# neu-vi/Superpoints_Registration

Hardware: AMD Instinct MI355X
Metric: point-cloud pairs/sec (16 384 pts/cloud) (higher is better)
Workload: dtype f32 (matrix products: range-scaled split-f16x2 MFMA, f32 accumulate; attention weights below 2^-5 of their row sum carried in one f16 plane); 1 GPU; synthetic 16384-pt pairs, full KPConv backbone + superpoint attn + Sinkhorn-SVD pose (3dmatch config, BASELINE configs[1]); streams_per_gpu=1, points_per_cloud=16384, generator=box, point_order=reference, upsample_indices=True, cross_step_overlap=True, streams_inside_a_forward=3: main path, pyramid searches, ResNet shortcut branches

## Files before the change

### include/spr.h

```cpp
#ifndef SPR_H_
#define SPR_H_

#include <stddef.h>
#include <stdint.h>

#ifdef __cplusplus
extern "C" {
#endif

#define SPR_VERSION 5

#define SPR_ACT_NONE 0
#define SPR_ACT_RELU 1
#define SPR_ACT_SIGMOID 2

#define SPR_ORDER_REFERENCE 0
#define SPR_ORDER_CANONICAL 1

int spr_version(void);
const char* spr_last_error(void);

size_t spr_grid_subsample_workspace_bytes(int n, int nb);
int spr_grid_subsample(const float* xyz, const int* cu, int n, int nb, float dl,
                       int max_p, int order_mode, float* out_xyz, int* out_lens,
                       int* out_total, void* ws, size_t ws_bytes, void* stream);

size_t spr_voxel_downsample_workspace_bytes(int n);
int spr_voxel_downsample(const float* xyz, int n, double voxel_size, int* out_idx,
                         int* out_count, void* ws, size_t ws_bytes, void* stream);

size_t spr_radius_neighbors_workspace_bytes(int nq, int ns, int nb);
int spr_radius_neighbors(const float* q_xyz, const int* q_cu, int nq,
                         const float* s_xyz, const int* s_cu, int ns, int nb,
                         float radius, int limit, int algo, int* out_idx,
                         int* max_count, void* ws, size_t ws_bytes, void* stream);

size_t spr_radius_table_bytes(int ns, int nb);
size_t spr_radius_table_build_workspace_bytes(int ns, int nb);
size_t spr_radius_table_query_workspace_bytes(int nq);
int spr_radius_table_slots(void);
int spr_radius_table_build(const float* s_xyz, const int* s_cu, int ns, int nb, float radius,
                           void* table, size_t table_bytes, void* ws, size_t ws_bytes, void* stream);
int spr_radius_table_query(const float* q_xyz, const int* q_cu, int nq, int self, int ns, int nb,
                           float radius, int limit, int slot, const void* table, int* out_idx,
                           int* max_count, void* ws, size_t ws_bytes, void* stream);
int spr_radius_table_query_a(const float* q_xyz, const int* q_cu, int nq, int self, int ns, int nb,
                             float radius, int limit, int slot, const void* table, int* out_idx,
                             int* max_count, int algo, void* ws, size_t ws_bytes, void* stream);

size_t spr_kpconv_workspace_bytes(int nq, int ns, int cin, int cout);
int spr_kpconv_fwd(const float* q_xyz, int nq, const float* s_xyz, int ns,
                   const int* nbr, int nbr_stride, int kmax, int rows_sorted,
                   const float* x, int cin, const float* weights, int cout,
                   const float* kernel_points, int n_kp, float kp_extent,
                   float* out, int impl, void* ws, size_t ws_bytes,
                   void* stream);

size_t spr_instnorm_workspace_bytes(int max_len_host, int nb, int c);
int spr_instnorm(const float* x, const int* cu, int n, int nb, int max_len_host,
                 int c, float eps, int norm, const float* add, float slope,
                 float* out, void* ws, size_t ws_bytes, void* stream);

int spr_block_tail_tile_rows(int ka, int kb, int n_out);
size_t spr_block_tail_tiles_len(int n, int nb, int tile_rows);
int spr_block_tail_tiles(const int* cu, int n, int nb, int tile_rows, int* tiles, void* stream);
size_t spr_block_tail_workspace_bytes(int n, int nb, int kb, int n_out, int tile_rows);
int spr_block_tail(const float* xa, int ka, const float* wa, const float* xb, int kb,
                   const float* wb, const float* add, const int* cu, const int* tiles, int n,
                   int nb, int n_out, float eps, float slope, float* out,
                   const float* xa_range, int xa_range_n, const float* wa_range, int wa_range_n,
                   const float* xb_range, int xb_range_n, const float* wb_range, int wb_range_n,
                   float* out_range, int out_range_n, void* ws, size_t ws_bytes, void* stream);
int spr_block_tail_n(const float* xa, int ka, const float* wa, const float* xb, int kb, const float* wb,
                     const float* add, const int* cu, const int* tiles, int n, int nb, int n_out, float eps,
                     float slope, float* out, const float* xa_range, int xa_range_n, const float* wa_range,
                     int wa_range_n, const float* xb_range, int xb_range_n, const float* wb_range,
                     int wb_range_n, float* out_range, int out_range_n, const float* xa_mean,
                     const float* xa_rstd, float xa_slope, void* ws, size_t ws_bytes, void* stream);
int spr_instnorm_stats(const float* x, const int* cu, int n, int nb, int max_len_host, int c, float eps,
                       float* mean, float* rstd, void* ws, size_t ws_bytes, void* stream);

int spr_maxpool_gather(const float* x, int ns, int c, const int* idx, int nq,
                       int idx_stride, int k, float* out, void* stream);

size_t spr_linear_workspace_bytes(void);
int spr_linear(const float* x, int m, int k, const float* w, int n,
               const float* bias, const float* residual, int act, float* out,
               void* ws, size_t ws_bytes, void* stream);
int spr_range_parts(void);
int spr_absmax(const float* x, long rows, int cols, long stride, float* parts, void* stream);
int spr_absmax_multi(const void* jobs_dev, int njobs, int parts_per_job, float* parts_out, void* stream);
int spr_linear_r(const float* x, int m, int k, const float* w, int n, const float* bias,
                 const float* residual, int act, float* out, const float* x_range,
                 int x_range_n, const float* w_range, int w_range_n, float* out_range,
                 int out_range_cap, int* out_range_n_host, void* ws, size_t ws_bytes, void* stream);
int spr_kpconv_fwd_r(const float* q_xyz, int nq, const float* s_xyz, int ns, const int* nbr,
                     int nbr_stride, int kmax, int rows_sorted, const float* x, int cin,
                     const float* weights, int cout, const float* kernel_points, int n_kp,
                     float kp_extent, float* out, int impl, const float* x_range, int x_range_n,
                     const float* w_range, int w_range_n, void* ws, size_t ws_bytes, void* stream);
size_t spr_kpconv_plan_bytes(int nq);
int spr_kpconv_plan(const int* nbr, int nq, int ns, int nbr_stride, int kmax, int rows_sorted,
                    const int* order, void* plan, size_t plan_bytes, void* stream);
size_t spr_kpconv_wplanes_bytes(int cin, int cout);
int spr_kpconv_prep_weights(const float* weights, int n_kp, int cin, int cout, const float* w_range,
                            int w_range_n, void* wplanes, size_t wplanes_bytes, void* stream);
int spr_kpconv_fwd_p(const float* q_xyz, int nq, const float* s_xyz, int ns, const int* nbr,
                     int nbr_stride, int kmax, int rows_sorted, const float* x, int cin,
                     const float* weights, int cout, const float* kernel_points, int n_kp,
                     float kp_extent, float* out, int impl, const float* x_range, int x_range_n,
                     const float* w_range, int w_range_n, const void* plan, const void* wplanes,
                     void* ws, size_t ws_bytes, void* stream);
int spr_instnorm_r(const float* x, const int* cu, int n, int nb, int max_len_host, int c,
                   float eps, int norm, const float* add, float slope, float* out,
                   float* out_range, int out_range_n, void* ws, size_t ws_bytes, void* stream);
int spr_maxpool_gather_r(const float* x, int ns, int c, const int* idx, int nq, int idx_stride,
                         int k, float* out, float* out_range, int out_range_n, void* stream);
int spr_maxpool_gather_o(const float* x, int ns, int c, const int* idx, int nq, int idx_stride, int k,
                         const int* order, float* out, float* out_range, int out_range_n, void* stream);
size_t spr_cell_order_workspace_bytes(int n);
int spr_cell_order(const float* xyz, const int* cu, int n, int nb, float cell, int* order, void* ws, size_t ws_bytes,
                   void* stream);
int spr_layernorm_range_count(int m);
int spr_layernorm_r(const float* x, int m, int c, const float* gamma, const float* beta,
                    float eps, const float* pos, float* out_norm, float* out_pos,
                    float* range_norm, float* range_pos, void* stream);
int spr_attn_inproj_prepare(const float* w_in, int d, float* out, void* stream);
int spr_attn_inproj_varlen_fwd_r(const float* x_qk, const float* x_v, int t, const float* w_in,
                                 const float* b_in, const int* cu, const int* kv_seg, int nseg,
                                 int max_len_host, int nhead, int head_dim, float scale,
                                 float* out, int o_stride, const float* xqk_range,
                                 int xqk_range_n, const float* xv_range, int xv_range_n,
                                 float* out_range, const float* w_prep, void* ws, size_t ws_bytes, void* stream);

int spr_set_gemm_mode(int mode);

int spr_layernorm(const float* x, int m, int c, const float* gamma,
                  const float* beta, float eps, const float* pos,
                  float* out_norm, float* out_pos, void* stream);

int spr_posemb_sine(const float* xyz, int n, int d_model, float scale,
                    float temperature, float* out, void* stream);

size_t spr_attn_workspace_bytes(int t, int nseg, int nhead, int head_dim);
int spr_attn_varlen_fwd(const float* q, int q_stride, const float* k,
                        int k_stride, const float* v, int v_stride,
                        const int* cu, const int* kv_seg, int t, int nseg,
                        int max_len_host, int nhead, int head_dim, float scale,
                        float* out, int o_stride, void* ws, size_t ws_bytes,
                        void* stream);
int spr_attn_varlen_fwd_lse(const float* q, int q_stride, const float* k, int k_stride, const float* v,
                            int v_stride, const int* cu, const int* kv_seg, int t, int nseg, int max_len_host,
                            int nhead, int head_dim, float scale, float* out, int o_stride, float* lse,
                            int* lse_written, void* ws, size_t ws_bytes, void* stream);

size_t spr_attn_inproj_workspace_bytes(int t, int nseg, int nhead, int head_dim);
int spr_attn_inproj_varlen_fwd(const float* x_qk, const float* x_v, int t,
                               const float* w_in, const float* b_in,
                               const int* cu, const int* kv_seg, int nseg,
                               int max_len_host, int nhead, int head_dim,
                               float scale, float* out, int o_stride, void* ws,
                               size_t ws_bytes, void* stream);

size_t spr_attn_probs_workspace_bytes(int t, int nhead, int head_dim);
int spr_attn_probs(const float* q, int q_stride, const float* k, int k_stride, const int* cu,
                   const int* kv_seg, int t, int nseg, int max_len_host, int nhead, int head_dim,
                   float scale, int per_head, float* out, const long long* place, int max_rows_host,
                   int max_cols_host, void* ws, size_t ws_bytes, void* stream);

#define SPR_XENC_PTRS_PER_LAYER 18
size_t spr_xenc_prepared_bytes(int n_layers, int d_ff);
size_t spr_xenc_plan_bytes(void);
int spr_xenc_prepare(const void* const* layer_ptrs_host, const float* eps_host, int n_layers,
                     int d_model, int nhead, int d_ff, const float* final_g, const float* final_b,
                     float final_eps, float pos_bound, void* prepared, size_t prepared_bytes,
                     void* plan_host, size_t plan_bytes, void* stream);
size_t spr_xenc_workspace_bytes(int t, int nseg);
int spr_xenc_forward(const void* plan_host, const float* x, const float* pos, const int* cu,
                     const int* kv_self, const int* kv_cross, int t, int nseg, int max_len_host,
                     float* out, void* ws, size_t ws_bytes, void* stream);

size_t spr_attn_bwd_workspace_bytes(int t, int nhead);
size_t spr_attn_bwd_workspace_bytes2(int t, int nseg, int nhead);
int spr_attn_varlen_bwd(const float* q, int q_stride, const float* k, int k_stride, const float* v,
                        int v_stride, const float* out, int o_stride, const float* dout,
                        int do_stride, const int* cu, const int* kv_seg, const int* q_seg, int t,
                        int nseg, int max_len_host, int nhead, int head_dim, float scale,
                        float* dq, float* dk, float* dv, void* ws, size_t ws_bytes, void* stream);
int spr_attn_varlen_bwd_lse(const float* q, int q_stride, const float* k, int k_stride, const float* v,
                            int v_stride, const float* out, int o_stride, const float* dout, int do_stride,
                            const float* lse, const int* cu, const int* kv_seg, const int* q_seg, int t, int nseg,
                            int max_len_host, int nhead, int head_dim, float scale, float* dq, float* dk,
                            float* dv, void* ws, size_t ws_bytes, void* stream);

int spr_set_attn_mode(int mode);

size_t spr_match_workspace_bytes(const int* cu_host, int npairs);
int spr_match_dualsoftmax(const float* feat, int d, const int* cu,
                          const int* cu_host, int npairs, float* match_val,
                          int* match_ind, void* ws, size_t ws_bytes,
                          void* stream);

int spr_match_dualsoftmax2(const float* feat, int d, const int* cu,
                           const int* cu_host, int npairs, float* match_val,
                           float* match_val2, int* match_ind, void* ws, size_t ws_bytes,
                           void* stream);

int spr_pose_residuals(const float* pose, const float* a, const float* b, const int* pair_cu,
                       int npairs, int total_host, float* res, void* stream);
int spr_pose_scores(const float* poses, int nh, const float* a, const float* b, int n,
                    float* score, void* stream);

int spr_weighted_procrustes(const float* a, const float* b, const float* w,
                            const int* pair_cu, int npairs, float* out_pose,
                            void* stream);

size_t spr_sinkhorn_workspace_bytes(const int* cu_host, int npairs);
int spr_sinkhorn_correspondences(const float* feat, int d, const float* xyz,
                                 const int* cu, const int* cu_host, int npairs,
                                 const float* alpha, const float* beta, int n_iters,
                                 int slack, float* out_w, float* out_that,
                                 void* ws, size_t ws_bytes, void* stream);

int spr_match_sinkhorn(const float* feat, int d, const float* xyz, const int* cu, const int* cu_host,
                       int npairs, const float* alpha, const float* beta, int n_iters, float* match_val,
                       float* match_val2, int* match_ind, float* out_w, float* out_that, void* ws,
                       size_t ws_bytes, void* stream);

int spr_gather_rows(const float* x, int n_src, int c, const int* idx, int n,
                    float* out, void* stream);

size_t spr_loss_workspace_bytes(int n_max, int m_max, int d);
int spr_overlap_pool(const float* ov_prev, int ns_prev, const int* pool,
                     int pool_stride, int w, int nq, float* out, void* stream);
int spr_bce_logits_mean(const float* x, const float* y, int n, float* out,
                        void* ws, size_t ws_bytes, void* stream);
int spr_infonce_pair(const float* anchor_feat, int n, const float* positive_feat,
                     int m, int d, const float* anchor_xyz, const float* pose_gt,
                     const float* positive_xyz, const float* W, float r_p,
                     float r_n, float* out, void* ws, size_t ws_bytes,
                     void* stream);
int spr_transform_l1_pair(const float* pose_gt, const float* pose_pred,
                          const float* xyz, int n, float* out, void* ws,
                          size_t ws_bytes, void* stream);
int spr_sum_scaled(const float* values, int n, float scale, float* out,
                   void* stream);

int spr_bgemm(const float* A, const float* B, float* C, const void* desc_dev, int nbatch,
              int max_m, int max_n, long sa_i, long sa_k, long sb_k, long sb_j, long sc_i,
              long sc_j, float alpha, float beta, void* stream);
size_t spr_tn_product_split_workspace_bytes(void);
int spr_tn_product_split(const float* L, const float* R, long rows, int nl, int nr, int chunk,
                         const float* l_range, int l_range_n, const float* r_range, int r_range_n,
                         float* parts, void* ws, size_t ws_bytes, void* stream);
size_t spr_tn_product_f64_workspace_bytes(long rows, int nl, int nr);
int spr_tn_product_f64(const float* L, const float* R, long rows, int nl, int nr, float* out,
                       void* ws, size_t ws_bytes, void* stream);
int spr_reduce_parts(const float* parts, int nparts, long n, float scale, float* out,
                     int accumulate, void* stream);
int spr_act_bwd(const float* y, const float* dy, int act, long n, float* out, void* stream);
size_t spr_colsum_workspace_bytes(int n);
int spr_colsum(const float* x, long m, int n, float* out, void* ws, size_t ws_bytes, void* stream);
size_t spr_layernorm_bwd_workspace_bytes(int c);
int spr_layernorm_bwd(const float* x, int m, int c, const float* gamma, float eps,
                      const float* dy_norm, const float* dy_pos, float* dx, float* dgamma,
                      float* dbeta, void* ws, size_t ws_bytes, void* stream);
size_t spr_instnorm_bwd_workspace_bytes(int max_len_host, int nb, int c);
int spr_instnorm_bwd(const float* x, const float* out, const float* dout, const int* cu, int n,
                     int nb, int max_len_host, int c, float eps, int norm, float slope,
                     float* dx, float* dadd, void* ws, size_t ws_bytes, void* stream);
size_t spr_scatter_workspace_bytes(long rows, int c);
int spr_maxpool_bwd(const float* x, int ns, int c, const int* idx, int nq, int idx_stride, int k,
                    const float* dy, float* dx, void* ws, size_t ws_bytes, void* stream);
int spr_scatter_rows_add(const float* dy, const int* idx, int n, int c, int n_src, float* dx,
                         void* ws, size_t ws_bytes, void* stream);
int spr_kpconv_weighted_features(const float* q_xyz, int nq, const float* s_xyz, int ns,
                                 const int* nbr, int nbr_stride, int kmax, const float* x, int cin,
                                 const float* kernel_points, int n_kp, float kp_extent,
                                 float* wf, float* cnt, void* stream);
int spr_kpconv_weighted_features_f(const float* q_xyz, int nq, const float* s_xyz, int ns,
                                   const int* nbr, int nbr_stride, int kmax, const float* x, int cin,
                                   const float* kernel_points, int n_kp, float kp_extent,
                                   float* wf, float* cnt, void* ws, size_t ws_bytes, void* stream);
size_t spr_kpconv_weighted_features_workspace_bytes(int ns);
int spr_kpconv_bwd_dx(const float* q_xyz, int nq, const float* s_xyz, int ns, const int* nbr,
                      int nbr_stride, int kmax, int cin, const float* kernel_points, int n_kp,
                      float kp_extent, const float* dwf, float* dx, void* ws, size_t ws_bytes,
                      void* stream);
int spr_kpconv_bwd_dx_r(const float* q_xyz, int nq, const float* s_xyz, int ns, const int* nbr,
                        int nbr_stride, int kmax, int cin, const float* kernel_points, int n_kp,
                        float kp_extent, const float* dwf, const float* dwf_range, int dwf_range_n, float* dx,
                        void* ws, size_t ws_bytes, void* stream);
int spr_softmax_rows(float* mat, const void* desc_dev, int nbatch, int max_m, void* stream);
int spr_softmax_bwd_rows(const float* p, float* dp, const void* desc_dev, int nbatch, int max_m,
                         void* stream);

int spr_bce_logits_mean_bwd(const float* x, const float* y, int n, const float* gout, float* dx,
                            void* stream);
int spr_infonce_pair_dlogits(const float* anchor_feat, int n, const float* positive_feat, int m,
                             int d, const float* anchor_xyz, const float* pose_gt,
                             const float* positive_xyz, const float* W, float r_p, float r_n,
                             float* dlogits, float* row_mask, float* wsym_out, float* t_out,
                             void* ws, size_t ws_bytes, void* stream);
int spr_wsym_bwd(const float* dwsym, int d, float* dW, void* stream);
int spr_transform_l1_pair_bwd(const float* pose_gt, const float* pose_pred, const float* xyz, int n,
                              const float* gout, float* dpose_pred, void* stream);
int spr_weighted_procrustes_bwd(const float* a, const float* b, const float* w,
                                const int* pair_cu, int npairs, const float* dpose, float* da,
                                float* db, float* dw, void* stream);
size_t spr_sinkhorn_bwd_workspace_bytes(const int* cu_host, int npairs, int n_iters);
int spr_sinkhorn_bwd(const float* feat, int d, const float* xyz, const int* cu,
                     const int* cu_host, int npairs, const float* alpha, const float* beta,
                     int n_iters, const float* dw, const float* dthat, float* dfeat,
                     float* dalpha, float* dbeta, void* ws, size_t ws_bytes, void* stream);

size_t spr_circle_loss_workspace_bytes(int nbatch, int max_n, int max_m);
int spr_circle_loss(const float* src_feat, const float* tgt_feat, int d, const float* src_xyz,
                    const float* pose_gt, const float* tgt_xyz, const int* cu_src, const int* cu_tgt,
                    int nbatch, int max_n, int max_m, float r_p, float r_n, float* out, void* ws,
                    size_t ws_bytes, void* stream);
int spr_circle_loss_bwd(const float* src_feat, const float* tgt_feat, int d, const float* src_xyz,
                        const float* pose_gt, const float* tgt_xyz, const int* cu_src, const int* cu_tgt,
                        int nbatch, int max_n, int max_m, float r_p, float r_n, const float* gout, float* G,
                        float* d_src, float* d_tgt, void* ws, size_t ws_bytes, void* stream);

int spr_prof_enable(int on);
int spr_prof_read(int max_records, int* codes_host, int* nqs_host, float* ms_host);

int spr_selftest(int* status_host);

#ifdef __cplusplus
}
#endif
#endif
```

### superpoints_registration_amd/_lib.py

```python
import ctypes
import os
import subprocess

_HERE = os.path.dirname(os.path.abspath(__file__))
LIB_PATH = os.environ.get("SPR_HIP_LIB") or os.path.join(_HERE, "libspr_hip.so")

_vp = ctypes.c_void_p
_i = ctypes.c_int
_f = ctypes.c_float
_sz = ctypes.c_size_t
_l = ctypes.c_long

SIGNATURES = {
    "spr_version": (_i, []),
    "spr_last_error": (ctypes.c_char_p, []),
    "spr_grid_subsample_workspace_bytes": (_sz, [_i, _i]),
    "spr_grid_subsample": (_i, [_vp, _vp, _i, _i, _f, _i, _i, _vp, _vp, _vp, _vp, _sz, _vp]),
    "spr_voxel_downsample_workspace_bytes": (_sz, [_i]),
    "spr_voxel_downsample": (_i, [_vp, _i, ctypes.c_double, _vp, _vp, _vp, _sz, _vp]),
    "spr_radius_neighbors_workspace_bytes": (_sz, [_i, _i, _i]),
    "spr_radius_neighbors": (_i, [_vp, _vp, _i, _vp, _vp, _i, _i, _f, _i, _i, _vp, _vp, _vp, _sz, _vp]),
    "spr_radius_table_bytes": (_sz, [_i, _i]),
    "spr_radius_table_build_workspace_bytes": (_sz, [_i, _i]),
    "spr_radius_table_query_workspace_bytes": (_sz, [_i]),
    "spr_radius_table_slots": (_i, []),
    "spr_radius_table_build": (_i, [_vp, _vp, _i, _i, _f, _vp, _sz, _vp, _sz, _vp]),
    "spr_radius_table_query": (_i, [_vp, _vp, _i, _i, _i, _i, _f, _i, _i, _vp, _vp, _vp, _vp, _sz, _vp]),
    "spr_radius_table_query_a": (_i, [_vp, _vp, _i, _i, _i, _i, _f, _i, _i, _vp, _vp, _vp, _i, _vp, _sz, _vp]),
    "spr_kpconv_workspace_bytes": (_sz, [_i, _i, _i, _i]),
    "spr_kpconv_fwd": (_i, [_vp, _i, _vp, _i, _vp, _i, _i, _i, _vp, _i, _vp, _i, _vp, _i, _f, _vp,
                            _i, _vp, _sz, _vp]),
    "spr_instnorm_workspace_bytes": (_sz, [_i, _i, _i]),
    "spr_instnorm": (_i, [_vp, _vp, _i, _i, _i, _i, _f, _i, _vp, _f, _vp, _vp, _sz, _vp]),
    "spr_maxpool_gather": (_i, [_vp, _i, _i, _vp, _i, _i, _i, _vp, _vp]),
    "spr_linear_workspace_bytes": (_sz, []),
    "spr_linear": (_i, [_vp, _i, _i, _vp, _i, _vp, _vp, _i, _vp, _vp, _sz, _vp]),
    "spr_linear_r": (_i, [_vp, _i, _i, _vp, _i, _vp, _vp, _i, _vp, _vp, _i, _vp, _i, _vp, _i, _vp, _vp, _sz, _vp]),
    "spr_range_parts": (_i, []),
    "spr_absmax_multi": (_i, [_vp, _i, _i, _vp, _vp]),
    "spr_absmax": (_i, [_vp, _l, _i, _l, _vp, _vp]),
    "spr_kpconv_fwd_r": (_i, [_vp, _i, _vp, _i, _vp, _i, _i, _i, _vp, _i, _vp, _i, _vp, _i, _f, _vp,
                              _i, _vp, _i, _vp, _i, _vp, _sz, _vp]),
    "spr_kpconv_plan_bytes": (_sz, [_i]),
    "spr_kpconv_plan": (_i, [_vp, _i, _i, _i, _i, _i, _vp, _vp, _sz, _vp]),
    "spr_kpconv_wplanes_bytes": (_sz, [_i, _i]),
    "spr_kpconv_prep_weights": (_i, [_vp, _i, _i, _i, _vp, _i, _vp, _sz, _vp]),
    "spr_kpconv_fwd_p": (_i, [_vp, _i, _vp, _i, _vp, _i, _i, _i, _vp, _i, _vp, _i, _vp, _i, _f, _vp,
                              _i, _vp, _i, _vp, _i, _vp, _vp, _vp, _sz, _vp]),
    "spr_instnorm_r": (_i, [_vp, _vp, _i, _i, _i, _i, _f, _i, _vp, _f, _vp, _vp, _i, _vp, _sz, _vp]),
    "spr_block_tail_tile_rows": (_i, [_i, _i, _i]),
    "spr_block_tail_tiles_len": (_sz, [_i, _i, _i]),
    "spr_block_tail_tiles": (_i, [_vp, _i, _i, _i, _vp, _vp]),
    "spr_block_tail_workspace_bytes": (_sz, [_i, _i, _i, _i, _i]),
    "spr_block_tail": (_i, [_vp, _i, _vp, _vp, _i, _vp, _vp, _vp, _vp, _i, _i, _i, _f, _f, _vp, _vp, _i, _vp, _i,
                            _vp, _i, _vp, _i, _vp, _i, _vp, _sz, _vp]),
    "spr_block_tail_n": (_i, [_vp, _i, _vp, _vp, _i, _vp, _vp, _vp, _vp, _i, _i, _i, _f, _f, _vp, _vp, _i, _vp, _i,
                              _vp, _i, _vp, _i, _vp, _i, _vp, _vp, _f, _vp, _sz, _vp]),
    "spr_instnorm_stats": (_i, [_vp, _vp, _i, _i, _i, _i, _f, _vp, _vp, _vp, _sz, _vp]),
    "spr_maxpool_gather_r": (_i, [_vp, _i, _i, _vp, _i, _i, _i, _vp, _vp, _i, _vp]),
    "spr_maxpool_gather_o": (_i, [_vp, _i, _i, _vp, _i, _i, _i, _vp, _vp, _vp, _i, _vp]),
    "spr_cell_order_workspace_bytes": (_sz, [_i]),
    "spr_cell_order": (_i, [_vp, _vp, _i, _i, _f, _vp, _vp, _sz, _vp]),
    "spr_layernorm_range_count": (_i, [_i]),
    "spr_layernorm_r": (_i, [_vp, _i, _i, _vp, _vp, _f, _vp, _vp, _vp, _vp, _vp, _vp]),
    "spr_attn_inproj_varlen_fwd_r": (_i, [_vp, _vp, _i, _vp, _vp, _vp, _vp, _i, _i, _i, _i, _f, _vp, _i, _vp, _i, _vp,
                                          _i, _vp, _vp, _vp, _sz, _vp]),
    "spr_attn_inproj_prepare": (_i, [_vp, _i, _vp, _vp]),
    "spr_set_gemm_mode": (_i, [_i]),
    "spr_layernorm": (_i, [_vp, _i, _i, _vp, _vp, _f, _vp, _vp, _vp, _vp]),
    "spr_posemb_sine": (_i, [_vp, _i, _i, _f, _f, _vp, _vp]),
    "spr_attn_workspace_bytes": (_sz, [_i, _i, _i, _i]),
    "spr_attn_varlen_fwd": (_i, [_vp, _i, _vp, _i, _vp, _i, _vp, _vp, _i, _i, _i, _i, _i, _f, _vp, _i,
                                 _vp, _sz, _vp]),
    "spr_attn_varlen_fwd_lse": (_i, [_vp, _i, _vp, _i, _vp, _i, _vp, _vp, _i, _i, _i, _i, _i, _f, _vp, _i, _vp, _vp,
                                     _vp, _sz, _vp]),
    "spr_attn_varlen_bwd_lse": (_i, [_vp, _i, _vp, _i, _vp, _i, _vp, _i, _vp, _i, _vp, _vp, _vp, _vp, _i, _i, _i, _i,
                                     _i, _f, _vp, _vp, _vp, _vp, _sz, _vp]),
    "spr_attn_probs_workspace_bytes": (_sz, [_i, _i, _i]),
    "spr_attn_probs": (_i, [_vp, _i, _vp, _i, _vp, _vp, _i, _i, _i, _i, _i, _f, _i, _vp, _vp, _i, _i, _vp, _sz,
                            _vp]),
    "spr_attn_bwd_workspace_bytes": (_sz, [_i, _i]),
    "spr_attn_bwd_workspace_bytes2": (_sz, [_i, _i, _i]),
    "spr_attn_varlen_bwd": (_i, [_vp, _i, _vp, _i, _vp, _i, _vp, _i, _vp, _i, _vp, _vp, _vp, _i, _i, _i, _i, _i, _f,
                                 _vp, _vp, _vp, _vp, _sz, _vp]),
    "spr_attn_inproj_workspace_bytes": (_sz, [_i, _i, _i, _i]),
    "spr_attn_inproj_varlen_fwd": (_i, [_vp, _vp, _i, _vp, _vp, _vp, _vp, _i, _i, _i, _i, _f, _vp, _i, _vp,
                                        _sz, _vp]),
    "spr_set_attn_mode": (_i, [_i]),
    "spr_xenc_prepared_bytes": (_sz, [_i, _i]),
    "spr_xenc_plan_bytes": (_sz, []),
    "spr_xenc_prepare": (_i, [_vp, _vp, _i, _i, _i, _i, _vp, _vp, _f, _f, _vp, _sz, _vp, _sz, _vp]),
    "spr_xenc_workspace_bytes": (_sz, [_i, _i]),
    "spr_xenc_forward": (_i, [_vp, _vp, _vp, _vp, _vp, _vp, _i, _i, _i, _vp, _vp, _sz, _vp]),
    "spr_match_workspace_bytes": (_sz, [_vp, _i]),
    "spr_match_dualsoftmax": (_i, [_vp, _i, _vp, _vp, _i, _vp, _vp, _vp, _sz, _vp]),
    "spr_match_dualsoftmax2": (_i, [_vp, _i, _vp, _vp, _i, _vp, _vp, _vp, _vp, _sz, _vp]),
    "spr_pose_residuals": (_i, [_vp, _vp, _vp, _vp, _i, _i, _vp, _vp]),
    "spr_pose_scores": (_i, [_vp, _i, _vp, _vp, _i, _vp, _vp]),
    "spr_weighted_procrustes": (_i, [_vp, _vp, _vp, _vp, _i, _vp, _vp]),
    "spr_sinkhorn_workspace_bytes": (_sz, [_vp, _i]),
    "spr_match_sinkhorn": (_i, [_vp, _i, _vp, _vp, _vp, _i, _vp, _vp, _i, _vp, _vp, _vp, _vp, _vp, _vp, _sz, _vp]),
    "spr_sinkhorn_correspondences": (_i, [_vp, _i, _vp, _vp, _vp, _i, _vp, _vp, _i, _i, _vp, _vp, _vp,
                                          _sz, _vp]),
    "spr_loss_workspace_bytes": (_sz, [_i, _i, _i]),
    "spr_overlap_pool": (_i, [_vp, _i, _vp, _i, _i, _i, _vp, _vp]),
    "spr_bce_logits_mean": (_i, [_vp, _vp, _i, _vp, _vp, _sz, _vp]),
    "spr_infonce_pair": (_i, [_vp, _i, _vp, _i, _i, _vp, _vp, _vp, _vp, _f, _f, _vp, _vp, _sz, _vp]),
    "spr_transform_l1_pair": (_i, [_vp, _vp, _vp, _i, _vp, _vp, _sz, _vp]),
    "spr_sum_scaled": (_i, [_vp, _i, _f, _vp, _vp]),
    "spr_gather_rows": (_i, [_vp, _i, _i, _vp, _i, _vp, _vp]),
    "spr_bgemm": (_i, [_vp, _vp, _vp, _vp, _i, _i, _i, _l, _l, _l, _l, _l, _l, _f, _f, _vp]),
    "spr_tn_product_split_workspace_bytes": (_sz, []),
    "spr_tn_product_split": (_i, [_vp, _vp, _l, _i, _i, _i, _vp, _i, _vp, _i, _vp, _vp, _sz, _vp]),
    "spr_tn_product_f64_workspace_bytes": (_sz, [_l, _i, _i]),
    "spr_tn_product_f64": (_i, [_vp, _vp, _l, _i, _i, _vp, _vp, _sz, _vp]),
    "spr_reduce_parts": (_i, [_vp, _i, _l, _f, _vp, _i, _vp]),
    "spr_act_bwd": (_i, [_vp, _vp, _i, _l, _vp, _vp]),
    "spr_colsum_workspace_bytes": (_sz, [_i]),
    "spr_colsum": (_i, [_vp, _l, _i, _vp, _vp, _sz, _vp]),
    "spr_layernorm_bwd_workspace_bytes": (_sz, [_i]),
    "spr_layernorm_bwd": (_i, [_vp, _i, _i, _vp, _f, _vp, _vp, _vp, _vp, _vp, _vp, _sz, _vp]),
    "spr_instnorm_bwd_workspace_bytes": (_sz, [_i, _i, _i]),
    "spr_instnorm_bwd": (_i, [_vp, _vp, _vp, _vp, _i, _i, _i, _i, _f, _i, _f, _vp, _vp, _vp, _sz, _vp]),
    "spr_scatter_workspace_bytes": (_sz, [_l, _i]),
    "spr_maxpool_bwd": (_i, [_vp, _i, _i, _vp, _i, _i, _i, _vp, _vp, _vp, _sz, _vp]),
    "spr_scatter_rows_add": (_i, [_vp, _vp, _i, _i, _i, _vp, _vp, _sz, _vp]),
    "spr_kpconv_weighted_features_workspace_bytes": (_sz, [_i]),
    "spr_kpconv_weighted_features": (_i, [_vp, _i, _vp, _i, _vp, _i, _i, _vp, _i, _vp, _i, _f, _vp, _vp, _vp]),
    "spr_kpconv_weighted_features_f": (_i, [_vp, _i, _vp, _i, _vp, _i, _i, _vp, _i, _vp, _i, _f, _vp, _vp, _vp, _sz, _vp]),
    "spr_kpconv_bwd_dx": (_i, [_vp, _i, _vp, _i, _vp, _i, _i, _i, _vp, _i, _f, _vp, _vp, _vp, _sz, _vp]),
    "spr_kpconv_bwd_dx_r": (_i, [_vp, _i, _vp, _i, _vp, _i, _i, _i, _vp, _i, _f, _vp, _vp, _i, _vp, _vp, _sz, _vp]),
    "spr_softmax_rows": (_i, [_vp, _vp, _i, _i, _vp]),
    "spr_softmax_bwd_rows": (_i, [_vp, _vp, _vp, _i, _i, _vp]),
    "spr_bce_logits_mean_bwd": (_i, [_vp, _vp, _i, _vp, _vp, _vp]),
    "spr_infonce_pair_dlogits": (_i, [_vp, _i, _vp, _i, _i, _vp, _vp, _vp, _vp, _f, _f, _vp, _vp, _vp, _vp, _vp, _sz,
                                      _vp]),
    "spr_wsym_bwd": (_i, [_vp, _i, _vp, _vp]),
    "spr_transform_l1_pair_bwd": (_i, [_vp, _vp, _vp, _i, _vp, _vp, _vp]),
    "spr_weighted_procrustes_bwd": (_i, [_vp, _vp, _vp, _vp, _i, _vp, _vp, _vp, _vp, _vp]),
    "spr_sinkhorn_bwd_workspace_bytes": (_sz, [_vp, _i, _i]),
    "spr_sinkhorn_bwd": (_i, [_vp, _i, _vp, _vp, _vp, _i, _vp, _vp, _i, _vp, _vp, _vp, _vp, _vp, _vp, _sz, _vp]),
    "spr_circle_loss_workspace_bytes": (_sz, [_i, _i, _i]),
    "spr_circle_loss": (_i, [_vp, _vp, _i, _vp, _vp, _vp, _vp, _vp, _i, _i, _i, _f, _f, _vp, _vp, _sz, _vp]),
    "spr_circle_loss_bwd": (_i, [_vp, _vp, _i, _vp, _vp, _vp, _vp, _vp, _i, _i, _i, _f, _f, _vp, _vp, _vp, _vp, _vp,
                                 _sz, _vp]),
    "spr_selftest": (_i, [_vp]),
    "spr_prof_enable": (_i, [_i]),
    "spr_prof_read": (_i, [_i, _vp, _vp, _vp]),
}

_lib = None


def build(force: bool = False) -> str:
    if force:
        subprocess.check_call(["make", "-s", "-C", os.path.join(_HERE, "csrc"), "clean"])
    subprocess.check_call(["make", "-s", "-j8", "-C", os.path.join(_HERE, "csrc")])
    return LIB_PATH


def lib():
    global _lib
    if _lib is None:
        if not os.path.exists(LIB_PATH):
            raise RuntimeError(
                f"{LIB_PATH} is missing: build it with "
                "`python -c 'import __graft_entry__ as g; g.build()'` "
                "(there is no fallback path)")
        l = ctypes.CDLL(LIB_PATH)
        for name, (res, args) in SIGNATURES.items():
            fn = getattr(l, name)
            fn.restype = res
            fn.argtypes = args
        _lib = l
    return _lib


def check(rc: int, what: str) -> None:
    if rc != 0:
        msg = lib().spr_last_error()
        raise RuntimeError(f"{what}: {msg.decode() if msg else 'error'} (status {rc})")
```

### superpoints_registration_amd/csrc/kpconv.hip

```cpp
#include "spr_common.h"

namespace spr {
namespace {

constexpr int kKP = 15;

__global__ __launch_bounds__(256) void k_rowflag(const float* __restrict__ x, const float* __restrict__ s_xyz,
                                                 int ns, int cin, unsigned char* __restrict__ flag,
                                                 float4* __restrict__ sxf, int* __restrict__ tile_ctr) {
  const int wid = (blockIdx.x * blockDim.x + threadIdx.x) >> 6;
  const int lane = threadIdx.x & 63;
  const int c4 = cin >> 2;
  if (blockIdx.x == 0 && threadIdx.x == 0) {
    sxf[ns] = make_float4(-1.0e17f, -1.0e17f, -1.0e17f, __int_as_float(0));
    tile_ctr[0] = 0;
  }
  if ((cin & 3) == 0 && c4 <= 64 && (c4 & (c4 - 1)) == 0) {
    constexpr int kRfSteps = 4;
    const int rpl = 64 / c4;
    const int sub = lane / c4, chunk = lane % c4;
    const int row0 = wid * rpl * kRfSteps + sub;
    float4 v[kRfSteps];
#pragma unroll
    for (int r = 0; r < kRfSteps; ++r) {
      const int row = row0 + r * rpl;
      v[r] = make_float4(0.f, 0.f, 0.f, 0.f);
      if (row < ns) v[r] = reinterpret_cast<const float4*>(x + (size_t)row * cin)[chunk];
    }
#pragma unroll
    for (int r = 0; r < kRfSteps; ++r) {
      const int row = row0 + r * rpl;
      float c[4] = {v[r].x, v[r].y, v[r].z, v[r].w};
#pragma unroll
      for (int e = 0; e < 4; ++e) {
        float t = c[e];
        if (c4 == 64) {
          const int b = lane & 15;
          const float a0 = __shfl(t, b, 64), a1 = __shfl(t, b | 16, 64), a2 = __shfl(t, b | 32, 64),
                      a3 = __shfl(t, b | 48, 64);
          t = ((a0 + a1) + a2) + a3;
        } else if (c4 == 32) {
          t += __shfl_xor(t, 16, 64);
        }
        for (int o = (c4 < 16 ? c4 : 16) >> 1; o > 0; o >>= 1) t += __shfl_xor(t, o, 64);
        c[e] = t;
      }
      const float t = (c[0] + c[2]) + (c[1] + c[3]);
      if (chunk == 0 && row < ns) {
        const int f = t > 0.f ? 1 : 0;
        flag[row] = (unsigned char)f;
        sxf[row] = make_float4(s_xyz[3 * (size_t)row], s_xyz[3 * (size_t)row + 1],
                               s_xyz[3 * (size_t)row + 2], __int_as_float(f));
      }
    }
    return;
  }
  const int row = wid;
  if (row >= ns) return;
  float s = 0.f;
  for (int c = lane; c < cin; c += 64) s += x[(size_t)row * cin + c];
  s = wave_sum(s);
  if (lane == 0) {
    const int f = s > 0.f ? 1 : 0;
    flag[row] = (unsigned char)f;
    sxf[row] = make_float4(s_xyz[3 * (size_t)row], s_xyz[3 * (size_t)row + 1],
                           s_xyz[3 * (size_t)row + 2], __int_as_float(f));
  }
}

__global__ void k_kpconv_simple(const float* __restrict__ q_xyz, int nq,
                                const float* __restrict__ s_xyz, int ns,
                                const int* __restrict__ nbr, int nbr_stride, int kmax,
                                const float* __restrict__ x, int cin,
                                const float* __restrict__ W, int cout,
                                const float* __restrict__ kpts, int n_kp, float inv_extent,
                                const unsigned char* __restrict__ flag,
                                float* __restrict__ out) {
  const long gid = (long)blockIdx.x * blockDim.x + threadIdx.x;
  if (gid >= (long)nq * cout) return;
  const int n = (int)(gid / cout), o = (int)(gid % cout);
  const float qx = q_xyz[3 * (size_t)n], qy = q_xyz[3 * (size_t)n + 1], qz = q_xyz[3 * (size_t)n + 2];
  float acc = 0.f;
  int cnt = 0;
  for (int k = 0; k < kmax; ++k) {
    const int idx = nbr[(size_t)n * nbr_stride + k];
    if (idx < 0 || idx >= ns) continue;
    cnt += flag[idx];
    const float rx = s_xyz[3 * (size_t)idx] - qx, ry = s_xyz[3 * (size_t)idx + 1] - qy,
                rz = s_xyz[3 * (size_t)idx + 2] - qz;
    for (int p = 0; p < n_kp; ++p) {
      const float dx = rx - kpts[3 * p], dy = ry - kpts[3 * p + 1], dz = rz - kpts[3 * p + 2];
      const float w = fmaxf(0.f, 1.f - sqrtf(dx * dx + dy * dy + dz * dz) * inv_extent);
      if (w > 0.f) {
        float d = 0.f;
        for (int c = 0; c < cin; ++c)
          d += x[(size_t)idx * cin + c] * W[((size_t)p * cin + c) * cout + o];
        acc += w * d;
      }
    }
  }
  out[(size_t)n * cout + o] = acc / (float)max(cnt, 1);
}

__global__ __launch_bounds__(256) void k_records_cin1(const float* __restrict__ x, const float* __restrict__ s_xyz,
                                                      int ns, float4* __restrict__ sxf) {
  const int i = blockIdx.x * blockDim.x + threadIdx.x;
  if (i < ns) sxf[i] = make_float4(s_xyz[3 * (size_t)i], s_xyz[3 * (size_t)i + 1], s_xyz[3 * (size_t)i + 2], x[i]);
}

__global__ __launch_bounds__(256) void k_kpconv_cin1(
    const float* __restrict__ q_xyz, int nq, const float* __restrict__ s_xyz, int ns,
    const int* __restrict__ nbr, int nbr_stride, int kmax, int rows_sorted,
    const float4* __restrict__ sxf, const float* __restrict__ W, int cout,
    const float* __restrict__ kpts, int n_kp, float inv_extent, float* __restrict__ out) {
  const int lane = threadIdx.x & 63, wave = threadIdx.x >> 6;
  const int qv = lane & 15, g = lane >> 4;
  const int q0 = blockIdx.x * 64 + wave * 16;
  if (q0 >= nq) return;
  const int n = min(q0 + qv, nq - 1);
  const float qx = q_xyz[3 * (size_t)n], qy = q_xyz[3 * (size_t)n + 1], qz = q_xyz[3 * (size_t)n + 2];
  float kx[4], ky[4], kz[4];
  bool kok[4];
#pragma unroll
  for (int s = 0; s < 4; ++s) {
    const int p = 4 * s + g;
    kok[s] = p < n_kp;
    kx[s] = kok[s] ? kpts[3 * p] : 0.f;
    ky[s] = kok[s] ? kpts[3 * p + 1] : 0.f;
    kz[s] = kok[s] ? kpts[3 * p + 2] : 0.f;
  }
  float wf[4] = {0.f, 0.f, 0.f, 0.f};
  int cnt = 0;
  const int* row = nbr + (size_t)n * nbr_stride;
  for (int k = 0; k < kmax; ++k) {
    const int idx = row[k];
    const bool ok = idx >= 0 && idx < ns;
    if (rows_sorted && __ballot(ok) == 0ull) break;
    const size_t id = ok ? (size_t)idx : 0;
    const float4 rec = sxf[id];
    const float xv = ok ? rec.w : 0.f;
    cnt += xv > 0.f ? 1 : 0;
    const float rx = rec.x - qx, ry = rec.y - qy, rz = rec.z - qz;
#pragma unroll
    for (int s = 0; s < 4; ++s) {
      const float dx = rx - kx[s], dy = ry - ky[s], dz = rz - kz[s];
      const float w = fmaxf(0.f, 1.f - __builtin_amdgcn_sqrtf(dx * dx + dy * dy + dz * dz) * inv_extent);
      wf[s] += kok[s] ? w * xv : 0.f;
    }
  }
  const float inv = 1.f / (float)max(cnt, 1);
#pragma unroll
  for (int s = 0; s < 4; ++s) wf[s] *= inv;
  for (int o0 = 0; o0 < cout; o0 += 16) {
    f32x4 acc = {0.f, 0.f, 0.f, 0.f};
#pragma unroll
    for (int s = 0; s < 4; ++s) {
      const int p = 4 * s + g;
      const float bv = (p < n_kp && o0 + qv < cout) ? W[(size_t)p * cout + o0 + qv] : 0.f;
      acc = __builtin_amdgcn_mfma_f32_16x16x4f32(wf[s], bv, acc, 0, 0, 0);
    }
#pragma unroll
    for (int r = 0; r < 4; ++r) {
      const int qn = q0 + 4 * g + r;
      if (qn < nq && o0 + qv < cout) out[(size_t)qn * cout + o0 + qv] = acc[r];
    }
  }
}

__global__ __launch_bounds__(256) void k_w_prep(const float* __restrict__ W, int cin, int cout, int cc,
                                                const float* __restrict__ w_parts, int n_wparts,
                                                _Float16* __restrict__ Wh, _Float16* __restrict__ Wl) {
  __shared__ float sh[17];
  const float sb = pow2f(pow2_exp_for(block_absmax(w_parts, sh, n_wparts)));
  const int total = kKP * cin * cout;
  const int i = blockIdx.x * blockDim.x + threadIdx.x;
  if (i >= total) return;
  const int KS = kKP * cc / 32, NT = cout / 16;
  const int e = i & 7, lane = (i >> 3) & 63;
  int r = i >> 9;
  const int ks = r % KS;
  r /= KS;
  const int nt = r % NT, chunk = r / NT;
  const int p16 = lane & 15, j4 = lane >> 4;
  const int kk = 32 * ks + 8 * j4 + e;
  const int p = kk / cc, c = chunk * cc + kk % cc;
  const float w = W[((size_t)p * cin + c) * cout + 16 * nt + p16] * sb;
  const _Float16 h = (_Float16)w;
  Wh[i] = h;
  Wl[i] = (_Float16)(w - (float)h);
}

__device__ __forceinline__ void wait_vm(int n) {
  switch (n) {
    case 0: asm volatile("s_waitcnt vmcnt(0)" ::: "memory"); break;
    case 2: asm volatile("s_waitcnt vmcnt(2)" ::: "memory"); break;
    case 4: asm volatile("s_waitcnt vmcnt(4)" ::: "memory"); break;
    case 6: asm volatile("s_waitcnt vmcnt(6)" ::: "memory"); break;
    case 8: asm volatile("s_waitcnt vmcnt(8)" ::: "memory"); break;
    case 12: asm volatile("s_waitcnt vmcnt(12)" ::: "memory"); break;
    case 16: asm volatile("s_waitcnt vmcnt(16)" ::: "memory"); break;
    default: asm volatile("s_waitcnt vmcnt(0)" ::: "memory"); break;
  }
}

typedef _Float16 kh8 __attribute__((ext_vector_type(8)));
template <int N> struct VecF;
template <> struct VecF<2> { typedef float type __attribute__((ext_vector_type(2))); };
template <> struct VecF<4> { typedef float type __attribute__((ext_vector_type(4))); };
template <int N> struct VecH;
template <> struct VecH<2> { typedef _Float16 type __attribute__((ext_vector_type(2))); };
template <> struct VecH<4> { typedef _Float16 type __attribute__((ext_vector_type(4))); };

template <int NTC>
struct KpItem {
  int idx[4];
  float4 sp[4];
  float b[4][NTC];
  float qx, qy, qz;
};

template <int CC, int TQ, int NTW, int NW, int SK, int P1W>
__global__ __launch_bounds__(64 * P1W) void k_kpconv_mfma(
    const float* __restrict__ q_xyz, int nq, const float* __restrict__ s_xyz, int ns,
    const int* __restrict__ nbr, int nbr_stride, int kmax, int rows_sorted,
    const float* __restrict__ x, int cin, const _Float16* __restrict__ Wh,
    const _Float16* __restrict__ Wl, int cout, const float* __restrict__ kpts, float inv_extent,
    const float4* __restrict__ sxf, const float* __restrict__ x_parts,
    const float* __restrict__ w_parts, int n_xparts, int n_wparts, float* __restrict__ out) {
  constexpr int NTC = CC / 16;
  constexpr int MT = TQ / 16;
  constexpr int KW = kKP * CC;
  constexpr int SH = KW + 16;
  constexpr int QPW = TQ / P1W;
  constexpr int NTHR = 64 * P1W;
  static_assert(P1W >= NW && TQ % P1W == 0, "phase-1 waves");
  extern __shared__ __align__(16) unsigned char lds_raw[];
  _Float16* wfh = (_Float16*)lds_raw;
  _Float16* wfl = wfh + TQ * SH;
  int* lcnt = (int*)(wfl + TQ * SH);
  int* lnit = lcnt + TQ;
  int* litem = lnit + P1W;
  const int nblk = (kmax + 15) >> 4;
  const int KP = nblk * 16;
  int* lidx = litem + P1W * QPW * nblk;

  const int tid = threadIdx.x;
  const int wave = tid >> 6, lane = tid & 63;
  const int p16 = lane & 15, j4 = lane >> 4;

  float kx = 0.f, ky = 0.f, kz = 0.f;
  if (p16 < kKP) {
    kx = kpts[3 * p16];
    ky = kpts[3 * p16 + 1];
    kz = kpts[3 * p16 + 2];
  }

  float sa, unscale;
  {
    float* shf = reinterpret_cast<float*>(lds_raw);
    const int ka = pow2_exp_for(block_absmax(x_parts, shf, n_xparts) * (float)kmax);
    const int kb = pow2_exp_for(block_absmax(w_parts, shf, n_wparts));
    __syncthreads();
    sa = pow2f(ka);
    unscale = pow2f(-ka - kb);
  }

  const int ntiles = (nq + TQ - 1) / TQ;
  for (int tile = blockIdx.x; tile < ntiles; tile += gridDim.x) {
  const int q0 = tile * TQ;

  for (int e = tid; e < TQ * KP; e += NTHR) {
    const int q = e / KP, k = e - q * KP;
    const int n = q0 + q;
    lidx[e] = (n < nq && k < kmax) ? nbr[(size_t)n * nbr_stride + k] : ns;
  }
  __syncthreads();
  {
    int n_it = 0;
    for (int qi = 0; qi < QPW; ++qi) {
      const int* row = lidx + (wave * QPW + qi) * KP;
      int nb = nblk;
      if (rows_sorted) {
        int v = 0;
        for (int k0 = 0; k0 < KP; k0 += 64) {
          const int k = k0 + lane;
          const bool ok = k < KP && row[min(k, KP - 1)] >= 0 && row[min(k, KP - 1)] < ns;
          v += __popcll(__ballot(ok));
        }
        nb = max(1, (v + 15) >> 4);
      }
      if (lane < nb) litem[wave * QPW * nblk + n_it + lane] = (qi << 8) | ((lane == nb - 1) ? 128 : 0) | lane;
      n_it += nb;
    }
    if (lane == 0) lnit[wave] = n_it;
  }
  __syncthreads();
  const int n_items = lnit[wave];
  const int* my_items = litem + wave * QPW * nblk;

  constexpr int NG = (SK == 1) ? NW / MT : NW / SK;
  constexpr int MTW = (SK == 1) ? 1 : MT;
  const int mt = (SK == 1) ? wave % MT : 0;
  const int ng = (SK == 1) ? wave / MT : wave % NG;
  const int kh = (SK == 1) ? 0 : wave / NG;
  f32x4 acc2[MTW][NTW];
#pragma unroll
  for (int m = 0; m < MTW; ++m)
#pragma unroll
    for (int t = 0; t < NTW; ++t) acc2[m][t] = (f32x4){0.f, 0.f, 0.f, 0.f};

  for (int c0 = 0; c0 < cin; c0 += CC) {
    f32x4 acc1[NTC];
#pragma unroll
    for (int t = 0; t < NTC; ++t) acc1[t] = (f32x4){0.f, 0.f, 0.f, 0.f};
    int cnt = 0;

    auto issue = [&](int it, KpItem<NTC>& I) {
      const int code = my_items[min(it, n_items - 1)];
      const int qi = code >> 8, b = code & 127;
      const int n = min(q0 + wave * QPW + qi, nq - 1);
      const int* row = lidx + (wave * QPW + qi) * KP + b * 16 + j4;
      I.qx = q_xyz[3 * (size_t)n];
      I.qy = q_xyz[3 * (size_t)n + 1];
      I.qz = q_xyz[3 * (size_t)n + 2];
#pragma unroll
      for (int s = 0; s < 4; ++s) {
        const int id_ = row[4 * s];
        I.idx[s] = id_;
        const bool ok = id_ >= 0 && id_ < ns;
        const size_t id = ok ? (size_t)id_ : 0;
        I.sp[s] = sxf[id];
        typedef typename VecF<NTC>::type vec_t;
        const vec_t xv = *reinterpret_cast<const vec_t*>(x + id * cin + c0 + NTC * p16);
#pragma unroll
        for (int t = 0; t < NTC; ++t) I.b[s][t] = xv[t];
      }
    };
    auto compute = [&](int it, const KpItem<NTC>& I) {
      if (it >= n_items) return;
      const int code = my_items[it];
#pragma unroll
      for (int s = 0; s < 4; ++s) {
        const bool ok = I.idx[s] >= 0 && I.idx[s] < ns;
        const float dx = (I.sp[s].x - I.qx) - kx, dy = (I.sp[s].y - I.qy) - ky,
                    dz = (I.sp[s].z - I.qz) - kz;
        float w = fmaxf(0.f, 1.f - __builtin_amdgcn_sqrtf(dx * dx + dy * dy + dz * dz) * inv_extent);
        if (!ok || p16 >= kKP) w = 0.f;
        cnt += (ok && c0 == 0 && p16 == 0) ? __float_as_int(I.sp[s].w) : 0;
#pragma unroll
        for (int t = 0; t < NTC; ++t) {
          acc1[t] = __builtin_amdgcn_mfma_f32_16x16x4f32(w, I.b[s][t], acc1[t], 0, 0, 0);
        }
      }
      if (code & 128) {
        const int ql = wave * QPW + (code >> 8);
#pragma unroll
        for (int r = 0; r < 4; ++r) {
          const int p = 4 * j4 + r;
          typedef typename VecH<NTC>::type hv_t;
          hv_t hh, ll;
          if constexpr (NTC == 2) {
            unsigned int hu, lu;
            split_pk_s(acc1[0][r], acc1[1][r], sa, hu, lu);
            hh = __builtin_bit_cast(hv_t, hu);
            ll = __builtin_bit_cast(hv_t, lu);
          } else {
            static_assert(NTC == 4, "NTC is 2 or 4");
            typedef unsigned int u2_t __attribute__((ext_vector_type(2)));
            unsigned int h0, l0, h1, l1;
            split_pk_s(acc1[0][r], acc1[1][r], sa, h0, l0);
            split_pk_s(acc1[2][r], acc1[3][r], sa, h1, l1);
            hh = __builtin_bit_cast(hv_t, (u2_t){h0, h1});
            ll = __builtin_bit_cast(hv_t, (u2_t){l0, l1});
          }
          if (p < kKP) {
            *reinterpret_cast<hv_t*>(wfh + ql * SH + p * CC + NTC * p16) = hh;
            *reinterpret_cast<hv_t*>(wfl + ql * SH + p * CC + NTC * p16) = ll;
          }
        }
#pragma unroll
        for (int t = 0; t < NTC; ++t) acc1[t] = (f32x4){0.f, 0.f, 0.f, 0.f};
        if (c0 == 0) {
          int c = cnt;
          c += __shfl_xor(c, 16, 64);
          c += __shfl_xor(c, 32, 64);
          if (lane == 0) lcnt[ql] = c;
        }
        cnt = 0;
      }
    };

    {
      KpItem<NTC> A, B;
      issue(0, A);
      for (int it = 0; it < n_items; it += 2) {
        issue(it + 1, B);
        compute(it, A);
        issue(it + 2, A);
        compute(it + 1, B);
      }
    }
    __syncthreads();
    if (wave < NW) {
      constexpr int NBATCH = KW / 32 / SK;
      const int ks0 = kh * NBATCH;
      constexpr int LPB = 2 * NTW;
      constexpr int D = (NTW <= 2) ? 5 : 3;
      static_assert(NBATCH % D == 0 && NBATCH >= 2 * D && (D - 1) * LPB <= 16, "ring shape");
      const _Float16* ah_row = wfh + (mt * 16 + p16) * SH + 8 * j4;
      const _Float16* al_row = wfl + (mt * 16 + p16) * SH + 8 * j4;
      constexpr int KS = KW / 32;
      const size_t wofs = ((size_t)(c0 / CC) * (cout / 16) + ng * NTW) * KS * 512 + lane * 8;
      kh8 bh[D][NTW], bl[D][NTW];
      auto load_step = [&](int ks, kh8 (&dh)[NTW], kh8 (&dl)[NTW]) {
        const size_t gk = wofs + (size_t)(ks0 + ks) * 512;
#pragma unroll
        for (int t = 0; t < NTW; ++t) {
          const _Float16* ph = Wh + gk + (size_t)t * KS * 512;
          const _Float16* pl = Wl + gk + (size_t)t * KS * 512;
          asm volatile("global_load_dwordx4 %0, %1, off" : "=v"(dh[t]) : "v"(ph));
          asm volatile("global_load_dwordx4 %0, %1, off" : "=v"(dl[t]) : "v"(pl));
        }
      };
      auto mma_step = [&](int ks, const kh8 (&sh)[NTW], const kh8 (&sl)[NTW]) {
#pragma unroll
        for (int m = 0; m < MTW; ++m) {
          const kh8 ah = *reinterpret_cast<const kh8*>(ah_row + m * 16 * SH + 32 * (ks0 + ks));
          const kh8 al = *reinterpret_cast<const kh8*>(al_row + m * 16 * SH + 32 * (ks0 + ks));
#pragma unroll
          for (int t = 0; t < NTW; ++t) {
            acc2[m][t] = __builtin_amdgcn_mfma_f32_16x16x32_f16(ah, sl[t], acc2[m][t], 0, 0, 0);
            acc2[m][t] = __builtin_amdgcn_mfma_f32_16x16x32_f16(al, sh[t], acc2[m][t], 0, 0, 0);
            acc2[m][t] = __builtin_amdgcn_mfma_f32_16x16x32_f16(ah, sh[t], acc2[m][t], 0, 0, 0);
          }
        }
      };
      wait_vm(0);
#pragma unroll
      for (int d = 0; d < D; ++d) load_step(d, bh[d], bl[d]);
      for (int b0 = 0; b0 < NBATCH - D; b0 += D) {
#pragma unroll
        for (int d = 0; d < D; ++d) {
          wait_vm((D - 1) * LPB);
          __builtin_amdgcn_sched_barrier(0);
          mma_step(b0 + d, bh[d], bl[d]);
          __builtin_amdgcn_sched_barrier(0);
          load_step(b0 + d + D, bh[d], bl[d]);
        }
      }
#pragma unroll
      for (int d = 0; d < D; ++d) {
        wait_vm((D - 1 - d) * LPB);
        __builtin_amdgcn_sched_barrier(0);
        mma_step(NBATCH - D + d, bh[d], bl[d]);
      }
    }
    __syncthreads();
  }
  const bool writer = (SK == 1) ? (wave < NW) : (wave < NW && kh == 0);
  if (SK == 2) {
    float* red = reinterpret_cast<float*>(lds_raw);
    if (wave < NW && kh == 1) {
#pragma unroll
      for (int m = 0; m < MTW; ++m)
#pragma unroll
        for (int t = 0; t < NTW; ++t)
#pragma unroll
          for (int r = 0; r < 4; ++r)
            red[(((ng * MTW + m) * NTW + t) * 4 + r) * 64 + lane] = acc2[m][t][r];
    }
    __syncthreads();
    if (writer) {
#pragma unroll
      for (int m = 0; m < MTW; ++m)
#pragma unroll
        for (int t = 0; t < NTW; ++t)
#pragma unroll
          for (int r = 0; r < 4; ++r)
            acc2[m][t][r] += red[(((ng * MTW + m) * NTW + t) * 4 + r) * 64 + lane];
    }
  }
  if (writer) {
#pragma unroll
    for (int m = 0; m < MTW; ++m)
#pragma unroll
      for (int r = 0; r < 4; ++r) {
        const int ql = (mt + m) * 16 + 4 * j4 + r;
        const int n = q0 + ql;
        if (n < nq) {
          const float inv = unscale / (float)max(lcnt[ql], 1);
#pragma unroll
          for (int t = 0; t < NTW; ++t)
            out[(size_t)n * cout + (ng * NTW + t) * 16 + p16] = acc2[m][t][r] * inv;
        }
      }
  }
  __syncthreads();
  }
}

template <int CC, int TQ, int NTW, int NW, int SK, int P1W = NW>
int launch_mfma(const float* q_xyz, int nq, const float* s_xyz, int ns, const int* nbr,
                int nbr_stride, int kmax, int rows_sorted, const float* x, int cin,
                const _Float16* Wh, const _Float16* Wl, int cout, const float* kpts,
                float inv_extent, const float4* sxf, const float* x_parts, const float* w_parts, int n_xparts,
                int n_wparts, float* out, hipStream_t stream) {
  constexpr int SH = kKP * CC + 16;
  constexpr int QPW = TQ / P1W;
  const int nblk = (kmax + 15) / 16;
  const size_t lds = 2 * sizeof(_Float16) * (size_t)TQ * SH + sizeof(int) * (TQ + P1W) +
                     sizeof(int) * (size_t)P1W * QPW * nblk + sizeof(int) * (size_t)TQ * nblk * 16;
  auto kern = k_kpconv_mfma<CC, TQ, NTW, NW, SK, P1W>;
  ProfScope prof(stream, cin * 100000 + cout, nq);
  SPR_REQUIRE(lds <= 160 * 1024, "kpconv: neighbour rows too wide for the LDS tile (kmax=%d)", kmax);
  if (lds > 64 * 1024)
    if (int rc = ensure_dyn_lds((const void*)kern, 160 * 1024)) return rc;
  const int n_cu = device_cu_count();
  const int per_cu = (int)((160 * 1024) / lds) > 0 ? (int)((160 * 1024) / lds) : 1;
  const int ntiles = cdiv(nq, TQ);
  const int grid = ntiles < n_cu * per_cu ? ntiles : n_cu * per_cu;
  hipLaunchKernelGGL(kern, dim3(grid), dim3(64 * P1W), lds, stream, q_xyz, nq, s_xyz, ns,
                     nbr, nbr_stride, kmax, rows_sorted, x, cin, Wh, Wl, cout, kpts, inv_extent,
                     sxf, x_parts, w_parts, n_xparts, n_wparts, out);
  SPR_LAUNCH_CHECK();
  return 0;
}


constexpr int kRingTQ = 16;
#ifndef SPR_KP_NS64
#define SPR_KP_NS64 4
#endif

__global__ __launch_bounds__(256) void k_kp_tiles(const int* __restrict__ nbr, int nq, int ns, int nbr_stride,
                                                  int kmax, int rows_sorted, const int* __restrict__ order,
                                                  int ntiles, int4* __restrict__ desc, int* __restrict__ pad_word) {
  const int tile = (blockIdx.x * blockDim.x + threadIdx.x) >> 6;
  const int lane = threadIdx.x & 63;
  if (blockIdx.x == 0 && threadIdx.x == 0) pad_word[0] = ns;
  if (tile >= ntiles) return;
  int my_q = -1, my_c = 0;
  for (int r = 0; r < kRingTQ; ++r) {
    const int pos = tile * kRingTQ + r;
    int q = -1, c = 0;
    if (pos < nq) {
      q = order ? order[pos] : pos;
      if (rows_sorted) {
        int v = 0;
        for (int k0 = 0; k0 < kmax; k0 += 64) {
          const int k = k0 + lane;
          const int id = k < kmax ? nbr[(size_t)q * nbr_stride + k] : ns;
          v += __popcll(__ballot(id >= 0 && id < ns));
        }
        c = max(1, (v + 7) >> 3);
      } else {
        c = (kmax + 7) >> 3;
      }
    }
    if (lane == r) { my_q = q; my_c = c; }
  }
  int rank = 0;
  for (int j = 0; j < kRingTQ; ++j) {
    const int cj = __shfl(my_c, j, 64);
    rank += (cj > my_c || (cj == my_c && j < lane)) ? 1 : 0;
  }
  if (lane < kRingTQ) {
    int* d = reinterpret_cast<int*>(desc + (size_t)tile * 8);
    const int w = rank < 8 ? rank : 15 - rank, second = rank < 8 ? 0 : 1;
    d[w * 4 + second] = my_q;
    d[w * 4 + 2 + second] = my_c;
  }
}

__device__ __forceinline__ void ring_dma16(const void* base, unsigned off, unsigned dst_s) {
  unsigned keep;
  asm volatile(
      "s_waitcnt lgkmcnt(0)\n\ts_mov_b32 %0, m0\n\ts_mov_b32 m0, %3\n\ts_nop 0\n\t"
      "global_load_lds_dwordx4 %1, %2\n\ts_mov_b32 m0, %0"
      : "=&s"(keep) : "v"(off), "s"(base), "s"(dst_s) : "memory");
}
__device__ __forceinline__ void ring_dma16_nw(const void* base, unsigned off, unsigned dst_s) {
  unsigned keep;
  asm volatile(
      "s_mov_b32 %0, m0\n\ts_mov_b32 m0, %3\n\ts_nop 0\n\t"
      "global_load_lds_dwordx4 %1, %2\n\ts_mov_b32 m0, %0"
      : "=&s"(keep) : "v"(off), "s"(base), "s"(dst_s) : "memory");
}
__device__ __forceinline__ void ring_dma16_m0(const void* base, unsigned off, unsigned dst_s) {
  asm volatile("s_mov_b32 m0, %2\n\ts_nop 0\n\tglobal_load_lds_dwordx4 %0, %1"
               : : "v"(off), "s"(base), "s"(dst_s) : "memory", "m0");
}
__device__ __forceinline__ void ring_dma16_rec8(const void* base, unsigned off, unsigned dst_s) {
  unsigned long long keep;
  asm volatile(
      "s_mov_b64 %0, exec\n\ts_mov_b64 exec, 0xff\n\ts_mov_b32 m0, %3\n\ts_nop 0\n\t"
      "global_load_lds_dwordx4 %1, %2\n\ts_mov_b64 exec, %0"
      : "=&s"(keep) : "v"(off), "s"(base), "s"(dst_s) : "memory", "m0");
}
template <int PPI, int RB>
__device__ __forceinline__ void ring_item_dma(const void* x, const void* x_m1k, const void* sx_m, unsigned off0,
                                              unsigned off1, unsigned off_rec, unsigned dst_s) {
  unsigned long long keep;
  if constexpr (PPI == 2) {
    asm volatile(
        "s_mov_b32 m0, %7\n\ts_nop 0\n\t"
        "global_load_lds_dwordx4 %1, %4\n\t"
        "global_load_lds_dwordx4 %2, %5 offset:1024\n\t"
        "s_mov_b64 %0, exec\n\ts_mov_b64 exec, 0xff\n\t"
        "global_load_lds_dwordx4 %3, %6 offset:%8\n\t"
        "s_mov_b64 exec, %0"
        : "=&s"(keep) : "v"(off0), "v"(off1), "v"(off_rec), "s"(x), "s"(x_m1k), "s"(sx_m), "s"(dst_s), "n"(8 * RB)
        : "memory", "m0");
  } else {
    asm volatile(
        "s_mov_b32 m0, %5\n\ts_nop 0\n\t"
        "global_load_lds_dwordx4 %1, %3\n\t"
        "s_mov_b64 %0, exec\n\ts_mov_b64 exec, 0xff\n\t"
        "global_load_lds_dwordx4 %2, %4 offset:%6\n\t"
        "s_mov_b64 exec, %0"
        : "=&s"(keep) : "v"(off0), "v"(off_rec), "s"(x), "s"(sx_m), "s"(dst_s), "n"(8 * RB)
        : "memory", "m0");
  }
}
__device__ __forceinline__ void ring_dma4(const void* base, unsigned off, unsigned dst_s) {
  unsigned keep;
  asm volatile(
      "s_waitcnt lgkmcnt(0)\n\ts_mov_b32 %0, m0\n\ts_mov_b32 m0, %3\n\ts_nop 0\n\t"
      "global_load_lds_dword %1, %2\n\ts_mov_b32 m0, %0"
      : "=&s"(keep) : "v"(off), "s"(base), "s"(dst_s) : "memory");
}
__device__ __forceinline__ void wait_vm_any(int n) {
  switch (n) {
    case 0: asm volatile("s_waitcnt vmcnt(0)" ::: "memory"); break;
    case 1: asm volatile("s_waitcnt vmcnt(1)" ::: "memory"); break;
    case 2: asm volatile("s_waitcnt vmcnt(2)" ::: "memory"); break;
    case 3: asm volatile("s_waitcnt vmcnt(3)" ::: "memory"); break;
    case 4: asm volatile("s_waitcnt vmcnt(4)" ::: "memory"); break;
    case 5: asm volatile("s_waitcnt vmcnt(5)" ::: "memory"); break;
    case 6: asm volatile("s_waitcnt vmcnt(6)" ::: "memory"); break;
    case 7: asm volatile("s_waitcnt vmcnt(7)" ::: "memory"); break;
    case 8: asm volatile("s_waitcnt vmcnt(8)" ::: "memory"); break;
    case 9: asm volatile("s_waitcnt vmcnt(9)" ::: "memory"); break;
    case 10: asm volatile("s_waitcnt vmcnt(10)" ::: "memory"); break;
    case 11: asm volatile("s_waitcnt vmcnt(11)" ::: "memory"); break;
    case 12: asm volatile("s_waitcnt vmcnt(12)" ::: "memory"); break;
    case 13: asm volatile("s_waitcnt vmcnt(13)" ::: "memory"); break;
    case 14: asm volatile("s_waitcnt vmcnt(14)" ::: "memory"); break;
    case 15: asm volatile("s_waitcnt vmcnt(15)" ::: "memory"); break;
    case 16: asm volatile("s_waitcnt vmcnt(16)" ::: "memory"); break;
    case 17: asm volatile("s_waitcnt vmcnt(17)" ::: "memory"); break;
    case 18: asm volatile("s_waitcnt vmcnt(18)" ::: "memory"); break;
    case 19: asm volatile("s_waitcnt vmcnt(19)" ::: "memory"); break;
    case 20: asm volatile("s_waitcnt vmcnt(20)" ::: "memory"); break;
    case 21: asm volatile("s_waitcnt vmcnt(21)" ::: "memory"); break;
    case 22: asm volatile("s_waitcnt vmcnt(22)" ::: "memory"); break;
    case 23: asm volatile("s_waitcnt vmcnt(23)" ::: "memory"); break;
    case 24: asm volatile("s_waitcnt vmcnt(24)" ::: "memory"); break;
    case 25: asm volatile("s_waitcnt vmcnt(25)" ::: "memory"); break;
    case 26: asm volatile("s_waitcnt vmcnt(26)" ::: "memory"); break;
    case 27: asm volatile("s_waitcnt vmcnt(27)" ::: "memory"); break;
    case 28: asm volatile("s_waitcnt vmcnt(28)" ::: "memory"); break;
    default: asm volatile("s_waitcnt vmcnt(0)" ::: "memory"); break;
  }
}

template <int CC, int COUT, int NS>
struct RingShape {
  static constexpr int NTC = CC / 16;
  static constexpr int KW = kKP * CC;
  static constexpr int SH = KW + 16;
  static constexpr int KS = KW / 32;
  static constexpr int NG = COUT / 16;
  static constexpr int SPLIT = 8 / NG;
  static constexpr int KSW = (KS + SPLIT - 1) / SPLIT;
  static constexpr int RB = CC * 4;
  static constexpr int LPR = RB / 16;
  static constexpr int RPP = 64 / LPR;
  static constexpr int PPI = 8 / RPP;
  static constexpr int DPI = PPI + 1;
  static constexpr int SLOT = 8 * RB + 128;
  static constexpr int WF_BYTES = 2 * kRingTQ * SH * 2;
  static constexpr int RED_BYTES = NG * (SPLIT - 1) * 4 * 64 * 4;
  static constexpr int RING_BYTES = 8 * NS * SLOT;
  static constexpr int SMALL_BYTES = 2 * kRingTQ * 4 * 2 + 16;
  static constexpr int MINW = (CC == 32 && COUT == 32) ? 4 : 2;
  static_assert(NG * SPLIT == 8 && NS >= 3, "shape");
  static __host__ __device__ size_t lds_bytes(int idxw) {
    return (size_t)WF_BYTES + RED_BYTES + RING_BYTES + SMALL_BYTES + (size_t)8 * 2 * 2 * idxw * 4;
  }
};

#ifdef SPR_KP_RING_PROF
constexpr int kTraceN = 160;
__device__ unsigned long long g_kp_trace[8 * kTraceN];
#define KP_STAMP(id)                                                                            \
  do {                                                                                          \
    if (blockIdx.x == 0 && trace_n < kTraceN) {                                                 \
      const unsigned long long t_ = __builtin_amdgcn_s_memtime();                               \
      if (lane == 0) trace_lds[wave * kTraceN + trace_n] = (t_ << 4) | (unsigned long long)(id); \
      ++trace_n;                                                                                \
    }                                                                                           \
  } while (0)
#else
#define KP_STAMP(id)
#endif

template <int CC, int COUT, int NS>
__global__ __launch_bounds__(512, (RingShape<CC, COUT, NS>::MINW)) void k_kpconv_ring(
    const float* __restrict__ q_xyz, int ns, const int* __restrict__ nbr, int nbr_stride, int kmax,
    const float* __restrict__ x, const _Float16* __restrict__ Wh, const _Float16* __restrict__ Wl,
    const float* __restrict__ kpts, float inv_extent, const float4* __restrict__ sxf,
    const int4* __restrict__ desc, int ntiles, const int* __restrict__ pad_word, int idxw,
    const float* __restrict__ x_parts, const float* __restrict__ w_parts, int n_xparts, int n_wparts,
    int* __restrict__ tile_ctr, float* __restrict__ out) {
  typedef RingShape<CC, COUT, NS> S;
  constexpr int NTC = S::NTC, SH = S::SH, KS = S::KS, NG = S::NG, SPLIT = S::SPLIT, KSW = S::KSW;
  constexpr int RB = S::RB, LPR = S::LPR, RPP = S::RPP, PPI = S::PPI, DPI = S::DPI, SLOT = S::SLOT;
  extern __shared__ __align__(16) unsigned char lds_raw[];
  _Float16* wfh = (_Float16*)lds_raw;
  _Float16* wfl = wfh + kRingTQ * SH;
  float* red = (float*)(lds_raw + S::WF_BYTES);
  unsigned char* ring_all = lds_raw + S::WF_BYTES + S::RED_BYTES;
  int* lcnt = (int*)(ring_all + S::RING_BYTES);
  int* lqid = lcnt + 2 * kRingTQ;
  int* ltile = lqid + 2 * kRingTQ;
  int* idx_all = ltile + 4;

  const int tid = threadIdx.x;
  const int lane = tid & 63;
  const int wave = __builtin_amdgcn_readfirstlane(tid >> 6);
  const int p16 = lane & 15, j4 = lane >> 4;
  unsigned char* ring = ring_all + wave * (NS * SLOT);
  int* idxbuf = idx_all + wave * (4 * idxw);
  const unsigned ring_s = (unsigned)(uintptr_t)ring;
  const unsigned idx_s = (unsigned)(uintptr_t)idxbuf;

  float kx = 1.0e18f, ky = 1.0e18f, kz = 1.0e18f;
  if (p16 < kKP) {
    kx = kpts[3 * p16];
    ky = kpts[3 * p16 + 1];
    kz = kpts[3 * p16 + 2];
  }
  float sa, unscale;
  {
    float* shf = reinterpret_cast<float*>(lds_raw);
    const int ka = pow2_exp_for(block_absmax(x_parts, shf, n_xparts) * (float)kmax);
    const int kb = pow2_exp_for(block_absmax(w_parts, shf, n_wparts));
    __syncthreads();
    sa = pow2f(ka);
    unscale = pow2f(-ka - kb);
  }

  const int ng = wave % NG, sp = wave / NG;
  const int ks0 = sp * KSW;
  kh8 bh[KSW], bl[KSW];
#pragma unroll
  for (int k = 0; k < KSW; ++k) {
    const int ks = ks0 + k;
    if (ks < KS) {
      const size_t o = ((size_t)ng * KS + ks) * 512 + lane * 8;
      bh[k] = *reinterpret_cast<const kh8*>(Wh + o);
      bl[k] = *reinterpret_cast<const kh8*>(Wl + o);
    } else {
#pragma unroll
      for (int e = 0; e < 8; ++e) { bh[k][e] = (_Float16)0.f; bl[k][e] = (_Float16)0.f; }
    }
  }
  asm volatile("s_waitcnt vmcnt(0)" ::: "memory");

  const int idxb = 2 * idxw;
  auto stage_idx = [&](const int4 d, int par) {
#pragma unroll
    for (int sel = 0; sel < 2; ++sel) {
      const int q = sel ? d.y : d.x;
      for (int h = 0; h < idxw; h += 64) {
        const int k = h + lane;
        const unsigned dst = __builtin_amdgcn_readfirstlane(idx_s + (par * idxb + (sel ? 8 * d.z : 0) + h) * 4);
        if (q >= 0 && k < kmax) ring_dma4(nbr, (unsigned)(((size_t)q * nbr_stride + k) * 4), dst);
        else ring_dma4(pad_word, 0u, dst);
      }
    }
  };
  struct Ids { unsigned row[PPI]; unsigned rec; };
  const unsigned a_idr = (lane / LPR) * 4, a_idc = (lane & 7) * 4;
  auto load_ids = [&](int par, int j) -> Ids {
    const unsigned char* base = reinterpret_cast<const unsigned char*>(idxbuf) + (par * idxb + 8 * j) * 4;
    Ids r;
#pragma unroll
    for (int pc = 0; pc < PPI; ++pc) r.row[pc] = *reinterpret_cast<const unsigned*>(base + a_idr + pc * RPP * 4);
    r.rec = *reinterpret_cast<const unsigned*>(base + a_idc);
    return r;
  };
  const unsigned a_dma = (lane % LPR) * 16;
  auto issue_ids = [&](unsigned slot_off, const Ids& ids) {
#ifdef SPR_KP_ABL_NODMA
    return;
#endif
    const unsigned slot = __builtin_amdgcn_readfirstlane(ring_s + slot_off);
#ifndef SPR_KP_RING_NO_LGKM
    asm volatile("s_waitcnt lgkmcnt(0)" ::: "memory");
#endif
#ifdef SPR_KP_ITEM_DMA_OLD
#pragma unroll
    for (int pc = 0; pc < PPI; ++pc) {
      const unsigned rid = min(ids.row[pc], (unsigned)(ns - 1));
      ring_dma16_m0(x, rid * RB + a_dma, slot + pc * 1024);
    }
    ring_dma16_rec8(sxf, min(ids.rec, (unsigned)ns) * 16, slot + 8 * RB);
#else
    static_assert(PPI == 1 || PPI == 2, "ring item: one or two row pieces");
    const unsigned o0 = min(ids.row[0], (unsigned)(ns - 1)) * RB + a_dma;
    const unsigned o1 = min(ids.row[PPI - 1], (unsigned)(ns - 1)) * RB + a_dma;
    const unsigned orec = min(ids.rec, (unsigned)ns) * 16;
    ring_item_dma<PPI, RB>(x, reinterpret_cast<const char*>(x) - 1024, reinterpret_cast<const char*>(sxf) - 8 * RB, o0, o1,
                           orec, slot);
#endif
  };
  auto prime = [&](const int4 d, int par) {
    const int n = d.z + d.w;
    Ids ids[NS];
#pragma unroll
    for (int i = 0; i < NS; ++i) ids[i] = load_ids(par, i);
#pragma unroll
    for (int i = 0; i < NS; ++i)
      if (i < n) issue_ids(i * SLOT, ids[i]);
  };

#ifdef SPR_KP_PRIO
  if (wave >= 4) __builtin_amdgcn_s_setprio(1);
#endif
  if (tid == 0) {
    const int t0 = __hip_atomic_fetch_add(tile_ctr, 3, __ATOMIC_RELAXED, __HIP_MEMORY_SCOPE_AGENT);
    ltile[0] = t0;
  }
  __syncthreads();
  int tile = __builtin_amdgcn_readfirstlane(ltile[0]);
  int tile_nxt = tile + 1, tile_nn = tile + 2;
  __syncthreads();
  int4 d_cur = make_int4(-1, -1, 0, 0), d_nxt = make_int4(-1, -1, 0, 0);
  if (tile < ntiles) d_cur = desc[(size_t)tile * 8 + wave];
  if (tile_nxt < ntiles) d_nxt = desc[(size_t)tile_nxt * 8 + wave];
  if (tile < ntiles) {
    stage_idx(d_cur, 0);
    asm volatile("s_waitcnt vmcnt(0)" ::: "memory");
    if (tile_nxt < ntiles) stage_idx(d_nxt, 1);
    prime(d_cur, 0);
  }

#ifdef SPR_KP_RING_PROF
  unsigned long long* trace_lds = reinterpret_cast<unsigned long long*>(lds_raw + S::lds_bytes(idxw));
  int trace_n = 0;
#endif
  typedef typename VecF<NTC>::type vec_t;
  struct KStep { float4 rec; vec_t xv; };
  const unsigned a_rec = 8 * RB + j4 * 16, a_xv = j4 * RB + p16 * (NTC * 4);
  auto ld_kstep = [&](unsigned slot_off, int s2) -> KStep {
    KStep k;
    k.rec = *reinterpret_cast<const float4*>(ring + slot_off + a_rec + s2 * 64);
    k.xv = *reinterpret_cast<const vec_t*>(ring + slot_off + a_xv + s2 * 4 * RB);
    return k;
  };
  float pend_v[4] = {0.f, 0.f, 0.f, 0.f};
  int pend_n[4] = {-1, -1, -1, -1};
  auto flush_pending = [&]() {
#pragma unroll
    for (int r = 0; r < 4; ++r)
      if (pend_n[r] >= 0) out[(size_t)pend_n[r] * COUT + ng * 16 + p16] = pend_v[r];
  };
  int par = 0;
  for (; tile < ntiles; par ^= 1) {
    const int4 d = d_cur;
    KP_STAMP(1);
    const int n_items = d.z + d.w;
    int4 d_nn = make_int4(-1, -1, 0, 0);
    const bool has_nxt = tile_nxt < ntiles, has_nn = tile_nn < ntiles;
    if (has_nn) d_nn = desc[(size_t)tile_nn * 8 + wave];
    int drawn = ntiles;
    if (tid == 0 && has_nn) drawn = __hip_atomic_fetch_add(tile_ctr, 1, __ATOMIC_RELAXED, __HIP_MEMORY_SCOPE_AGENT);

    float qax = 0.f, qay = 0.f, qaz = 0.f, qbx = 0.f, qby = 0.f, qbz = 0.f;
    if (d.x >= 0) { qax = q_xyz[3 * (size_t)d.x]; qay = q_xyz[3 * (size_t)d.x + 1]; qaz = q_xyz[3 * (size_t)d.x + 2]; }
    if (d.y >= 0) { qbx = q_xyz[3 * (size_t)d.y]; qby = q_xyz[3 * (size_t)d.y + 1]; qbz = q_xyz[3 * (size_t)d.y + 2]; }
    auto wait_item = [&](int i) {
      const int younger = n_items - 1 - i;
      if (younger >= NS - 2) wait_vm_any(DPI * (NS - 2));
      else wait_vm_any(DPI * max(younger, 0));
    };
    KStep R0, R1;
    if (n_items == 0) {
      wait_vm_any(0);
    } else {
      wait_item(0);
      R0 = ld_kstep(0, 0);
      R1 = ld_kstep(0, 1);
    }
    Ids ids_next = load_ids(par, NS);
    int i = 0;
    unsigned slot_off = 0;
    auto flush = [&](const f32x4 (&acc)[NTC], int cnt, int ql, int qid) {
#pragma unroll
      for (int r = 0; r < 4; ++r) {
        const int p = 4 * j4 + r;
        typedef typename VecH<NTC>::type hv_t;
        hv_t hh, ll;
        if constexpr (NTC == 2) {
          unsigned int hu, lu;
          split_pk_s(acc[0][r], acc[1][r], sa, hu, lu);
          hh = __builtin_bit_cast(hv_t, hu);
          ll = __builtin_bit_cast(hv_t, lu);
        } else {
          typedef unsigned int u2_t __attribute__((ext_vector_type(2)));
          unsigned int h0, l0, h1, l1;
          split_pk_s(acc[0][r], acc[1][r], sa, h0, l0);
          split_pk_s(acc[2][r], acc[3][r], sa, h1, l1);
          hh = __builtin_bit_cast(hv_t, (u2_t){h0, h1});
          ll = __builtin_bit_cast(hv_t, (u2_t){l0, l1});
        }
        if (p < kKP) {
          *reinterpret_cast<hv_t*>(wfh + ql * SH + p * CC + NTC * p16) = hh;
          *reinterpret_cast<hv_t*>(wfl + ql * SH + p * CC + NTC * p16) = ll;
        }
      }
      int c = cnt;
      c += __shfl_xor(c, 16, 64);
      c += __shfl_xor(c, 32, 64);
      if (lane == 0) {
        lcnt[par * kRingTQ + ql] = c;
        lqid[par * kRingTQ + ql] = qid;
      }
    };
    auto item = [&](f32x4 (&acc)[NTC], int& cnt, float qx, float qy, float qz, auto&& between) {
      KP_STAMP(2);
      const unsigned nslot = slot_off + SLOT == NS * SLOT ? 0u : slot_off + SLOT;
      {
        const float dx = (R0.rec.x - qx) - kx, dy = (R0.rec.y - qy) - ky, dz = (R0.rec.z - qz) - kz;
        const float w = fmaxf(0.f, 1.f - __builtin_amdgcn_sqrtf(dx * dx + dy * dy + dz * dz) * inv_extent);
        cnt += __float_as_int(R0.rec.w);
#ifndef SPR_KP_ABL_NOMFMA1
#pragma unroll
        for (int t = 0; t < NTC; ++t) acc[t] = __builtin_amdgcn_mfma_f32_16x16x4f32(w, R0.xv[t], acc[t], 0, 0, 0);
#else
#pragma unroll
        for (int t = 0; t < NTC; ++t) acc[t][0] += w * R0.xv[t];
#endif
      }
      wait_item(i + 1);
      R0 = ld_kstep(nslot, 0);
      if (i + NS < n_items) issue_ids(slot_off, ids_next);
      between();
      {
        const float dx = (R1.rec.x - qx) - kx, dy = (R1.rec.y - qy) - ky, dz = (R1.rec.z - qz) - kz;
        const float w = fmaxf(0.f, 1.f - __builtin_amdgcn_sqrtf(dx * dx + dy * dy + dz * dz) * inv_extent);
        cnt += __float_as_int(R1.rec.w);
#ifndef SPR_KP_ABL_NOMFMA1
#pragma unroll
        for (int t = 0; t < NTC; ++t) acc[t] = __builtin_amdgcn_mfma_f32_16x16x4f32(w, R1.xv[t], acc[t], 0, 0, 0);
#else
#pragma unroll
        for (int t = 0; t < NTC; ++t) acc[t][0] += w * R1.xv[t];
#endif
      }
      R1 = ld_kstep(nslot, 1);
      ids_next = load_ids(par, i + NS + 1);
      slot_off = nslot;
      ++i;
    };
    auto nothing = [] {};
    f32x4 accA[NTC], accB[NTC];
#pragma unroll
    for (int t = 0; t < NTC; ++t) accA[t] = accB[t] = (f32x4){0.f, 0.f, 0.f, 0.f};
    int cntA = 0, cntB = 0;
#pragma unroll 1
    for (int b = 0; b < d.z; ++b) item(accA, cntA, qax, qay, qaz, nothing);
    if (d.w > 0) {
      item(accB, cntB, qbx, qby, qbz, [&] { flush(accA, cntA, wave, d.x); });
#pragma unroll 1
      for (int b = 1; b < d.w; ++b) item(accB, cntB, qbx, qby, qbz, nothing);
      flush(accB, cntB, 15 - wave, d.y);
    } else if (d.z > 0) {
      flush(accA, cntA, wave, d.x);
    }
    KP_STAMP(3);
    if (lane == 0) {
      if (d.x < 0) lqid[par * kRingTQ + wave] = -1;
      if (d.y < 0) lqid[par * kRingTQ + 15 - wave] = -1;
    }
    if (sp == 0) flush_pending();
    if (tid == 0) ltile[1 + par] = drawn;
    if (has_nn) stage_idx(d_nn, par);
    if (has_nxt) prime(d_nxt, par ^ 1);
    KP_STAMP(4);
    asm volatile("s_waitcnt lgkmcnt(0)" ::: "memory");
    __builtin_amdgcn_s_barrier();
    KP_STAMP(5);

    f32x4 acc2 = {0.f, 0.f, 0.f, 0.f};
    {
      const _Float16* ah_row = wfh + p16 * SH + 8 * j4;
      const _Float16* al_row = wfl + p16 * SH + 8 * j4;
#ifdef SPR_KP_ABL_NOP2
      if (ntiles < 0)
#endif
#pragma unroll
      for (int k = 0; k < KSW; ++k) {
        const int ks = min(ks0 + k, KS - 1);
        const kh8 ah = *reinterpret_cast<const kh8*>(ah_row + 32 * ks);
        const kh8 al = *reinterpret_cast<const kh8*>(al_row + 32 * ks);
        acc2 = __builtin_amdgcn_mfma_f32_16x16x32_f16(ah, bl[k], acc2, 0, 0, 0);
        acc2 = __builtin_amdgcn_mfma_f32_16x16x32_f16(al, bh[k], acc2, 0, 0, 0);
        acc2 = __builtin_amdgcn_mfma_f32_16x16x32_f16(ah, bh[k], acc2, 0, 0, 0);
      }
    }
    if (sp > 0) {
#pragma unroll
      for (int r = 0; r < 4; ++r) red[((ng * (SPLIT - 1) + sp - 1) * 4 + r) * 64 + lane] = acc2[r];
    }
    KP_STAMP(6);
    asm volatile("s_waitcnt lgkmcnt(0)" ::: "memory");
    __builtin_amdgcn_s_barrier();
    KP_STAMP(7);
    if (sp == 0) {
#pragma unroll
      for (int s2 = 1; s2 < SPLIT; ++s2)
#pragma unroll
        for (int r = 0; r < 4; ++r) acc2[r] += red[((ng * (SPLIT - 1) + s2 - 1) * 4 + r) * 64 + lane];
#pragma unroll
      for (int r = 0; r < 4; ++r) {
        const int ql = 4 * j4 + r;
        pend_n[r] = lqid[par * kRingTQ + ql];
        const float inv = unscale / (float)max(lcnt[par * kRingTQ + ql], 1);
        pend_v[r] = acc2[r] * inv;
      }
    }
    KP_STAMP(8);
    d_cur = d_nxt;
    d_nxt = d_nn;
    tile = tile_nxt;
    tile_nxt = tile_nn;
    tile_nn = __builtin_amdgcn_readfirstlane(ltile[1 + par]);
  }
  if (sp == 0) flush_pending();
  asm volatile("s_waitcnt vmcnt(0)" ::: "memory");
#ifdef SPR_KP_RING_PROF
  if (blockIdx.x == 0) {
    asm volatile("s_waitcnt lgkmcnt(0)" ::: "memory");
    for (int k = lane; k < kTraceN; k += 64) g_kp_trace[wave * kTraceN + k] = k < trace_n ? trace_lds[wave * kTraceN + k] : 0ull;
  }
#endif
}

template <int CC, int COUT, int NS>
int launch_ring(const float* q_xyz, int nq, int ns, const int* nbr, int nbr_stride, int kmax, const float* x,
                const _Float16* Wh, const _Float16* Wl, const float* kpts, float inv_extent, const float4* sxf,
                const int4* desc, const int* pad_word, const float* x_parts, const float* w_parts, int n_xparts,
                int n_wparts, int* tile_ctr, float* out, hipStream_t stream) {
  typedef RingShape<CC, COUT, NS> S;
  const int idxw = kmax <= 64 ? 64 : 128;
#ifdef SPR_KP_RING_PROF
  const size_t lds = S::lds_bytes(idxw) + 8 * kTraceN * 8;
#else
  const size_t lds = S::lds_bytes(idxw);
#endif
  auto kern = k_kpconv_ring<CC, COUT, NS>;
  ProfScope prof(stream, CC * 100000 + COUT, nq);
  if (lds > 64 * 1024)
    if (int rc = ensure_dyn_lds((const void*)kern, 160 * 1024)) return rc;
  const int ntiles = cdiv(nq, kRingTQ);
  const int n_cu = device_cu_count();
  int per_cu = (int)((160 * 1024) / lds);
  per_cu = per_cu < 1 ? 1 : (per_cu > S::MINW / 2 ? S::MINW / 2 : per_cu);
  const int grid = ntiles < n_cu * per_cu ? ntiles : n_cu * per_cu;
  hipLaunchKernelGGL(kern, dim3(grid), dim3(512), lds, stream, q_xyz, ns, nbr, nbr_stride, kmax, x, Wh, Wl, kpts,
                     inv_extent, sxf, desc, ntiles, pad_word, idxw, x_parts, w_parts, n_xparts, n_wparts, tile_ctr, out);
  SPR_LAUNCH_CHECK();
  return 0;
}

}

void launch_rowflag(const float* x, const float* s_xyz, int ns, int cin, unsigned char* flag, float4* sxf,
                    int* tile_ctr, hipStream_t stream) {
  const int c4 = cin >> 2;
  const bool wide = (cin & 3) == 0 && c4 <= 64 && (c4 & (c4 - 1)) == 0;
  const long waves = wide ? cdiv(ns, (64 / c4) * 4) : (long)ns;
  hipLaunchKernelGGL(k_rowflag, dim3(cdiv(waves * 64, 256)), dim3(256), 0, stream, x, s_xyz, ns, cin, flag, sxf, tile_ctr);
}
}

using namespace spr;

#ifdef SPR_KP_RING_PROF
extern "C" int spr_debug_kp_trace(unsigned long long* out, int n) {
  if (hipDeviceSynchronize() != hipSuccess) return 1;
  if (hipMemcpyFromSymbol(out, HIP_SYMBOL(g_kp_trace), sizeof(unsigned long long) * n) != hipSuccess) return 1;
  return 0;
}
#endif

static inline size_t plan_desc_bytes(int nq) { return align_up((size_t)cdiv(nq > 0 ? nq : 1, kRingTQ) * 8 * sizeof(int4), 256); }
static inline int w_chunk(int cin) { return cin % 64 == 0 ? 64 : 32; }
static inline bool ring_shape(int cin, int cout) {
  return (cin == 32 || cin == 64) && cin * cout <= 4096 && cout % 32 == 0 && 8 % (cout / 16) == 0;
}

extern "C" size_t spr_kpconv_plan_bytes(int nq) { return plan_desc_bytes(nq) + 256; }

extern "C" int spr_kpconv_plan(const int* nbr, int nq, int ns, int nbr_stride, int kmax, int rows_sorted,
                               const int* order, void* plan, size_t plan_bytes, void* stream_) {
  hipStream_t stream = (hipStream_t)stream_;
  SPR_REQUIRE(nq > 0 && ns > 0 && kmax >= 1 && kmax <= nbr_stride, "kpconv plan: bad sizes");
  SPR_REQUIRE(plan != nullptr && plan_bytes >= spr_kpconv_plan_bytes(nq), "kpconv plan: buffer too small");
  const int ntiles = cdiv(nq, kRingTQ);
  int4* desc = (int4*)plan;
  int* pad_word = (int*)((char*)plan + plan_desc_bytes(nq));
  hipLaunchKernelGGL(k_kp_tiles, dim3(cdiv((long)ntiles * 64, 256)), dim3(256), 0, stream, nbr, nq, ns, nbr_stride,
                     kmax, rows_sorted, order, ntiles, desc, pad_word);
  SPR_LAUNCH_CHECK();
  return 0;
}

extern "C" size_t spr_kpconv_wplanes_bytes(int cin, int cout) { return 2 * align_up((size_t)32 * cin * cout * 2, 256); }

extern "C" int spr_kpconv_prep_weights(const float* weights, int n_kp, int cin, int cout, const float* w_range,
                                       int w_range_n, void* wplanes, size_t bytes, void* stream_) {
  hipStream_t stream = (hipStream_t)stream_;
  SPR_REQUIRE(n_kp == kKP && cin % 32 == 0 && cout % 32 == 0 && cout <= 256,
              "kpconv weight planes exist for the MFMA shapes only (15 kernel points, channels in multiples of 32)");
  SPR_REQUIRE(w_range != nullptr && w_range_n >= 1, "kpconv weight planes: the weight range is required");
  SPR_REQUIRE(wplanes != nullptr && bytes >= spr_kpconv_wplanes_bytes(cin, cout), "kpconv weight planes: buffer too small");
  _Float16* wh = (_Float16*)wplanes;
  _Float16* wl = (_Float16*)((char*)wplanes + align_up((size_t)32 * cin * cout * 2, 256));
  hipLaunchKernelGGL(k_w_prep, dim3(cdiv((long)n_kp * cin * cout, 256)), dim3(256), 0, stream, weights, cin, cout,
                     w_chunk(cin), w_range, w_range_n, wh, wl);
  SPR_LAUNCH_CHECK();
  return 0;
}

extern "C" size_t spr_kpconv_workspace_bytes(int nq, int ns, int cin, int cout) {
  const size_t n = (size_t)(ns > 0 ? ns : 1);
  return align_up(n, 256) + align_up(16 * (n + 1), 256) + spr_kpconv_wplanes_bytes(cin, cout) +
         2 * align_up(kAmaxParts * sizeof(float), 256) + spr_kpconv_plan_bytes(nq) + 256;
}

extern "C" int spr_kpconv_fwd(const float* q_xyz, int nq, const float* s_xyz, int ns,
                              const int* nbr, int nbr_stride, int kmax, int rows_sorted,
                              const float* x, int cin, const float* weights, int cout,
                              const float* kernel_points, int n_kp, float kp_extent,
                              float* out, int impl, void* ws, size_t ws_bytes,
                              void* stream_) {
  return spr_kpconv_fwd_r(q_xyz, nq, s_xyz, ns, nbr, nbr_stride, kmax, rows_sorted, x, cin, weights, cout, kernel_points,
                          n_kp, kp_extent, out, impl, nullptr, 0, nullptr, 0, ws, ws_bytes, stream_);
}

extern "C" int spr_kpconv_fwd_r(const float* q_xyz, int nq, const float* s_xyz, int ns,
                                const int* nbr, int nbr_stride, int kmax, int rows_sorted,
                                const float* x, int cin, const float* weights, int cout,
                                const float* kernel_points, int n_kp, float kp_extent,
                                float* out, int impl, const float* x_range, int x_range_n, const float* w_range,
                                int w_range_n, void* ws, size_t ws_bytes, void* stream_) {
  return spr_kpconv_fwd_p(q_xyz, nq, s_xyz, ns, nbr, nbr_stride, kmax, rows_sorted, x, cin, weights, cout, kernel_points,
                          n_kp, kp_extent, out, impl, x_range, x_range_n, w_range, w_range_n, nullptr, nullptr, ws,
                          ws_bytes, stream_);
}

extern "C" int spr_kpconv_fwd_p(const float* q_xyz, int nq, const float* s_xyz, int ns,
                                const int* nbr, int nbr_stride, int kmax, int rows_sorted,
                                const float* x, int cin, const float* weights, int cout,
                                const float* kernel_points, int n_kp, float kp_extent,
                                float* out, int impl, const float* x_range, int x_range_n, const float* w_range,
                                int w_range_n, const void* plan, const void* wplanes, void* ws, size_t ws_bytes,
                                void* stream_) {
  hipStream_t stream = (hipStream_t)stream_;
  SPR_REQUIRE((x_range == nullptr || x_range_n >= 1) && (w_range == nullptr || w_range_n >= 1),
              "kpconv: a range needs a count");
  SPR_REQUIRE(nq > 0 && ns > 0, "kpconv: empty input");
  SPR_REQUIRE(kmax >= 1 && kmax <= nbr_stride, "kpconv: bad kmax=%d stride=%d", kmax, nbr_stride);
  SPR_REQUIRE(cin >= 1 && cout >= 1 && n_kp >= 1 && n_kp <= 32, "kpconv: bad dims");
  SPR_REQUIRE(kp_extent > 0.f, "kpconv: KP_extent must be > 0");
  SPR_REQUIRE(ws_bytes >= spr_kpconv_workspace_bytes(nq, ns, cin, cout), "kpconv: workspace too small");
  unsigned char* flag = (unsigned char*)ws;
  float4* sxf = (float4*)((char*)ws + align_up((size_t)ns, 256));
  _Float16* wh = (_Float16*)((char*)sxf + align_up(((size_t)ns + 1) * 16, 256));
  _Float16* wl = (_Float16*)((char*)wh + align_up((size_t)32 * cin * cout * 2, 256));
  float* x_parts = (float*)((char*)wl + align_up((size_t)32 * cin * cout * 2, 256));
  float* w_parts = x_parts + align_up(kAmaxParts * sizeof(float), 256) / sizeof(float);
  void* ws_plan = (char*)w_parts + align_up(kAmaxParts * sizeof(float), 256);
  int* tile_ctr = (int*)((char*)ws_plan + spr_kpconv_plan_bytes(nq));
  SPR_REQUIRE(wplanes == nullptr || w_range != nullptr, "kpconv: prepared weight planes come with the range they were scaled by");
  if (wplanes != nullptr) {
    wh = (_Float16*)wplanes;
    wl = (_Float16*)((char*)wplanes + align_up((size_t)32 * cin * cout * 2, 256));
  }
  const float inv_extent = 1.0f / kp_extent;

  if (cin == 1 && (impl == 0 || impl == 2) && n_kp <= 16) {
    hipLaunchKernelGGL(k_records_cin1, dim3(cdiv(ns, 256)), dim3(256), 0, stream, x, s_xyz, ns, sxf);
    ProfScope prof(stream, cin * 100000 + cout, nq);
    hipLaunchKernelGGL(k_kpconv_cin1, dim3(cdiv(nq, 64)), dim3(256), 0, stream, q_xyz, nq, s_xyz, ns, nbr,
                       nbr_stride, kmax, rows_sorted, sxf, weights, cout, kernel_points, n_kp, inv_extent, out);
    SPR_LAUNCH_CHECK();
    return 0;
  }

  launch_rowflag(x, s_xyz, ns, cin, flag, sxf, tile_ctr, stream);
  SPR_LAUNCH_CHECK();

  if ((impl == 0 || impl == 2) && n_kp == kKP && cin % 32 == 0 && cout % 32 == 0 && cout <= 256) {
    const int ktot = n_kp * cin;
    const float* xp = x_range != nullptr ? x_range : x_parts;
    const float* wp = w_range != nullptr ? w_range : w_parts;
    const int n_xp = x_range != nullptr ? x_range_n : kAmaxParts, n_wp = w_range != nullptr ? w_range_n : kAmaxParts;
    if (x_range == nullptr && w_range == nullptr) {
      if (int rc = launch_absmax2(x, ns, cin, cin, x_parts, weights, ktot, cout, cout, w_parts, stream)) return rc;
    } else if (x_range == nullptr) {
      if (int rc = launch_absmax(x, ns, cin, cin, x_parts, stream)) return rc;
    } else if (w_range == nullptr) {
      if (int rc = launch_absmax(weights, ktot, cout, cout, w_parts, stream)) return rc;
    }
    if (wplanes == nullptr)
      hipLaunchKernelGGL(k_w_prep, dim3(cdiv((long)ktot * cout, 256)), dim3(256), 0, stream, weights, cin, cout,
                         w_chunk(cin), wp, n_wp, wh, wl);
    const bool ring_ok = impl == 0 && ring_shape(cin, cout) && kmax <= 128 && (size_t)ns * cin * 4 < (1ull << 32) &&
                         (size_t)nq * nbr_stride * 4 < (1ull << 32);
    if (ring_ok) {
      if (plan == nullptr) {
        if (int rc = spr_kpconv_plan(nbr, nq, ns, nbr_stride, kmax, rows_sorted, nullptr, ws_plan,
                                     spr_kpconv_plan_bytes(nq), stream_)) return rc;
        plan = ws_plan;
      }
      const int4* desc = (const int4*)plan;
      const int* pad_word = (const int*)((const char*)plan + plan_desc_bytes(nq));
#define SPR_RING_ARGS                                                                                       \
  q_xyz, nq, ns, nbr, nbr_stride, kmax, x, wh, wl, kernel_points, inv_extent, sxf, desc, pad_word, xp, wp, \
      n_xp, n_wp, tile_ctr, out, stream
      if (cin == 64 && cout == 64) return launch_ring<64, 64, SPR_KP_NS64>(SPR_RING_ARGS);
      if (cin == 64 && cout == 32) return launch_ring<64, 32, 4>(SPR_RING_ARGS);
      if (cin == 32 && cout == 32) return launch_ring<32, 32, 3>(SPR_RING_ARGS);
      if (cin == 32 && cout == 64) return launch_ring<32, 64, 8>(SPR_RING_ARGS);
      if (cin == 32 && cout == 128) return launch_ring<32, 128, 8>(SPR_RING_ARGS);
#undef SPR_RING_ARGS
    }
#define SPR_KP_ARGS                                                                         \
  q_xyz, nq, s_xyz, ns, nbr, nbr_stride, kmax, rows_sorted, x, cin, wh, wl, cout,           \
      kernel_points, inv_extent, sxf, xp, wp, n_xp, n_wp, out, stream
    if (cin % 64 == 0) {
      if (cout == 64) return launch_mfma<64, 32, 1, 8, 2>(SPR_KP_ARGS);
      if (cout == 128) return launch_mfma<64, 32, 2, 8, 2>(SPR_KP_ARGS);
      if (cout == 256) return launch_mfma<64, 32, 4, 8, 2>(SPR_KP_ARGS);
    } else {
      if (cout == 32) return launch_mfma<32, 64, 1, 8, 1>(SPR_KP_ARGS);
      if (cout == 64) return launch_mfma<32, 64, 2, 8, 1>(SPR_KP_ARGS);
      if (cout == 128) return launch_mfma<32, 64, 4, 8, 1>(SPR_KP_ARGS);
    }
#undef SPR_KP_ARGS
  }
  const long total = (long)nq * cout;
  hipLaunchKernelGGL(k_kpconv_simple, dim3(cdiv(total, 256)), dim3(256), 0, stream, q_xyz, nq,
                     s_xyz, ns, nbr, nbr_stride, kmax, x, cin, weights, cout, kernel_points, n_kp,
                     inv_extent, flag, out);
  SPR_LAUNCH_CHECK();
  return 0;
}
```

### superpoints_registration_amd/csrc/spr_common.h

```cpp
#pragma once
#include <hip/hip_runtime.h>

#include <cstdarg>
#include <cstdio>
#include <cstdint>
#include <cstring>

#include "../../include/spr.h"

namespace spr {

constexpr int kWave = 64;

void set_error(const char* fmt, ...);

#define SPR_HIP_CHECK(expr)                                                   \
  do {                                                                        \
    hipError_t _e = (expr);                                                   \
    if (_e != hipSuccess) {                                                   \
      ::spr::set_error("%s failed: %s (%s:%d)", #expr, hipGetErrorString(_e), \
                       __FILE__, __LINE__);                                   \
      return 1;                                                               \
    }                                                                         \
  } while (0)

#define SPR_LAUNCH_CHECK()                                                  \
  do {                                                                      \
    hipError_t _e = hipGetLastError();                                      \
    if (_e != hipSuccess) {                                                 \
      ::spr::set_error("kernel launch failed: %s (%s:%d)",                  \
                       hipGetErrorString(_e), __FILE__, __LINE__);          \
      return 1;                                                             \
    }                                                                       \
  } while (0)

#define SPR_REQUIRE(cond, ...)        \
  do {                                \
    if (!(cond)) {                    \
      ::spr::set_error(__VA_ARGS__);  \
      return 2;                       \
    }                                 \
  } while (0)

static inline size_t align_up(size_t x, size_t a) { return (x + a - 1) / a * a; }
static inline int cdiv(long a, long b) { return (int)((a + b - 1) / b); }

struct Workspace {
  char* base;
  size_t size;
  size_t off;
  Workspace(void* p, size_t n) : base((char*)p), size(n), off(0) {}
  template <typename T>
  T* take(size_t count) {
    size_t bytes = align_up(count * sizeof(T), 256);
    if (off + bytes > size) return nullptr;
    T* r = (T*)(base + off);
    off += bytes;
    return r;
  }
};

bool prof_enabled();
void prof_push(hipEvent_t beg, hipEvent_t end, int code, int n);
struct ProfScope {
  hipStream_t stream;
  bool on;
  hipEvent_t beg, end;
  int code, n;
  ProfScope(hipStream_t s, int code_, int n_) : stream(s), on(prof_enabled()), code(code_), n(n_) {
    if (!on) return;
    if (hipEventCreate(&beg) != hipSuccess || hipEventCreate(&end) != hipSuccess) {
      on = false;
      return;
    }
    (void)hipEventRecord(beg, stream);
  }
  ~ProfScope() {
    if (!on) return;
    (void)hipEventRecord(end, stream);
    prof_push(beg, end, code, n);
  }
};

int ensure_dyn_lds(const void* kernel, int bytes);
int device_cu_count();

int launch_absmax(const float* x, long rows, int cols, long stride, float* parts, hipStream_t stream);
int launch_absmax2(const float* x0, long rows0, int cols0, long stride0, float* parts0, const float* x1,
                   long rows1, int cols1, long stride1, float* parts1, hipStream_t stream);

#ifdef __HIPCC__
typedef float f32x4 __attribute__((ext_vector_type(4)));
typedef float f32x16 __attribute__((ext_vector_type(16)));

__device__ __forceinline__ int find_segment(const int* __restrict__ cu, int nseg,
                                            int i) {
  int lo = 0, hi = nseg;
  while (hi - lo > 1) {
    int mid = (lo + hi) >> 1;
    if (cu[mid] <= i)
      lo = mid;
    else
      hi = mid;
  }
  return lo;
}

__device__ __forceinline__ int xcd_swizzle(int b, int nwg) {
  const int q = nwg >> 3, r = nwg & 7;
  const int xcd = b & 7, idx = b >> 3;
  const int base = (xcd < r) ? xcd * (q + 1) : r * (q + 1) + (xcd - r) * q;
  return base + idx;
}

typedef _Float16 spr_h16x2 __attribute__((ext_vector_type(2)));
__device__ __forceinline__ void split_pk(float a, float b, unsigned int& hi_u, unsigned int& lo_u) {
  const spr_h16x2 hi = {(_Float16)a, (_Float16)b};
  hi_u = __builtin_bit_cast(unsigned int, hi);
  asm("v_fma_mixlo_f16 %0, %1, -1.0, %2 op_sel_hi:[1,0,0]\n\t"
      "v_fma_mixhi_f16 %0, %1, -1.0, %3 op_sel:[1,0,0] op_sel_hi:[1,0,0]"
      : "=&v"(lo_u)
      : "v"(hi_u), "v"(a), "v"(b));
}

__device__ __forceinline__ void split_pk_s(float a, float b, float s, unsigned int& hi_u,
                                           unsigned int& lo_u) {
  asm("v_fma_mixlo_f16 %0, %1, %3, 0 op_sel_hi:[0,0,0]\n\t"
      "v_fma_mixhi_f16 %0, %2, %3, 0 op_sel_hi:[0,0,0]"
      : "=&v"(hi_u)
      : "v"(a), "v"(b), "v"(s));
  asm("v_fma_mixlo_f16 %0, %2, %4, -%1 op_sel_hi:[0,0,1]\n\t"
      "v_fma_mixhi_f16 %0, %3, %4, -%1 op_sel:[0,0,1] op_sel_hi:[0,0,1]"
      : "=&v"(lo_u)
      : "v"(hi_u), "v"(a), "v"(b), "v"(s));
}

__device__ __forceinline__ void split_pk_s_hi(float a, float b, float s, unsigned int& hi_u) {
  asm("v_fma_mixlo_f16 %0, %1, %3, 0 op_sel_hi:[0,0,0]\n\t"
      "v_fma_mixhi_f16 %0, %2, %3, 0 op_sel_hi:[0,0,0]"
      : "=&v"(hi_u)
      : "v"(a), "v"(b), "v"(s));
}
__device__ __forceinline__ void split_pk_s_lo(float a, float b, float s, unsigned int hi_u, unsigned int& lo_u) {
  asm("v_fma_mixlo_f16 %0, %2, %4, -%1 op_sel_hi:[0,0,1]\n\t"
      "v_fma_mixhi_f16 %0, %3, %4, -%1 op_sel:[0,0,1] op_sel_hi:[0,0,1]"
      : "=&v"(lo_u)
      : "v"(hi_u), "v"(a), "v"(b), "v"(s));
}

__host__ __device__ __forceinline__ int pow2_exp_for(float amax) {
  if (!(amax > 0.f) || !(amax < 3.0e38f)) return 0;
  unsigned int u;
#ifdef __HIP_DEVICE_COMPILE__
  u = __float_as_uint(amax);
#else
  memcpy(&u, &amax, 4);
#endif
  const int e = (int)((u >> 23) & 0xff) - 127;
  int k = 14 - e;
  if (k > 60) k = 60;
  if (k < -60) k = -60;
  return k;
}
__host__ __device__ __forceinline__ float pow2f(int k) {
  const unsigned int u = (unsigned int)(127 + k) << 23;
  float f;
#ifdef __HIP_DEVICE_COMPILE__
  f = __uint_as_float(u);
#else
  memcpy(&f, &u, 4);
#endif
  return f;
}

constexpr int kAmaxParts = 512;
constexpr int kRangeSlots = 64;
__device__ __forceinline__ float block_absmax(const float* __restrict__ parts, float* sh, int n = kAmaxParts) {
  float m = 0.f;
  for (int i = threadIdx.x; i < n; i += blockDim.x) m = fmaxf(m, parts[i]);
#pragma unroll
  for (int o = 32; o > 0; o >>= 1) m = fmaxf(m, __shfl_xor(m, o, 64));
  if ((threadIdx.x & 63) == 0) sh[threadIdx.x >> 6] = m;
  __syncthreads();
  if (threadIdx.x == 0) {
    float t = sh[0];
    for (int w = 1; w < (int)(blockDim.x >> 6); ++w) t = fmaxf(t, sh[w]);
    sh[16] = t;
  }
  __syncthreads();
  return sh[16];
}

__device__ __forceinline__ float wave_sum(float v) {
#pragma unroll
  for (int o = 32; o > 0; o >>= 1) v += __shfl_xor(v, o, 64);
  return v;
}
__device__ __forceinline__ double wave_sum_d(double v) {
#pragma unroll
  for (int o = 32; o > 0; o >>= 1) v += __shfl_xor(v, o, 64);
  return v;
}
__device__ __forceinline__ float wave_max(float v) {
#pragma unroll
  for (int o = 32; o > 0; o >>= 1) v = fmaxf(v, __shfl_xor(v, o, 64));
  return v;
}
#endif

}
```

### superpoints_registration_amd/ops.py

```python
import ctypes
import math
import threading
from typing import Optional, Sequence, Tuple

import numpy as np
import torch

from . import _lib

ACT_NONE, ACT_RELU, ACT_SIGMOID = 0, 1, 2
ORDER_REFERENCE, ORDER_CANONICAL = 0, 1


def _stream(t: torch.Tensor):
    return ctypes.c_void_p(torch.cuda.current_stream(t.device).cuda_stream)


def _ptr(t: Optional[torch.Tensor]):
    return None if t is None else ctypes.c_void_p(t.data_ptr())


def _dev(t: torch.Tensor, name: str, dtype=None) -> torch.Tensor:
    if not isinstance(t, torch.Tensor) or not t.is_cuda:
        raise RuntimeError(f"{name} must be a tensor on the MI355X device (got "
                           f"{t.device if isinstance(t, torch.Tensor) else type(t)}); "
                           "the HIP path has no CPU fallback")
    if dtype is not None and t.dtype != dtype:
        t = t.to(dtype)
    return t.contiguous()


_ws_cache = {}


_range_epoch = [0]


def invalidate_ranges() -> None:
    _range_epoch[0] += 1


def _set_range(t: torch.Tensor, parts: torch.Tensor, n: int, guard=None) -> None:
    if n > 0:
        t._spr_range = (parts, int(n), t._version, t.data_ptr(), _range_epoch[0], guard)


def _get_range(t):
    r = getattr(t, '_spr_range', None)
    if r is None or r[2] != t._version or r[3] != t.data_ptr() or r[4] != _range_epoch[0]:
        return None, 0
    if r[5] is not None:
        r[5].acquire()
    return r[0], r[1]

_RANGE_CAP = 4096
_STREAM_SLOTS = 512
_zero_pool = {}


def _zero_slots(n: int, device) -> torch.Tensor:
    key = (device, torch.cuda.current_stream(device).cuda_stream)
    pool = _zero_pool.get(key)
    if pool is None or pool[1] + n > pool[0].numel():
        pool = [torch.zeros(1 << 18, dtype=torch.float32, device=device), 0]
        _zero_pool[key] = pool
    out = pool[0][pool[1]:pool[1] + n]
    pool[1] += n
    return out


class _StreamGuard:

    def __init__(self, buf: torch.Tensor):
        self.stream = torch.cuda.current_stream(buf.device)
        self.event = torch.cuda.Event()
        self.event.record(self.stream)
        self.buf = buf
        self.seen = {self.stream.cuda_stream}

    def acquire(self):
        cur = torch.cuda.current_stream(self.buf.device)
        if cur.cuda_stream not in self.seen:
            cur.wait_event(self.event)
            self.buf.record_stream(cur)
            self.seen.add(cur.cuda_stream)


def _static_range(w: torch.Tensor):
    r, n = _get_range(w)
    if r is not None:
        return r, n
    L = _lib.lib()
    n = L.spr_range_parts()
    flat = w.reshape(-1, w.shape[-1])
    parts = torch.empty((n,), dtype=torch.float32, device=w.device)
    _lib.check(L.spr_absmax(_ptr(flat), flat.shape[0], flat.shape[1], flat.shape[1], _ptr(parts), _stream(w)),
               "spr_absmax")
    _set_range(w, parts, n, _StreamGuard(parts))
    return parts, n


_PRIME_PARTS = 16


def prime_weight_ranges(params) -> int:
    todo = [p for p in params if isinstance(p, torch.Tensor) and p.is_cuda and p.dtype == torch.float32
            and p.dim() >= 2 and p.is_contiguous() and p.numel() > 0 and _get_range(p)[0] is None]
    if not todo:
        return 0
    dev = todo[0].device
    todo = [p for p in todo if p.device == dev]
    rec = np.zeros((len(todo), 2), dtype=np.int64)
    for i, p in enumerate(todo):
        rec[i, 0] = p.data_ptr()
        rec[i, 1] = p.numel()
    jobs = torch.from_numpy(rec).to(dev)
    parts = torch.empty((len(todo), _PRIME_PARTS), dtype=torch.float32, device=dev)
    _lib.check(_lib.lib().spr_absmax_multi(_ptr(jobs), len(todo), _PRIME_PARTS, _ptr(parts), _stream(parts)),
               "spr_absmax_multi")
    guard = _StreamGuard(parts)
    for i, p in enumerate(todo):
        _set_range(p, parts[i], _PRIME_PARTS, guard)
    return len(todo)


def weight_transposed(w: torch.Tensor) -> torch.Tensor:
    c = getattr(w, '_spr_wt', None)
    if c is not None and c[1] == w._version and c[2] == w.data_ptr() and c[3] == _range_epoch[0]:
        c[4].acquire()
        return c[0]
    wt = w.detach().t().contiguous()
    r, n = _static_range(w)
    if r is not None:
        rw = getattr(w, '_spr_range', None)
        _set_range(wt, r, n, rw[5] if rw is not None else None)
    w._spr_wt = (wt, w._version, w.data_ptr(), _range_epoch[0], _StreamGuard(wt))
    return wt


def ensure_range(t: torch.Tensor) -> torch.Tensor:
    if t.dim() != 2 or not t.is_contiguous() or _get_range(t)[0] is not None:
        return t
    L = _lib.lib()
    n = L.spr_range_parts()
    parts = torch.empty((n,), dtype=torch.float32, device=t.device)
    _lib.check(L.spr_absmax(_ptr(t), t.shape[0], t.shape[1], t.shape[1], _ptr(parts), _stream(t)), "spr_absmax")
    _set_range(t, parts, n)
    return t


def _workspace(nbytes: int, device) -> torch.Tensor:
    key = (device, torch.cuda.current_stream(device).cuda_stream)
    buf = _ws_cache.get(key)
    if buf is None or buf.numel() < nbytes:
        buf = torch.empty(max(int(nbytes), 1 << 20), dtype=torch.uint8, device=device)
        _ws_cache[key] = buf
    return buf


def lengths_to_cu(lengths, device) -> torch.Tensor:
    if isinstance(lengths, torch.Tensor):
        l = lengths.to(device=device, dtype=torch.int32)
        cu = torch.zeros(l.numel() + 1, dtype=torch.int32, device=device)
        cu[1:] = torch.cumsum(l, 0)
        return cu
    arr = np.zeros(len(lengths) + 1, dtype=np.int32)
    arr[1:] = np.cumsum(np.asarray(lengths, dtype=np.int64))
    return torch.from_numpy(arr).to(device)


def selftest() -> None:
    st = ctypes.c_int(-1)
    _lib.check(_lib.lib().spr_selftest(ctypes.byref(st)), "spr_selftest")


def grid_subsample(points: torch.Tensor, cu: torch.Tensor, dl: float, max_p: int = 0,
                   order: int = ORDER_REFERENCE) -> Tuple[torch.Tensor, torch.Tensor]:
    points = _dev(points, "points", torch.float32)
    cu = _dev(cu, "cu", torch.int32)
    n, nb = points.shape[0], cu.numel() - 1
    L = _lib.lib()
    ws = _workspace(L.spr_grid_subsample_workspace_bytes(n, nb), points.device)
    out = torch.empty((max(n, 1), 3), dtype=torch.float32, device=points.device)
    out_lens = torch.empty((nb,), dtype=torch.int32, device=points.device)
    total = torch.empty((1,), dtype=torch.int32, device=points.device)
    _lib.check(L.spr_grid_subsample(_ptr(points), _ptr(cu), n, nb, float(dl), int(max_p), int(order),
                                    _ptr(out), _ptr(out_lens), _ptr(total), _ptr(ws), ws.numel(),
                                    _stream(points)), "spr_grid_subsample")
    m = int(total.item())
    if m < 0:
        raise RuntimeError("spr_grid_subsample: voxel grid too large for 40-bit keys")
    return out[:m], out_lens


def voxel_downsample(points: torch.Tensor, voxel_size: float) -> torch.Tensor:
    points = _dev(points, "points", torch.float32)
    n = points.shape[0]
    L = _lib.lib()
    ws = _workspace(L.spr_voxel_downsample_workspace_bytes(n), points.device)
    idx = torch.empty((n,), dtype=torch.int32, device=points.device)
    cnt = torch.empty((1,), dtype=torch.int32, device=points.device)
    _lib.check(L.spr_voxel_downsample(_ptr(points), n, float(voxel_size), _ptr(idx), _ptr(cnt), _ptr(ws), ws.numel(),
                                      _stream(points)), "spr_voxel_downsample")
    m = int(cnt.item())
    if m < 0:
        raise RuntimeError("spr_voxel_downsample: coordinates exceed 2^20 voxels")
    return points[idx[:m].long()]


def radius_neighbors(queries: torch.Tensor, supports: torch.Tensor, q_cu: torch.Tensor,
                     s_cu: torch.Tensor, radius: float, limit: int,
                     exact_width: bool = True, algo: int = 0) -> Tuple[torch.Tensor, int]:
    queries = _dev(queries, "queries", torch.float32)
    supports = _dev(supports, "supports", torch.float32)
    q_cu = _dev(q_cu, "q_cu", torch.int32)
    s_cu = _dev(s_cu, "s_cu", torch.int32)
    nq, ns, nb = queries.shape[0], supports.shape[0], q_cu.numel() - 1
    L = _lib.lib()
    ws = _workspace(L.spr_radius_neighbors_workspace_bytes(nq, ns, nb), queries.device)
    out = torch.empty((nq, limit), dtype=torch.int32, device=queries.device)
    mc = torch.empty((1,), dtype=torch.int32, device=queries.device)
    _lib.check(L.spr_radius_neighbors(_ptr(queries), _ptr(q_cu), nq, _ptr(supports), _ptr(s_cu), ns,
                                      nb, float(radius), int(limit), int(algo), _ptr(out), _ptr(mc),
                                      _ptr(ws), ws.numel(), _stream(queries)), "spr_radius_neighbors")
    if not exact_width:
        return out, -1
    m = int(mc.item())
    if m == -2 and algo == 0:
        return radius_neighbors(queries, supports, q_cu, s_cu, radius, limit, exact_width, algo=1)
    if m < 0:
        raise RuntimeError("spr_radius_neighbors: cloud extent / radius exceeds 8191 cells per axis")
    if m < 1:
        raise RuntimeError("Error")
    return out[:, :min(m, limit)], m


class RadiusTable:

    def __init__(self, supports: torch.Tensor, s_cu: torch.Tensor, radius: float):
        self.supports = _dev(supports, "supports", torch.float32)
        self.s_cu = _dev(s_cu, "s_cu", torch.int32)
        self.radius = float(radius)
        self.ns, self.nb = self.supports.shape[0], self.s_cu.numel() - 1
        L = _lib.lib()
        self.blob = torch.empty((L.spr_radius_table_bytes(self.ns, self.nb),), dtype=torch.uint8, device=supports.device)
        ws = _workspace(L.spr_radius_table_build_workspace_bytes(self.ns, self.nb), supports.device)
        _lib.check(L.spr_radius_table_build(_ptr(self.supports), _ptr(self.s_cu), self.ns, self.nb, self.radius,
                                            _ptr(self.blob), self.blob.numel(), _ptr(ws), ws.numel(),
                                            _stream(self.supports)), "spr_radius_table_build")
        self._slot = 0
        self._slots = L.spr_radius_table_slots()
        self._versions = (self.supports._version, self.s_cu._version)

    def matches(self, supports: torch.Tensor, s_cu: torch.Tensor, radius: float) -> bool:
        return (supports.data_ptr() == self.supports.data_ptr() and supports.shape[0] == self.ns
                and s_cu.data_ptr() == self.s_cu.data_ptr() and float(radius) == self.radius
                and (self.supports._version, self.s_cu._version) == self._versions
                and supports._version == self.supports._version and s_cu._version == self.s_cu._version
                and self._slot < self._slots)

    def query(self, queries: torch.Tensor, q_cu: torch.Tensor, limit: int,
              dense: Optional[bool] = None) -> Tuple[torch.Tensor, int]:
        queries = _dev(queries, "queries", torch.float32)
        q_cu = _dev(q_cu, "q_cu", torch.int32)
        nq = queries.shape[0]
        self_search = int(queries.data_ptr() == self.supports.data_ptr() and nq == self.ns
                          and q_cu.data_ptr() == self.s_cu.data_ptr())
        L = _lib.lib()
        ws = _workspace(L.spr_radius_table_query_workspace_bytes(nq), queries.device)
        out = torch.empty((nq, limit), dtype=torch.int32, device=queries.device)
        mc = torch.empty((1,), dtype=torch.int32, device=queries.device)
        slot, self._slot = self._slot, self._slot + 1
        if dense is None:
            _lib.check(L.spr_radius_table_query(_ptr(queries), _ptr(q_cu), nq, self_search, self.ns, self.nb, self.radius,
                                                int(limit), slot, _ptr(self.blob), _ptr(out), _ptr(mc), _ptr(ws),
                                                ws.numel(), _stream(queries)), "spr_radius_table_query")
        else:
            _lib.check(L.spr_radius_table_query_a(_ptr(queries), _ptr(q_cu), nq, self_search, self.ns, self.nb,
                                                  self.radius, int(limit), slot, _ptr(self.blob), _ptr(out), _ptr(mc),
                                                  1 if dense else 0, _ptr(ws), ws.numel(), _stream(queries)),
                       "spr_radius_table_query_a")
        m = int(mc.item())
        if m == -2:
            return radius_neighbors(queries, self.supports, q_cu, self.s_cu, self.radius, limit, True, algo=1)
        if m < 0:
            raise RuntimeError("spr_radius_neighbors: cloud extent / radius exceeds 8191 cells per axis")
        if m < 1:
            raise RuntimeError("Error")
        return out[:, :min(m, limit)], m


def _wants_grad(*tensors) -> bool:
    return torch.is_grad_enabled() and any(isinstance(t, torch.Tensor) and t.requires_grad for t in tensors)


def kpconv(q_pts, s_pts, nbr, x, weights, kernel_points, kp_extent: float, rows_sorted: bool = False,
           impl: int = 0) -> torch.Tensor:
    if _wants_grad(x, weights):
        from .autograd import KPConvFn
        return KPConvFn.apply(_dev(q_pts, "q_pts", torch.float32), _dev(s_pts, "s_pts", torch.float32), nbr,
                              _dev(x, "x", torch.float32), weights, kernel_points, float(kp_extent),
                              bool(rows_sorted), int(impl))
    return kpconv_raw(q_pts, s_pts, nbr, x, weights, kernel_points, kp_extent, rows_sorted, impl)


def kpconv_raw(q_pts, s_pts, nbr, x, weights, kernel_points, kp_extent: float, rows_sorted: bool = False,
               impl: int = 0, order: Optional[torch.Tensor] = None) -> torch.Tensor:
    q_pts = _dev(q_pts, "q_pts", torch.float32)
    s_pts = _dev(s_pts, "s_pts", torch.float32)
    x = _dev(x, "x", torch.float32)
    weights = _dev(weights, "weights", torch.float32)
    kernel_points = _dev(kernel_points, "kernel_points", torch.float32)
    if not nbr.is_cuda:
        raise RuntimeError("neighb_inds must be on the device")
    if nbr.dtype != torch.int32:
        nbr = nbr.to(torch.int32)
    stride = nbr.stride(0) if nbr.stride(1) == 1 and nbr.shape[1] > 0 else None
    if stride is None:
        nbr = nbr.contiguous()
        stride = nbr.shape[1]
    nq, ns, kmax = q_pts.shape[0], s_pts.shape[0], nbr.shape[1]
    n_kp, cin, cout = weights.shape
    assert x.shape == (ns, cin), (x.shape, ns, cin)
    L = _lib.lib()
    ws = _workspace(L.spr_kpconv_workspace_bytes(nq, ns, cin, cout), x.device)
    out = torch.empty((nq, cout), dtype=torch.float32, device=x.device)
    xr, xr_n = _get_range(x)
    wr, wr_n = _static_range(weights)
    plan = wplanes = None
    if impl == 0 and n_kp == 15 and cin % 32 == 0 and cout % 32 == 0 and cout <= 256:
        if cin in (32, 64) and cin * cout <= 4096 and kmax <= 128:
            plan = _kpconv_plan(nbr, nq, ns, int(stride), kmax, bool(rows_sorted), order)
        if wr is not None:
            wplanes = _kpconv_wplanes(weights, wr, wr_n)
    _lib.check(L.spr_kpconv_fwd_p(_ptr(q_pts), nq, _ptr(s_pts), ns, _ptr(nbr), int(stride), kmax,
                                  int(bool(rows_sorted)), _ptr(x), cin, _ptr(weights), cout,
                                  _ptr(kernel_points), n_kp, float(kp_extent), _ptr(out), int(impl),
                                  _ptr(xr), int(xr_n), _ptr(wr), int(wr_n), _ptr(plan), _ptr(wplanes),
                                  _ptr(ws), ws.numel(), _stream(x)), "spr_kpconv_fwd_p")
    return out


def _kpconv_plan(nbr: torch.Tensor, nq: int, ns: int, stride: int, kmax: int, rows_sorted: bool,
                 order: Optional[torch.Tensor] = None) -> torch.Tensor:
    if order is not None:
        order = _dev(order, "order", torch.int32)
        assert order.shape == (nq,)
    key = (nbr.data_ptr(), nbr._version, nq, ns, stride, kmax, rows_sorted, _range_epoch[0],
           None if order is None else (order.data_ptr(), order._version))
    c = getattr(nbr, '_spr_kp_plan', None)
    if c is not None and c[0] == key:
        c[2].acquire()
        return c[1]
    L = _lib.lib()
    nbytes = L.spr_kpconv_plan_bytes(nq)
    plan = torch.empty((nbytes,), dtype=torch.uint8, device=nbr.device)
    _lib.check(L.spr_kpconv_plan(_ptr(nbr), nq, ns, stride, kmax, int(rows_sorted), _ptr(order), _ptr(plan), nbytes,
                                 _stream(nbr)), "spr_kpconv_plan")
    nbr._spr_kp_plan = (key, plan, _StreamGuard(plan))
    return plan


def kpconv_plan_prefetch(nbr: torch.Tensor, ns: int, rows_sorted: bool = True) -> None:
    if nbr is None or not nbr.is_cuda or nbr.dtype != torch.int32 or nbr.dim() != 2 or nbr.shape[1] < 1:
        return
    if nbr.stride(1) != 1 or nbr.shape[1] > 128 or nbr.shape[0] < 1:
        return
    _kpconv_plan(nbr, nbr.shape[0], int(ns), int(nbr.stride(0)), nbr.shape[1], bool(rows_sorted))


def _kpconv_wplanes(weights: torch.Tensor, wr: torch.Tensor, wr_n: int) -> torch.Tensor:
    key = (weights.data_ptr(), weights._version, wr.data_ptr(), _range_epoch[0])
    c = getattr(weights, '_spr_kp_wplanes', None)
    if c is not None and c[0] == key:
        c[2].acquire()
        return c[1]
    L = _lib.lib()
    n_kp, cin, cout = weights.shape
    nbytes = L.spr_kpconv_wplanes_bytes(cin, cout)
    planes = torch.empty((nbytes,), dtype=torch.uint8, device=weights.device)
    _lib.check(L.spr_kpconv_prep_weights(_ptr(weights), n_kp, cin, cout, _ptr(wr), int(wr_n), _ptr(planes), nbytes,
                                         _stream(weights)), "spr_kpconv_prep_weights")
    weights._spr_kp_wplanes = (key, planes, _StreamGuard(planes))
    return planes


def instnorm(x, cu, eps: float = 1e-5, norm: bool = True, add=None, slope: float = 1.0,
             out=None, max_len: Optional[int] = None) -> torch.Tensor:
    if _wants_grad(x, add):
        from .autograd import InstNormFn
        return InstNormFn.apply(_dev(x, "x", torch.float32), _dev(cu, "cu", torch.int32), float(eps), bool(norm),
                                None if add is None else _dev(add, "add", torch.float32), float(slope), max_len)
    return instnorm_raw(x, cu, eps, norm, add, slope, out, max_len)


def instnorm_raw(x, cu, eps: float = 1e-5, norm: bool = True, add=None, slope: float = 1.0,
                 out=None, max_len: Optional[int] = None) -> torch.Tensor:
    x = _dev(x, "x", torch.float32)
    cu = _dev(cu, "cu", torch.int32)
    n, c = x.shape
    nb = cu.numel() - 1
    if add is not None:
        add = _dev(add, "add", torch.float32)
        assert add.shape == x.shape
    if out is None:
        out = torch.empty_like(x)
    L = _lib.lib()
    max_len = n if max_len is None else max(1, min(int(max_len), n))
    ws = _workspace(L.spr_instnorm_workspace_bytes(max_len, nb, c), x.device)
    cnt = _STREAM_SLOTS
    rng = _zero_slots(cnt, x.device)
    _lib.check(L.spr_instnorm_r(_ptr(x), _ptr(cu), n, nb, max_len, c, float(eps), int(bool(norm)), _ptr(add),
                                float(slope), _ptr(out), _ptr(rng), cnt, _ptr(ws), ws.numel(), _stream(x)),
               "spr_instnorm_r")
    if rng is not None:
        _set_range(out, rng, cnt)
    return out


def block_tail_tile_rows(ka: int, kb: int, n_out: int) -> int:
    if _modes["gemm"] != 1:
        return 0
    return int(_lib.lib().spr_block_tail_tile_rows(int(ka), int(kb), int(n_out)))


def _tail_tiles(cu: torch.Tensor, n: int, tr: int) -> torch.Tensor:
    key = (cu.data_ptr(), cu._version, n, tr, _range_epoch[0])
    cache = getattr(cu, '_spr_tail_tiles', None)
    if cache is None:
        cache = {}
        cu._spr_tail_tiles = cache
    c = cache.get(tr)
    if c is not None and c[0] == key:
        c[2].acquire()
        return c[1]
    L = _lib.lib()
    t = torch.empty((L.spr_block_tail_tiles_len(n, cu.numel() - 1, tr),), dtype=torch.int32, device=cu.device)
    _lib.check(L.spr_block_tail_tiles(_ptr(cu), n, cu.numel() - 1, tr, _ptr(t), _stream(cu)), "spr_block_tail_tiles")
    cache[tr] = (key, t, _StreamGuard(t))
    return t


def instnorm_stats(x, cu, eps: float = 1e-5, max_len: Optional[int] = None):
    x = _dev(x, "x", torch.float32)
    cu = _dev(cu, "cu", torch.int32)
    n, c = x.shape
    nb = cu.numel() - 1
    L = _lib.lib()
    max_len = n if max_len is None else max(1, min(int(max_len), n))
    ws = _workspace(L.spr_instnorm_workspace_bytes(max_len, nb, c), x.device)
    st = torch.empty((2, nb, c), dtype=torch.float32, device=x.device)
    _lib.check(L.spr_instnorm_stats(_ptr(x), _ptr(cu), n, nb, max_len, c, float(eps), _ptr(st[0]), _ptr(st[1]),
                                    _ptr(ws), ws.numel(), _stream(x)), "spr_instnorm_stats")
    return st[0], st[1]


_NORM_BOUNDS = {}


def _norm_bound(max_len: int, device) -> torch.Tensor:
    key = (int(max_len), str(device))
    t = _NORM_BOUNDS.get(key)
    if t is None:
        t = torch.full((1,), float(max(1, int(max_len))) ** 0.5, dtype=torch.float32, device=device)
        _NORM_BOUNDS[key] = t
    return t


def block_tail(xa, wa, cu, xb=None, wb=None, add=None, eps: float = 1e-5, slope: float = 0.1,
               xa_stats=None, xa_slope: float = 0.1, xa_max_len: Optional[int] = None) -> torch.Tensor:
    xa = _dev(xa, "xa", torch.float32)
    wa = _dev(wa, "wa", torch.float32)
    cu = _dev(cu, "cu", torch.int32)
    n, ka = xa.shape
    n_out = wa.shape[0]
    assert wa.shape[1] == ka
    kb = 0
    if xb is not None:
        xb = _dev(xb, "xb", torch.float32)
        wb = _dev(wb, "wb", torch.float32)
        kb = xb.shape[1]
        assert xb.shape[0] == n and wb.shape == (n_out, kb) and add is None
    if add is not None:
        add = _dev(add, "add", torch.float32)
        assert add.shape == (n, n_out)
    nb = cu.numel() - 1
    L = _lib.lib()
    tr = L.spr_block_tail_tile_rows(ka, kb, n_out)
    if tr <= 0:
        raise RuntimeError(f"block_tail: no kernel for ka={ka} kb={kb} n_out={n_out}")
    tiles = _tail_tiles(cu, n, tr)
    out = torch.empty((n, n_out), dtype=torch.float32, device=xa.device)
    ws = _workspace(L.spr_block_tail_workspace_bytes(n, nb, kb, n_out, tr), xa.device)
    if xa_stats is not None:
        xar, xar_n = _norm_bound(n if xa_max_len is None else xa_max_len, xa.device), 1
    else:
        xar, xar_n = _get_range(xa)
    war, war_n = _static_range(wa)
    xbr, xbr_n, wbr, wbr_n = None, 0, None, 0
    if kb > 0:
        xbr, xbr_n = _get_range(xb)
        wbr, wbr_n = _static_range(wb)
    cnt = _STREAM_SLOTS
    rng = _zero_slots(cnt, xa.device)
    if xa_stats is not None:
        mean, rstd = xa_stats
        assert mean.shape == (nb, ka) and rstd.shape == (nb, ka) and mean.is_contiguous() and rstd.is_contiguous()
        _lib.check(L.spr_block_tail_n(_ptr(xa), ka, _ptr(wa), _ptr(xb), kb, _ptr(wb), _ptr(add), _ptr(cu), _ptr(tiles),
                                      n, nb, n_out, float(eps), float(slope), _ptr(out), _ptr(xar), int(xar_n),
                                      _ptr(war), int(war_n), _ptr(xbr), int(xbr_n), _ptr(wbr), int(wbr_n),
                                      _ptr(rng), cnt, _ptr(mean), _ptr(rstd), float(xa_slope), _ptr(ws), ws.numel(),
                                      _stream(xa)), "spr_block_tail_n")
    else:
        _lib.check(L.spr_block_tail(_ptr(xa), ka, _ptr(wa), _ptr(xb), kb, _ptr(wb), _ptr(add), _ptr(cu), _ptr(tiles),
                                    n, nb, n_out, float(eps), float(slope), _ptr(out), _ptr(xar), int(xar_n),
                                    _ptr(war), int(war_n), _ptr(xbr), int(xbr_n), _ptr(wbr), int(wbr_n),
                                    _ptr(rng), cnt, _ptr(ws), ws.numel(), _stream(xa)), "spr_block_tail")
    if rng is not None:
        _set_range(out, rng, cnt)
    return out


def cell_order(points: torch.Tensor, cu: torch.Tensor, cell: float) -> torch.Tensor:
    points = _dev(points, "points", torch.float32)
    cu = _dev(cu, "cu", torch.int32)
    n, nb = points.shape[0], cu.numel() - 1
    L = _lib.lib()
    out = torch.empty((n,), dtype=torch.int32, device=points.device)
    ws = _workspace(L.spr_cell_order_workspace_bytes(n), points.device)
    _lib.check(L.spr_cell_order(_ptr(points), _ptr(cu), n, nb, float(cell), _ptr(out), _ptr(ws), ws.numel(),
                                _stream(points)), "spr_cell_order")
    return out


def maxpool(x, idx, order=None) -> torch.Tensor:
    if _wants_grad(x):
        from .autograd import MaxPoolFn
        return MaxPoolFn.apply(_dev(x, "x", torch.float32), idx)
    return maxpool_raw(x, idx, order)


def maxpool_raw(x, idx, order=None) -> torch.Tensor:
    x = _dev(x, "x", torch.float32)
    if idx.dtype != torch.int32:
        idx = idx.to(torch.int32)
    stride = idx.stride(0) if idx.stride(1) == 1 else None
    if stride is None:
        idx = idx.contiguous()
        stride = idx.shape[1]
    ns, c = x.shape
    nq, k = idx.shape
    out = torch.empty((nq, c), dtype=torch.float32, device=x.device)
    L = _lib.lib()
    cnt = _STREAM_SLOTS
    rng = _zero_slots(cnt, x.device)
    if order is not None:
        if order.dtype != torch.int32 or order.numel() != nq or not order.is_contiguous():
            raise ValueError("maxpool: order must be a contiguous int32 permutation of the query rows")
        _lib.check(L.spr_maxpool_gather_o(_ptr(x), ns, c, _ptr(idx), nq, int(stride), k, _ptr(order), _ptr(out),
                                          _ptr(rng), cnt, _stream(x)), "spr_maxpool_gather_o")
    else:
        _lib.check(L.spr_maxpool_gather_r(_ptr(x), ns, c, _ptr(idx), nq, int(stride), k, _ptr(out), _ptr(rng), cnt,
                                          _stream(x)), "spr_maxpool_gather_r")
    if rng is not None:
        _set_range(out, rng, cnt)
    return out


def linear(x, weight, bias=None, residual=None, act: int = ACT_NONE) -> torch.Tensor:
    if _wants_grad(x, weight, bias, residual):
        from .autograd import LinearFn
        return LinearFn.apply(_dev(x, "x", torch.float32), weight, bias, residual, int(act))
    return linear_raw(x, weight, bias, residual, act)


def linear_raw(x, weight, bias=None, residual=None, act: int = ACT_NONE) -> torch.Tensor:
    x = _dev(x, "x", torch.float32)
    weight = _dev(weight, "weight", torch.float32)
    m, k = x.shape
    n = weight.shape[0]
    assert weight.shape[1] == k
    if bias is not None:
        bias = _dev(bias, "bias", torch.float32)
    if residual is not None:
        residual = _dev(residual, "residual", torch.float32)
        assert residual.shape == (m, n)
    out = torch.empty((m, n), dtype=torch.float32, device=x.device)
    L = _lib.lib()
    ws = _workspace(L.spr_linear_workspace_bytes(), x.device)
    xr, xr_n = _get_range(x)
    wr, wr_n = _static_range(weight)
    orng = torch.empty((_RANGE_CAP,), dtype=torch.float32, device=x.device) if residual is None else None
    on = ctypes.c_int(0)
    _lib.check(L.spr_linear_r(_ptr(x), m, k, _ptr(weight), n, _ptr(bias), _ptr(residual), int(act), _ptr(out),
                              _ptr(xr), int(xr_n), _ptr(wr), int(wr_n), _ptr(orng),
                              _RANGE_CAP if orng is not None else 0, ctypes.byref(on),
                              _ptr(ws), ws.numel(), _stream(x)), "spr_linear_r")
    if orng is not None:
        _set_range(out, orng, on.value)
    return out


DEFAULT_ATTN_MODE = 4

_modes = {"gemm": 1, "attn": DEFAULT_ATTN_MODE}


def set_gemm_mode(mode: int) -> None:
    _lib.check(_lib.lib().spr_set_gemm_mode(int(mode)), "spr_set_gemm_mode")
    _modes["gemm"] = int(mode)


def layernorm(x, gamma, beta, eps: float = 1e-5, pos=None, want_norm: bool = True):
    if _wants_grad(x, gamma, beta):
        from .autograd import LayerNormFn
        n, p = LayerNormFn.apply(_dev(x, "x", torch.float32), gamma, beta, float(eps), pos, bool(want_norm))
        return (n if (want_norm or pos is None) else None), (p if pos is not None else None)
    return layernorm_raw(x, gamma, beta, eps, pos, want_norm)


def layernorm_raw(x, gamma, beta, eps: float = 1e-5, pos=None, want_norm: bool = True):
    x = _dev(x, "x", torch.float32)
    m, c = x.shape
    out_norm = torch.empty_like(x) if want_norm else None
    out_pos = None
    if pos is not None:
        pos = _dev(pos, "pos", torch.float32)
        out_pos = torch.empty_like(x)
    L = _lib.lib()
    cnt = L.spr_layernorm_range_count(m)
    rn = _zero_slots(cnt, x.device) if out_norm is not None else None
    rp = _zero_slots(cnt, x.device) if out_pos is not None else None
    _lib.check(L.spr_layernorm_r(_ptr(x), m, c, _ptr(_dev(gamma, "gamma", torch.float32)),
                                 _ptr(_dev(beta, "beta", torch.float32)), float(eps), _ptr(pos),
                                 _ptr(out_norm), _ptr(out_pos), _ptr(rn), _ptr(rp), _stream(x)), "spr_layernorm_r")
    if out_norm is not None:
        _set_range(out_norm, rn, cnt)
    if out_pos is not None:
        _set_range(out_pos, rp, cnt)
    return out_norm, out_pos


def posemb_sine(xyz, d_model: int, scale: float = 1.0, temperature: float = 10000.0) -> torch.Tensor:
    xyz = _dev(xyz, "xyz", torch.float32)
    n = xyz.shape[0]
    out = torch.empty((n, d_model), dtype=torch.float32, device=xyz.device)
    _lib.check(_lib.lib().spr_posemb_sine(_ptr(xyz), n, d_model, float(scale * 2 * math.pi),
                                          float(temperature), _ptr(out), _stream(xyz)),
               "spr_posemb_sine")
    return out


def attention(q, k, v, cu, kv_seg, max_len: int, nhead: int, out=None, lens_host=None,
              kv_seg_host=None) -> torch.Tensor:
    if _wants_grad(q, k, v):
        from .autograd import AttentionFn
        if lens_host is None:
            c = cu.cpu().tolist()
            lens_host = [c[i + 1] - c[i] for i in range(len(c) - 1)]
        if kv_seg_host is None:
            kv_seg_host = kv_seg.cpu().tolist()
        return AttentionFn.apply(q, k, v, _dev(cu, "cu", torch.int32), _dev(kv_seg, "kv_seg", torch.int32),
                                 int(max_len), int(nhead), list(lens_host), list(kv_seg_host))
    return attention_raw(q, k, v, cu, kv_seg, max_len, nhead, out)


def attention_raw(q, k, v, cu, kv_seg, max_len: int, nhead: int, out=None, want_lse: bool = False):
    for t, nm in ((q, "q"), (k, "k"), (v, "v")):
        if not t.is_cuda or t.dtype != torch.float32 or t.stride(1) != 1:
            raise RuntimeError(f"attention: {nm} must be a float32 device tensor with unit inner stride")
    T, d = q.shape
    hd = d // nhead
    cu = _dev(cu, "cu", torch.int32)
    kv_seg = _dev(kv_seg, "kv_seg", torch.int32)
    nseg = cu.numel() - 1
    if out is None:
        out = torch.empty((T, d), dtype=torch.float32, device=q.device)
    L = _lib.lib()
    ws = _workspace(L.spr_attn_workspace_bytes(T, nseg, nhead, hd), q.device)
    if want_lse:
        lse = torch.empty((T, nhead), dtype=torch.float32, device=q.device)
        written = ctypes.c_int(0)
        _lib.check(L.spr_attn_varlen_fwd_lse(_ptr(q), q.stride(0), _ptr(k), k.stride(0), _ptr(v), v.stride(0),
                                             _ptr(cu), _ptr(kv_seg), T, nseg, int(max_len), nhead, hd,
                                             1.0 / math.sqrt(hd), _ptr(out), out.stride(0), _ptr(lse),
                                             ctypes.byref(written), _ptr(ws), ws.numel(), _stream(q)),
                   "spr_attn_varlen_fwd_lse")
        return out, (lse if written.value else None)
    _lib.check(L.spr_attn_varlen_fwd(_ptr(q), q.stride(0), _ptr(k), k.stride(0), _ptr(v), v.stride(0),
                                     _ptr(cu), _ptr(kv_seg), T, nseg, int(max_len), nhead, hd,
                                     1.0 / math.sqrt(hd), _ptr(out), out.stride(0), _ptr(ws), ws.numel(),
                                     _stream(q)), "spr_attn_varlen_fwd")
    return out


def attention_probs(q, k, cu, kv_seg, max_len: int, nhead: int, average: bool = True, out=None, place=None,
                    max_rows: Optional[int] = None, max_cols: Optional[int] = None) -> torch.Tensor:
    for t, nm in ((q, "q"), (k, "k")):
        if not isinstance(t, torch.Tensor) or not t.is_cuda:
            raise RuntimeError(f"attention_probs: {nm} must be a tensor on the MI355X device; the HIP path has no "
                               "CPU fallback")
        if t.dtype != torch.float32 or t.stride(1) != 1:
            raise RuntimeError(f"attention_probs: {nm} must be float32 with unit inner stride")
    q, k = q.detach(), k.detach()
    T, d = q.shape
    hd = d // nhead
    cu = _dev(cu, "cu", torch.int32)
    kv_seg = _dev(kv_seg, "kv_seg", torch.int32)
    nseg = cu.numel() - 1
    L = int(max_len)
    if out is None:
        if place is not None:
            raise RuntimeError("attention_probs: `place` needs `out`")
        shape = (nseg, L, L) if average else (nseg, nhead, L, L)
        out = torch.empty(shape, dtype=torch.float32, device=q.device)
        per = L * L * (1 if average else nhead)
        pl = np.zeros((nseg, 5), dtype=np.int64)
        pl[:, 0] = np.arange(nseg, dtype=np.int64) * per
        pl[:, 1], pl[:, 2], pl[:, 3], pl[:, 4] = L, L * L, L, L
        place, max_rows, max_cols = pl, L, L
    else:
        if not out.is_cuda or out.dtype != torch.float32 or not out.is_contiguous():
            raise RuntimeError("attention_probs: out must be a contiguous float32 device tensor")
        if place is None:
            raise RuntimeError("attention_probs: `out` needs `place`")
    if isinstance(place, np.ndarray) or (isinstance(place, torch.Tensor) and not place.is_cuda):
        pl = np.asarray(place.cpu().numpy() if isinstance(place, torch.Tensor) else place, dtype=np.int64)
        if pl.shape != (nseg, 5):
            raise RuntimeError(f"attention_probs: place must be [nseg={nseg}, 5] (got {pl.shape})")
        nh = 1 if average else nhead
        last = pl[:, 0] + (nh - 1) * pl[:, 2] + (pl[:, 3] - 1) * pl[:, 1] + pl[:, 4]
        if (pl[:, 0] < 0).any() or (pl[:, 3] < 1).any() or (pl[:, 4] < 1).any() or (pl[:, 4] > pl[:, 1]).any() \
                or int(last.max()) > out.numel():
            raise RuntimeError("attention_probs: place describes entries outside `out`")
        max_rows, max_cols = int(pl[:, 3].max()), int(pl[:, 4].max())
        place = torch.from_numpy(pl).to(q.device)
    elif max_rows is None or max_cols is None:
        raise RuntimeError("attention_probs: a device `place` needs max_rows and max_cols")
    Lb = _lib.lib()
    ws = _workspace(Lb.spr_attn_probs_workspace_bytes(T, nhead, hd), q.device)
    _lib.check(Lb.spr_attn_probs(_ptr(q), q.stride(0), _ptr(k), k.stride(0), _ptr(cu), _ptr(kv_seg), T, nseg, L,
                                 nhead, hd, 1.0 / math.sqrt(hd), 0 if average else 1, _ptr(out), _ptr(place),
                                 int(max_rows), int(max_cols), _ptr(ws), ws.numel(), _stream(q)), "spr_attn_probs")
    return out


_seg_perm_cache = {}


def _segment_perms(kv_seg_host, device):
    key = (tuple(int(x) for x in kv_seg_host), str(device))
    c = _seg_perm_cache.get(key)
    if c is None:
        kv = np.asarray(key[0], dtype=np.int32)
        inv = np.empty_like(kv)
        inv[kv] = np.arange(kv.size, dtype=np.int32)
        c = (torch.from_numpy(kv).to(device), torch.from_numpy(inv).to(device))
        _seg_perm_cache[key] = c
    return c


def attention_bwd(q, k, v, out, dout, cu, kv_seg_host, max_len: int, nhead: int, lse=None):
    for t, nm in ((q, "q"), (k, "k"), (v, "v"), (out, "out"), (dout, "dout")):
        if not t.is_cuda or t.dtype != torch.float32 or t.stride(1) != 1:
            raise RuntimeError(f"attention_bwd: {nm} must be a float32 device tensor with unit inner stride")
    T, d = q.shape
    hd = d // nhead
    cu = _dev(cu, "cu", torch.int32)
    nseg = cu.numel() - 1
    kv, inv = _segment_perms(kv_seg_host, q.device)
    dq = torch.empty((T, d), dtype=torch.float32, device=q.device)
    dk = torch.empty_like(dq)
    dv = torch.empty_like(dq)
    L = _lib.lib()
    ws = _workspace(L.spr_attn_bwd_workspace_bytes2(T, nseg, nhead), q.device)
    _lib.check(L.spr_attn_varlen_bwd_lse(_ptr(q), q.stride(0), _ptr(k), k.stride(0), _ptr(v), v.stride(0), _ptr(out),
                                         out.stride(0), _ptr(dout), dout.stride(0), _ptr(lse), _ptr(cu), _ptr(kv),
                                         _ptr(inv), T, nseg, int(max_len), nhead, hd, 1.0 / math.sqrt(hd), _ptr(dq),
                                         _ptr(dk), _ptr(dv), _ptr(ws), ws.numel(), _stream(q)), "spr_attn_varlen_bwd_lse")
    return dq, dk, dv


def inproj_prepare(w_in: torch.Tensor):
    r = getattr(w_in, '_spr_inproj', None)
    if r is not None and r[1] == w_in._version and r[2] == w_in.data_ptr() and r[3] == _range_epoch[0]:
        r[4].acquire()
        return r[0]
    L = _lib.lib()
    d = w_in.shape[1]
    buf = torch.empty((L.spr_range_parts() + 3 * d,), dtype=torch.float32, device=w_in.device)
    _lib.check(L.spr_attn_inproj_prepare(_ptr(w_in), d, _ptr(buf), _stream(w_in)), "spr_attn_inproj_prepare")
    w_in._spr_inproj = (buf, w_in._version, w_in.data_ptr(), _range_epoch[0], _StreamGuard(buf))
    return buf


def attention_inproj(x_qk, x_v, w_in, b_in, cu, kv_seg, max_len: int, nhead: int, w_prep=None) -> torch.Tensor:
    x_qk = _dev(x_qk, "x_qk", torch.float32)
    x_v = x_qk if x_v is x_qk else _dev(x_v, "x_v", torch.float32)
    w_in = _dev(w_in, "w_in", torch.float32)
    b_in = _dev(b_in, "b_in", torch.float32)
    T, d = x_qk.shape
    assert x_v.shape == (T, d) and w_in.shape == (3 * d, d) and b_in.shape == (3 * d,)
    hd = d // nhead
    cu = _dev(cu, "cu", torch.int32)
    kv_seg = _dev(kv_seg, "kv_seg", torch.int32)
    nseg = cu.numel() - 1
    out = torch.empty((T, d), dtype=torch.float32, device=x_qk.device)
    L = _lib.lib()
    ws = _workspace(L.spr_attn_inproj_workspace_bytes(T, nseg, nhead, hd), x_qk.device)
    fused = _modes["attn"] != 0 and _modes["gemm"] == 1 and T >= 256
    qr, qn = _get_range(x_qk) if fused else (None, 0)
    vr, vn = (qr, qn) if x_v is x_qk else (_get_range(x_v) if fused else (None, 0))
    orng = torch.empty((1,), dtype=torch.float32, device=x_qk.device) if fused else None
    _lib.check(L.spr_attn_inproj_varlen_fwd_r(_ptr(x_qk), _ptr(x_v), T, _ptr(w_in), _ptr(b_in), _ptr(cu),
                                              _ptr(kv_seg), nseg, int(max_len), nhead, hd, 1.0 / math.sqrt(hd),
                                              _ptr(out), out.stride(0), _ptr(qr), int(qn), _ptr(vr), int(vn),
                                              _ptr(orng), _ptr(w_prep if fused else None), _ptr(ws), ws.numel(),
                                              _stream(x_qk)),
               "spr_attn_inproj_varlen_fwd_r")
    if orng is not None:
        _set_range(out, orng, 1)
    return out


_xenc_lock = threading.Lock()
XENC_PTRS_PER_LAYER = 18


class XencPlan:

    def __init__(self, key, prepared, plan, keep):
        self.key, self.prepared, self.plan, self.keep = key, prepared, plan, keep

    def __deepcopy__(self, memo):
        return None

    def __reduce__(self):
        return (_no_plan, ())


def _no_plan():
    return None


def xenc_available() -> bool:
    return _modes["gemm"] == 1 and _modes["attn"] in (1, 2, 3, 4)


def xenc_prepare(layer_params, layer_eps, final, nhead: int, d_ff: int, pos_bound: float, cached=None) -> XencPlan:
    flat = [t for lp in layer_params for t in lp] + ([final[0], final[1]] if final is not None else [])
    key = (tuple((t.data_ptr(), t._version) for t in flat), tuple(float(e) for le in layer_eps for e in le),
           None if final is None else float(final[2]), int(nhead), int(d_ff), float(pos_bound), _range_epoch[0])
    if cached is not None and cached.key == key:
        return cached
    with _xenc_lock:
        L = _lib.lib()
        n_layers = len(layer_params)
        keep = [_dev(t.detach(), "parameter", torch.float32) for t in flat]
        per = XENC_PTRS_PER_LAYER
        assert all(len(lp) == per for lp in layer_params)
        ptrs = (ctypes.c_void_p * (n_layers * per))(*[t.data_ptr() for t in keep[:n_layers * per]])
        eps = (ctypes.c_float * (3 * n_layers))(*[float(e) for le in layer_eps for e in le])
        dev = keep[0].device
        nbytes = L.spr_xenc_prepared_bytes(n_layers, int(d_ff))
        if nbytes == 0:
            raise RuntimeError("xenc_prepare: unsupported stack shape")
        prepared = torch.empty((nbytes,), dtype=torch.uint8, device=dev)
        plan = ctypes.create_string_buffer(L.spr_xenc_plan_bytes())
        fg = keep[-2] if final is not None else None
        fb = keep[-1] if final is not None else None
        _lib.check(L.spr_xenc_prepare(ptrs, eps, n_layers, 256, int(nhead), int(d_ff), _ptr(fg), _ptr(fb),
                                      float(final[2]) if final is not None else 0.0, float(pos_bound),
                                      _ptr(prepared), nbytes, plan, len(plan), _stream(prepared)), "spr_xenc_prepare")
        return XencPlan(key, prepared, plan, keep)


def xenc_forward(plan: XencPlan, x, pos, cu, seg_self, seg_cross, max_len: int) -> torch.Tensor:
    x = _dev(x, "x", torch.float32)
    pos = _dev(pos, "pos", torch.float32)
    cu = _dev(cu, "cu", torch.int32)
    seg_self = _dev(seg_self, "seg_self", torch.int32)
    seg_cross = _dev(seg_cross, "seg_cross", torch.int32)
    T, d = x.shape
    assert d == 256 and pos.shape == (T, d)
    nseg = cu.numel() - 1
    out = torch.empty_like(x)
    L = _lib.lib()
    ws = _workspace(L.spr_xenc_workspace_bytes(T, nseg), x.device)
    plan.prepared.record_stream(torch.cuda.current_stream(x.device))
    _lib.check(L.spr_xenc_forward(plan.plan, _ptr(x), _ptr(pos), _ptr(cu), _ptr(seg_self), _ptr(seg_cross), T, nseg,
                                  int(max_len), _ptr(out), _ptr(ws), ws.numel(), _stream(x)), "spr_xenc_forward")
    return out


def set_attn_mode(mode: int) -> None:
    _lib.check(_lib.lib().spr_set_attn_mode(int(mode)), "spr_set_attn_mode")
    _modes["attn"] = int(mode)


def _cu_host_arr(cu_host: Sequence[int]):
    arr = (ctypes.c_int * len(cu_host))(*[int(v) for v in cu_host])
    return arr


def match_dualsoftmax(feat, cu, cu_host: Sequence[int], npairs: int):
    if _wants_grad(feat):
        from .autograd import MatchDualSoftmaxFn
        return MatchDualSoftmaxFn.apply(_dev(feat, "feat", torch.float32), _dev(cu, "cu", torch.int32),
                                        list(cu_host), int(npairs))
    return match_dualsoftmax_raw(feat, cu, cu_host, npairs)


def match_dualsoftmax_top2(feat, cu, cu_host: Sequence[int], npairs: int):
    feat = _dev(feat, "feat", torch.float32)
    cu = _dev(cu, "cu", torch.int32)
    T, d = feat.shape
    arr = _cu_host_arr(cu_host)
    L = _lib.lib()
    ws = _workspace(L.spr_match_workspace_bytes(arr, npairs), feat.device)
    val = torch.zeros((T,), dtype=torch.float32, device=feat.device)
    val2 = torch.zeros((T,), dtype=torch.float32, device=feat.device)
    ind = torch.zeros((T,), dtype=torch.int32, device=feat.device)
    _lib.check(L.spr_match_dualsoftmax2(_ptr(feat), d, _ptr(cu), arr, npairs, _ptr(val), _ptr(val2), _ptr(ind),
                                        _ptr(ws), ws.numel(), _stream(feat)), "spr_match_dualsoftmax2")
    return val, val2, ind


def pose_residuals(pose, a, b, pair_cu) -> torch.Tensor:
    a, b = _dev(a, "a", torch.float32), _dev(b, "b", torch.float32)
    pose = _dev(pose, "pose", torch.float32)
    pair_cu = _dev(pair_cu, "pair_cu", torch.int32)
    n = a.shape[0]
    res = torch.empty((n,), dtype=torch.float32, device=a.device)
    _lib.check(_lib.lib().spr_pose_residuals(_ptr(pose), _ptr(a), _ptr(b), _ptr(pair_cu), pair_cu.numel() - 1, n,
                                             _ptr(res), _stream(a)), "spr_pose_residuals")
    return res


def pose_scores(poses, a, b) -> torch.Tensor:
    a, b = _dev(a, "a", torch.float32), _dev(b, "b", torch.float32)
    poses = _dev(poses, "poses", torch.float32)
    h = poses.shape[0]
    out = torch.empty((h,), dtype=torch.float32, device=a.device)
    _lib.check(_lib.lib().spr_pose_scores(_ptr(poses), h, _ptr(a), _ptr(b), a.shape[0], _ptr(out), _stream(a)),
               "spr_pose_scores")
    return out


def match_dualsoftmax_raw(feat, cu, cu_host: Sequence[int], npairs: int):
    feat = _dev(feat, "feat", torch.float32)
    cu = _dev(cu, "cu", torch.int32)
    T, d = feat.shape
    arr = _cu_host_arr(cu_host)
    L = _lib.lib()
    ws = _workspace(L.spr_match_workspace_bytes(arr, npairs), feat.device)
    val = torch.zeros((T,), dtype=torch.float32, device=feat.device)
    ind = torch.zeros((T,), dtype=torch.int32, device=feat.device)
    _lib.check(L.spr_match_dualsoftmax(_ptr(feat), d, _ptr(cu), arr, npairs, _ptr(val), _ptr(ind),
                                       _ptr(ws), ws.numel(), _stream(feat)), "spr_match_dualsoftmax")
    return val, ind


def _dev_scalar(v, device) -> torch.Tensor:
    if isinstance(v, torch.Tensor):
        return v.detach().to(device=device, dtype=torch.float32).reshape(1).contiguous()
    return torch.tensor([float(v)], dtype=torch.float32, device=device)


def sinkhorn_correspondences(feat, xyz, cu, cu_host: Sequence[int], npairs: int, alpha,
                             beta, n_iters: int, slack: bool = True):
    if _wants_grad(feat, alpha, beta):
        from .autograd import SinkhornFn
        dev = feat.device
        a = alpha if isinstance(alpha, torch.Tensor) else torch.tensor(float(alpha), device=dev)
        b = beta if isinstance(beta, torch.Tensor) else torch.tensor(float(beta), device=dev)
        return SinkhornFn.apply(_dev(feat, "feat", torch.float32), _dev(xyz, "xyz", torch.float32),
                                _dev(cu, "cu", torch.int32), list(cu_host), int(npairs), a, b, int(n_iters),
                                bool(slack))
    return sinkhorn_correspondences_raw(feat, xyz, cu, cu_host, npairs, alpha, beta, n_iters, slack)


def sinkhorn_correspondences_raw(feat, xyz, cu, cu_host: Sequence[int], npairs: int, alpha,
                                 beta, n_iters: int, slack: bool = True):
    feat = _dev(feat, "feat", torch.float32)
    alpha_t, beta_t = _dev_scalar(alpha, feat.device), _dev_scalar(beta, feat.device)
    xyz = _dev(xyz, "xyz", torch.float32)
    cu = _dev(cu, "cu", torch.int32)
    T, d = feat.shape
    tsrc = int(cu_host[npairs])
    arr = _cu_host_arr(cu_host)
    L = _lib.lib()
    ws = _workspace(L.spr_sinkhorn_workspace_bytes(arr, npairs), feat.device)
    w = torch.empty((tsrc,), dtype=torch.float32, device=feat.device)
    that = torch.empty((tsrc, 3), dtype=torch.float32, device=feat.device)
    _lib.check(L.spr_sinkhorn_correspondences(_ptr(feat), d, _ptr(xyz), _ptr(cu), arr, npairs,
                                              _ptr(alpha_t), _ptr(beta_t), int(n_iters), int(bool(slack)),
                                              _ptr(w), _ptr(that), _ptr(ws), ws.numel(), _stream(feat)),
               "spr_sinkhorn_correspondences")
    return w, that


def match_and_sinkhorn(feat, xyz, cu, cu_host: Sequence[int], npairs: int, alpha, beta, n_iters: int,
                       top2: bool = False):
    if _wants_grad(feat, alpha, beta):
        raise RuntimeError("match_and_sinkhorn is an inference operator (use match_dualsoftmax + sinkhorn_correspondences)")
    feat = _dev(feat, "feat", torch.float32)
    alpha_t, beta_t = _dev_scalar(alpha, feat.device), _dev_scalar(beta, feat.device)
    xyz = _dev(xyz, "xyz", torch.float32)
    cu = _dev(cu, "cu", torch.int32)
    T, d = feat.shape
    tsrc = int(cu_host[npairs])
    arr = _cu_host_arr(cu_host)
    L = _lib.lib()
    ws = _workspace(L.spr_match_workspace_bytes(arr, npairs), feat.device)
    val = torch.zeros((T,), dtype=torch.float32, device=feat.device)
    val2 = torch.zeros((T,), dtype=torch.float32, device=feat.device) if top2 else None
    ind = torch.zeros((T,), dtype=torch.int32, device=feat.device)
    w = torch.empty((tsrc,), dtype=torch.float32, device=feat.device)
    that = torch.empty((tsrc, 3), dtype=torch.float32, device=feat.device)
    _lib.check(L.spr_match_sinkhorn(_ptr(feat), d, _ptr(xyz), _ptr(cu), arr, npairs, _ptr(alpha_t), _ptr(beta_t),
                                    int(n_iters), _ptr(val), _ptr(val2), _ptr(ind), _ptr(w), _ptr(that), _ptr(ws),
                                    ws.numel(), _stream(feat)), "spr_match_sinkhorn")
    return val, val2, ind, w, that


def weighted_procrustes(a, b, w, pair_cu) -> torch.Tensor:
    if _wants_grad(a, b, w):
        from .autograd import ProcrustesFn
        return ProcrustesFn.apply(_dev(a, "a", torch.float32), _dev(b, "b", torch.float32),
                                  None if w is None else _dev(w, "w", torch.float32), _dev(pair_cu, "pair_cu", torch.int32))
    return weighted_procrustes_raw(a, b, w, pair_cu)


def weighted_procrustes_raw(a, b, w, pair_cu) -> torch.Tensor:
    a = _dev(a, "a", torch.float32)
    b = _dev(b, "b", torch.float32)
    if w is not None:
        w = _dev(w, "w", torch.float32)
    pair_cu = _dev(pair_cu, "pair_cu", torch.int32)
    p = pair_cu.numel() - 1
    out = torch.empty((p, 3, 4), dtype=torch.float32, device=a.device)
    _lib.check(_lib.lib().spr_weighted_procrustes(_ptr(a), _ptr(b), _ptr(w), _ptr(pair_cu), p,
                                                  _ptr(out), _stream(a)), "spr_weighted_procrustes")
    return out


def overlap_pool(ov_prev, pool_idx, ns_prev: int):
    ov_prev = _dev(ov_prev, "ov_prev", torch.float32)
    pool_idx = _dev(pool_idx, "pool_idx", torch.int32)
    nq, w = pool_idx.shape
    out = torch.empty((nq,), dtype=torch.float32, device=ov_prev.device)
    _lib.check(_lib.lib().spr_overlap_pool(_ptr(ov_prev), int(ns_prev), _ptr(pool_idx), pool_idx.stride(0), w,
                                           nq, _ptr(out), _stream(ov_prev)), "spr_overlap_pool")
    return out


def _loss_ws(n, m, d, device):
    return _workspace(_lib.lib().spr_loss_workspace_bytes(int(n), int(m), int(d)), device)


def bce_logits_mean(x, y):
    if _wants_grad(x):
        from .autograd import BCELogitsMeanFn
        return BCELogitsMeanFn.apply(_dev(x, "x", torch.float32), _dev(y, "y", torch.float32))
    return bce_logits_mean_raw(x, y)


def bce_logits_mean_raw(x, y):
    x = _dev(x, "x", torch.float32)
    y = _dev(y, "y", torch.float32)
    assert x.shape == y.shape and x.dim() == 1
    out = torch.empty((1,), dtype=torch.float32, device=x.device)
    ws = _loss_ws(x.numel(), 1, 32, x.device)
    _lib.check(_lib.lib().spr_bce_logits_mean(_ptr(x), _ptr(y), x.numel(), _ptr(out), _ptr(ws), ws.numel(),
                                              _stream(x)), "spr_bce_logits_mean")
    return out[0]


def infonce_pair(anchor_feat, positive_feat, anchor_xyz, pose_gt, positive_xyz, W, r_p: float, r_n: float):
    if _wants_grad(anchor_feat, positive_feat, W):
        from .autograd import InfoNCEFn
        return InfoNCEFn.apply(_dev(anchor_feat, "anchor_feat", torch.float32),
                               _dev(positive_feat, "positive_feat", torch.float32), anchor_xyz, pose_gt, positive_xyz,
                               W, float(r_p), float(r_n))
    return infonce_pair_raw(anchor_feat, positive_feat, anchor_xyz, pose_gt, positive_xyz, W, r_p, r_n)


def infonce_pair_raw(anchor_feat, positive_feat, anchor_xyz, pose_gt, positive_xyz, W, r_p: float, r_n: float):
    a = _dev(anchor_feat, "anchor_feat", torch.float32)
    p = _dev(positive_feat, "positive_feat", torch.float32)
    n, d = a.shape
    m = p.shape[0]
    out = torch.empty((1,), dtype=torch.float32, device=a.device)
    ws = _loss_ws(n, m, d, a.device)
    _lib.check(_lib.lib().spr_infonce_pair(_ptr(a), n, _ptr(p), m, d, _ptr(_dev(anchor_xyz, "anchor_xyz", torch.float32)),
                                           _ptr(_dev(pose_gt, "pose_gt", torch.float32)),
                                           _ptr(_dev(positive_xyz, "positive_xyz", torch.float32)),
                                           _ptr(_dev(W, "W", torch.float32)), float(r_p), float(r_n), _ptr(out),
                                           _ptr(ws), ws.numel(), _stream(a)), "spr_infonce_pair")
    return out[0]


def circle_loss(src_feat, tgt_feat, src_kp, pose_gt, tgt_kp, r_p: float, r_n: float):
    B = len(src_feat)
    if not (len(tgt_feat) == len(src_kp) == len(tgt_kp) == B >= 1):
        raise ValueError("circle_loss: src_feat, tgt_feat, src_kp and tgt_kp need one entry per pair")
    for name, ts in (("src_feat", src_feat), ("tgt_feat", tgt_feat), ("src_kp", src_kp), ("tgt_kp", tgt_kp)):
        for t in ts:
            _dev(t, name)
    src_lens = [int(t.shape[0]) for t in src_feat]
    tgt_lens = [int(t.shape[0]) for t in tgt_feat]
    cat = lambda ts: ts[0] if len(ts) == 1 else torch.cat(list(ts))
    return circle_loss_packed(cat(src_feat), cat(tgt_feat), cat(src_kp), pose_gt, cat(tgt_kp), src_lens, tgt_lens,
                              r_p, r_n)


def circle_loss_packed(src_feat, tgt_feat, src_kp, pose_gt, tgt_kp, src_lens, tgt_lens, r_p: float, r_n: float):
    if _wants_grad(src_feat, tgt_feat):
        from .autograd import CircleLossFn
        return CircleLossFn.apply(_dev(src_feat, "src_feat", torch.float32), _dev(tgt_feat, "tgt_feat", torch.float32),
                                  src_kp, pose_gt, tgt_kp, tuple(src_lens), tuple(tgt_lens), float(r_p), float(r_n))
    return circle_loss_raw(src_feat, tgt_feat, src_kp, pose_gt, tgt_kp, src_lens, tgt_lens, r_p, r_n)


def _circle_args(src_feat, tgt_feat, src_kp, pose_gt, tgt_kp, src_lens, tgt_lens):
    a = _dev(src_feat, "src_feat", torch.float32)
    b = _dev(tgt_feat, "tgt_feat", torch.float32)
    xa = _dev(src_kp, "src_kp", torch.float32)
    xb = _dev(tgt_kp, "tgt_kp", torch.float32)
    pose = _dev(pose_gt, "pose_gt", torch.float32)
    src_lens, tgt_lens = [int(n) for n in src_lens], [int(m) for m in tgt_lens]
    B = len(src_lens)
    d = a.shape[1] if a.dim() == 2 else -1
    if not (B >= 1 and len(tgt_lens) == B and min(src_lens) >= 1 and min(tgt_lens) >= 1):
        raise ValueError(f"circle_loss: every pair needs >= 1 row on both sides (got {src_lens}, {tgt_lens})")
    if a.shape != (sum(src_lens), d) or b.shape != (sum(tgt_lens), d) or d < 4 or d % 4:
        raise ValueError(f"circle_loss: features {tuple(a.shape)} / {tuple(b.shape)} do not match the lengths, "
                         "or D is not a multiple of 4")
    if xa.shape != (sum(src_lens), 3) or xb.shape != (sum(tgt_lens), 3) or pose.numel() != 12 * B:
        raise ValueError("circle_loss: keypoints or pose_gt do not match the lengths")
    return a, b, xa, pose, xb, src_lens, tgt_lens


def circle_loss_raw(src_feat, tgt_feat, src_kp, pose_gt, tgt_kp, src_lens, tgt_lens, r_p: float, r_n: float):
    a, b, xa, pose, xb, src_lens, tgt_lens = _circle_args(src_feat, tgt_feat, src_kp, pose_gt, tgt_kp, src_lens,
                                                          tgt_lens)
    B, max_n, max_m = len(src_lens), max(src_lens), max(tgt_lens)
    L = _lib.lib()
    out = torch.empty((B,), dtype=torch.float32, device=a.device)
    ws = _workspace(L.spr_circle_loss_workspace_bytes(B, max_n, max_m), a.device)
    cu_a, cu_b = lengths_to_cu(src_lens, a.device), lengths_to_cu(tgt_lens, a.device)
    _lib.check(L.spr_circle_loss(_ptr(a), _ptr(b), a.shape[1], _ptr(xa), _ptr(pose), _ptr(xb), _ptr(cu_a), _ptr(cu_b), B,
                                 max_n, max_m, float(r_p), float(r_n), _ptr(out), _ptr(ws), ws.numel(), _stream(a)),
               "spr_circle_loss")
    return out


def transform_l1_pair(pose_gt, pose_pred, xyz):
    if _wants_grad(pose_pred):
        from .autograd import TransformL1Fn
        return TransformL1Fn.apply(_dev(pose_gt, "pose_gt", torch.float32), pose_pred, _dev(xyz, "xyz", torch.float32))
    return transform_l1_pair_raw(pose_gt, pose_pred, xyz)


def transform_l1_pair_raw(pose_gt, pose_pred, xyz):
    xyz = _dev(xyz, "xyz", torch.float32)
    out = torch.empty((1,), dtype=torch.float32, device=xyz.device)
    ws = _loss_ws(xyz.shape[0], 1, 32, xyz.device)
    _lib.check(_lib.lib().spr_transform_l1_pair(_ptr(_dev(pose_gt, "pose_gt", torch.float32)),
                                                _ptr(_dev(pose_pred, "pose_pred", torch.float32)), _ptr(xyz),
                                                xyz.shape[0], _ptr(out), _ptr(ws), ws.numel(), _stream(xyz)),
               "spr_transform_l1_pair")
    return out[0]


def sum_scaled(values, scale: float = 1.0):
    values = _dev(values, "values", torch.float32)
    out = torch.empty((1,), dtype=torch.float32, device=values.device)
    _lib.check(_lib.lib().spr_sum_scaled(_ptr(values), values.numel(), float(scale), _ptr(out), _stream(values)),
               "spr_sum_scaled")
    return out[0]


def gather_rows(x, idx) -> torch.Tensor:
    if _wants_grad(x):
        from .autograd import GatherRowsFn
        return GatherRowsFn.apply(_dev(x, "x", torch.float32), _dev(idx, "idx", torch.int32))
    return gather_rows_raw(x, idx)


def gather_rows_raw(x, idx) -> torch.Tensor:
    x = _dev(x, "x", torch.float32)
    idx = _dev(idx, "idx", torch.int32)
    n_src, c = x.shape
    n = idx.numel()
    out = torch.empty((n, c), dtype=torch.float32, device=x.device)
    _lib.check(_lib.lib().spr_gather_rows(_ptr(x), n_src, c, _ptr(idx), n, _ptr(out), _stream(x)),
               "spr_gather_rows")
    return out
```

Baseline: 1236 pairs/s.

## Add pre-split f16 plane rows for 64x64 KPConv ring kernel

Adds a new ring KPConv kernel for cin=cout=64 that reads input features already split into high and low f16 planes, written once per source row by the rowflag pass. The kernel loads rows with direct global-to-LDS DMA and uses LDS transpose reads to feed MFMA, so gathered neighbour rows no longer need per-neighbour f32-to-f16 splitting. New entry points let callers build the planes once and reuse them across convolutions. The cost is a larger per-row buffer (4 bytes per channel in both cases, two f16 planes instead of one f32), more complex inline assembly, and LDS pressure.

```diff
diff --git a/include/spr.h b/include/spr.h
--- a/include/spr.h
+++ b/include/spr.h
@@ -111,6 +111,18 @@
                      float kp_extent, float* out, int impl, const float* x_range, int x_range_n,
                      const float* w_range, int w_range_n, const void* plan, const void* wplanes,
                      void* ws, size_t ws_bytes, void* stream);
+
+int spr_kpconv_plane_exp(float amax);
+int spr_kpconv_planes_supported(int cin, int cout);
+size_t spr_kpconv_sxf_bytes(int ns);
+int spr_kpconv_make_planes(const float* x, const float* s_xyz, int ns, int cin, int x_exp, void* planes,
+                           void* sxf, unsigned char* flag, void* stream);
+int spr_kpconv_fwd_planes(const float* q_xyz, int nq, const float* s_xyz, int ns, const int* nbr,
+                          int nbr_stride, int kmax, int rows_sorted, const void* x_planes, int x_exp,
+                          const void* sxf, int cin, const float* weights, int cout,
+                          const float* kernel_points, int n_kp, float kp_extent, float* out,
+                          const float* w_range, int w_range_n, const void* plan, const void* wplanes,
+                          void* ws, size_t ws_bytes, void* stream);
 int spr_instnorm_r(const float* x, const int* cu, int n, int nb, int max_len_host, int c,
                    float eps, int norm, const float* add, float slope, float* out,
                    float* out_range, int out_range_n, void* ws, size_t ws_bytes, void* stream);
diff --git a/superpoints_registration_amd/_lib.py b/superpoints_registration_amd/_lib.py
--- a/superpoints_registration_amd/_lib.py
+++ b/superpoints_registration_amd/_lib.py
@@ -47,6 +47,12 @@
     "spr_kpconv_prep_weights": (_i, [_vp, _i, _i, _i, _vp, _i, _vp, _sz, _vp]),
     "spr_kpconv_fwd_p": (_i, [_vp, _i, _vp, _i, _vp, _i, _i, _i, _vp, _i, _vp, _i, _vp, _i, _f, _vp,
                               _i, _vp, _i, _vp, _i, _vp, _vp, _vp, _sz, _vp]),
+    "spr_kpconv_plane_exp": (_i, [_f]),
+    "spr_kpconv_planes_supported": (_i, [_i, _i]),
+    "spr_kpconv_sxf_bytes": (_sz, [_i]),
+    "spr_kpconv_make_planes": (_i, [_vp, _vp, _i, _i, _i, _vp, _vp, _vp, _vp]),
+    "spr_kpconv_fwd_planes": (_i, [_vp, _i, _vp, _i, _vp, _i, _i, _i, _vp, _i, _vp, _i, _vp, _i, _vp, _i, _f, _vp,
+                                   _vp, _i, _vp, _vp, _vp, _sz, _vp]),
     "spr_instnorm_r": (_i, [_vp, _vp, _i, _i, _i, _i, _f, _i, _vp, _f, _vp, _vp, _i, _vp, _sz, _vp]),
     "spr_block_tail_tile_rows": (_i, [_i, _i, _i]),
     "spr_block_tail_tiles_len": (_sz, [_i, _i, _i]),
diff --git a/superpoints_registration_amd/csrc/kpconv.hip b/superpoints_registration_amd/csrc/kpconv.hip
--- a/superpoints_registration_amd/csrc/kpconv.hip
+++ b/superpoints_registration_amd/csrc/kpconv.hip
@@ -7,13 +7,20 @@
 
 __global__ __launch_bounds__(256) void k_rowflag(const float* __restrict__ x, const float* __restrict__ s_xyz,
                                                  int ns, int cin, unsigned char* __restrict__ flag,
-                                                 float4* __restrict__ sxf, int* __restrict__ tile_ctr) {
+                                                 float4* __restrict__ sxf, int* __restrict__ tile_ctr,
+                                                 unsigned char* __restrict__ planes,
+                                                 const float* __restrict__ x_parts, int n_xparts, int x_exp) {
   const int wid = (blockIdx.x * blockDim.x + threadIdx.x) >> 6;
   const int lane = threadIdx.x & 63;
   const int c4 = cin >> 2;
+  float ps = 0.f;
+  if (planes != nullptr) {
+    __shared__ float sh_amax[17];
+    ps = pow2f(n_xparts > 0 ? pow2_exp_for(block_absmax(x_parts, sh_amax, n_xparts)) : x_exp);
+  }
   if (blockIdx.x == 0 && threadIdx.x == 0) {
     sxf[ns] = make_float4(-1.0e17f, -1.0e17f, -1.0e17f, __int_as_float(0));
-    tile_ctr[0] = 0;
+    if (tile_ctr != nullptr) tile_ctr[0] = 0;
   }
   if ((cin & 3) == 0 && c4 <= 64 && (c4 & (c4 - 1)) == 0) {
     constexpr int kRfSteps = 4;
@@ -26,6 +33,19 @@
       const int row = row0 + r * rpl;
       v[r] = make_float4(0.f, 0.f, 0.f, 0.f);
       if (row < ns) v[r] = reinterpret_cast<const float4*>(x + (size_t)row * cin)[chunk];
+    }
+    if (planes != nullptr) {
+#pragma unroll
+      for (int r = 0; r < kRfSteps; ++r) {
+        const int row = row0 + r * rpl;
+        uint2 h, l;
+        plane_row_split4(v[r], ps, h, l);
+        if (row < ns) {
+          unsigned char* pr = planes + (size_t)row * cin * 4 + chunk * 8;
+          *reinterpret_cast<uint2*>(pr) = h;
+          *reinterpret_cast<uint2*>(pr + cin * 2) = l;
+        }
+      }
     }
 #pragma unroll
     for (int r = 0; r < kRfSteps; ++r) {
@@ -528,9 +548,6 @@
 
 
 constexpr int kRingTQ = 16;
-#ifndef SPR_KP_NS64
-#define SPR_KP_NS64 4
-#endif
 
 __global__ __launch_bounds__(256) void k_kp_tiles(const int* __restrict__ nbr, int nq, int ns, int nbr_stride,
                                                   int kmax, int rows_sorted, const int* __restrict__ order,
@@ -1076,14 +1093,387 @@
   return 0;
 }
 
-}
-
-void launch_rowflag(const float* x, const float* s_xyz, int ns, int cin, unsigned char* flag, float4* sxf,
-                    int* tile_ctr, hipStream_t stream) {
+constexpr int kInflExp = 12;
+
+template <int CC, int COUT>
+struct RingPShape {
+  static_assert(CC == 64, "plane-row phase 1: 64 input channels (256-byte rows)");
+  static constexpr int NB = CC / 16;
+  static constexpr int KW = kKP * CC;
+  static constexpr int SH = KW + 16;
+  static constexpr int KS = KW / 32;
+  static constexpr int NG = COUT / 16;
+  static constexpr int SPLIT = 8 / NG;
+  static constexpr int KSW = (KS + SPLIT - 1) / SPLIT;
+  static constexpr int RB = CC * 4;
+  static constexpr int SLOT = 8 * RB;
+  static constexpr int WF_BYTES = 2 * kRingTQ * SH * 2;
+  static constexpr int RED_BYTES = NG * (SPLIT - 1) * 4 * 64 * 4;
+  static constexpr int RING_BYTES = 8 * 4 * SLOT;
+  static constexpr int REC_BYTES = 8 * 2 * 4 * 128;
+  static constexpr int SMALL_BYTES = 2 * kRingTQ * 4 * 2 + 16;
+  static_assert(NG * SPLIT == 8 && WF_BYTES % 256 == 0 && RED_BYTES % 256 == 0, "shape");
+  static __host__ __device__ size_t lds_bytes(int idxw) {
+    return (size_t)WF_BYTES + RED_BYTES + RING_BYTES + REC_BYTES + SMALL_BYTES + (size_t)8 * 2 * 2 * idxw * 4;
+  }
+};
+
+typedef _Float16 kh4 __attribute__((ext_vector_type(4)));
+__device__ __forceinline__ kh4 tr_read_b64(unsigned addr) {
+  typedef __fp16 g4_t __attribute__((__vector_size__(4 * sizeof(__fp16))));
+  typedef __attribute__((address_space(3))) g4_t lds_g4_t;
+  return __builtin_bit_cast(kh4, __builtin_amdgcn_ds_read_tr16_b64_v4f16((lds_g4_t*)(uintptr_t)addr));
+}
+__device__ __forceinline__ void kstep_item_dma(const void* x, const void* sxf, unsigned off0, unsigned off1,
+                                               unsigned off_rec, unsigned dst_s, unsigned rec_s) {
+  asm volatile(
+      "s_mov_b32 m0, %5\n\ts_nop 0\n\t"
+      "global_load_lds_dwordx4 %0, %3\n\t"
+      "s_add_u32 m0, m0, 0x400\n\ts_nop 0\n\t"
+      "global_load_lds_dwordx4 %1, %3\n\t"
+      "s_mov_b64 exec, 0xff\n\ts_mov_b32 m0, %6\n\ts_nop 0\n\t"
+      "global_load_lds_dwordx4 %2, %4\n\t"
+      "s_mov_b64 exec, -1"
+      : : "v"(off0), "v"(off1), "v"(off_rec), "s"(x), "s"(sxf), "s"(dst_s), "s"(rec_s)
+      : "memory", "m0", "scc");
+}
+
+template <int CC, int COUT>
+__global__ __launch_bounds__(512, 2) void k_kpconv_ringp(
+    const float* __restrict__ q_xyz, int ns, const int* __restrict__ nbr, int nbr_stride, int kmax,
+    const unsigned char* __restrict__ xp, const _Float16* __restrict__ Wh, const _Float16* __restrict__ Wl,
+    const float* __restrict__ kpts, float inv_extent, const float4* __restrict__ sxf,
+    const int4* __restrict__ desc, int ntiles, const int* __restrict__ pad_word, int idxw,
+    const float* __restrict__ x_parts, const float* __restrict__ w_parts, int n_xparts, int n_wparts, int x_exp,
+    int* __restrict__ tile_ctr, float* __restrict__ out) {
+  typedef RingPShape<CC, COUT> S;
+  constexpr int NB = S::NB, SH = S::SH, KS = S::KS, NG = S::NG, SPLIT = S::SPLIT, KSW = S::KSW;
+  constexpr int RB = S::RB, SLOT = S::SLOT;
+  extern __shared__ __align__(16) unsigned char lds_raw[];
+  _Float16* wfh = (_Float16*)lds_raw;
+  _Float16* wfl = wfh + kRingTQ * SH;
+  float* red = (float*)(lds_raw + S::WF_BYTES);
+  unsigned char* ring_all = lds_raw + S::WF_BYTES + S::RED_BYTES;
+  unsigned char* rec_all = ring_all + S::RING_BYTES;
+  int* lcnt = (int*)(rec_all + S::REC_BYTES);
+  int* lqid = lcnt + 2 * kRingTQ;
+  int* ltile = lqid + 2 * kRingTQ;
+  int* idx_all = ltile + 4;
+
+  const int tid = threadIdx.x;
+  const int lane = tid & 63;
+  const int wave = __builtin_amdgcn_readfirstlane(tid >> 6);
+  const int p16 = lane & 15, j4 = lane >> 4;
+  unsigned char* ring = ring_all + wave * (4 * SLOT);
+  unsigned char* recb = rec_all + wave * (2 * 4 * 128);
+  int* idxbuf = idx_all + wave * (4 * idxw);
+  const unsigned ring_s = (unsigned)(uintptr_t)ring;
+  const unsigned rec_s = (unsigned)(uintptr_t)recb;
+  const unsigned idx_s = (unsigned)(uintptr_t)idxbuf;
+
+  float kx = 1.0e18f, ky = 1.0e18f, kz = 1.0e18f;
+  if (p16 < kKP) {
+    kx = kpts[3 * p16];
+    ky = kpts[3 * p16 + 1];
+    kz = kpts[3 * p16 + 2];
+  }
+  float sa2, unscale;
+  {
+    float* shf = reinterpret_cast<float*>(lds_raw);
+    int e = x_exp;
+    if (n_xparts > 0) e = pow2_exp_for(block_absmax(x_parts, shf, n_xparts));
+    const int kb = pow2_exp_for(block_absmax(w_parts, shf, n_wparts));
+    __syncthreads();
+    const int kk = pow2_exp_for(pow2f(15 + kInflExp) * (float)kmax);
+    sa2 = pow2f(kk);
+    unscale = pow2f(-e - kb) * pow2f(-(kInflExp + kk));
+  }
+  const float sw = pow2f(kInflExp);
+
+  const int ng = wave % NG, sp = wave / NG;
+  const int ks0 = sp * KSW;
+  kh8 bh[KSW], bl[KSW];
+#pragma unroll
+  for (int k = 0; k < KSW; ++k) {
+    const int ks = ks0 + k;
+    if (ks < KS) {
+      const size_t o = ((size_t)ng * KS + ks) * 512 + lane * 8;
+      bh[k] = *reinterpret_cast<const kh8*>(Wh + o);
+      bl[k] = *reinterpret_cast<const kh8*>(Wl + o);
+    } else {
+#pragma unroll
+      for (int e = 0; e < 8; ++e) { bh[k][e] = (_Float16)0.f; bl[k][e] = (_Float16)0.f; }
+    }
+  }
+  asm volatile("s_waitcnt vmcnt(0)" ::: "memory");
+
+  const int idxb = 2 * idxw;
+  auto stage_idx = [&](const int4 d, int par) {
+#pragma unroll
+    for (int sel = 0; sel < 2; ++sel) {
+      const int q = sel ? d.y : d.x;
+      for (int h = 0; h < idxw; h += 64) {
+        const int k = h + lane;
+        const unsigned dst = __builtin_amdgcn_readfirstlane(idx_s + (par * idxb + (sel ? 8 * d.z : 0) + h) * 4);
+        if (q >= 0 && k < kmax) ring_dma4(nbr, (unsigned)(((size_t)q * nbr_stride + k) * 4), dst);
+        else ring_dma4(pad_word, 0u, dst);
+      }
+    }
+  };
+  const unsigned a_idr = (lane >> 4) * 4, a_idc = (lane & 7) * 4;
+  const unsigned a_sw = (unsigned)(((lane & 15) ^ ((lane >> 4) << 2)) * 16);
+  auto issue_kstep = [&](int par, int j0, int live, int rp) {
+#pragma unroll
+    for (int g = 0; g < 4; ++g) {
+      const unsigned slot = __builtin_amdgcn_readfirstlane(ring_s + g * SLOT);
+      const unsigned rdst = __builtin_amdgcn_readfirstlane(rec_s + (rp * 4 + g) * 128);
+      if (g < live) {
+        const unsigned char* base = reinterpret_cast<const unsigned char*>(idxbuf) + (par * idxb + 8 * (j0 + g)) * 4;
+        const unsigned id0 = *reinterpret_cast<const unsigned*>(base + a_idr);
+        const unsigned id1 = *reinterpret_cast<const unsigned*>(base + a_idr + 16);
+        const unsigned idr = *reinterpret_cast<const unsigned*>(base + a_idc);
+        const unsigned o0 = min(id0, (unsigned)(ns - 1)) * RB + (a_sw ^ (unsigned)(((2 * g) & 3) * 16));
+        const unsigned o1 = min(id1, (unsigned)(ns - 1)) * RB + (a_sw ^ (unsigned)(((2 * g + 1) & 3) * 16));
+        const unsigned orec = min(idr, (unsigned)ns) * 16;
+        asm volatile("s_waitcnt lgkmcnt(0)" ::: "memory");
+        kstep_item_dma(xp, sxf, o0, o1, orec, slot, rdst);
+      } else {
+        *reinterpret_cast<uint4*>(ring + g * SLOT + lane * 16) = make_uint4(0u, 0u, 0u, 0u);
+        *reinterpret_cast<uint4*>(ring + g * SLOT + 1024 + lane * 16) = make_uint4(0u, 0u, 0u, 0u);
+        if (lane < 8)
+          *reinterpret_cast<float4*>(recb + (rp * 4 + g) * 128 + lane * 16) =
+              make_float4(-1.0e17f, -1.0e17f, -1.0e17f, __int_as_float(0));
+      }
+    }
+  };
+
+  if (tid == 0) {
+    const int t0 = __hip_atomic_fetch_add(tile_ctr, 3, __ATOMIC_RELAXED, __HIP_MEMORY_SCOPE_AGENT);
+    ltile[0] = t0;
+  }
+  __syncthreads();
+  int tile = __builtin_amdgcn_readfirstlane(ltile[0]);
+  int tile_nxt = tile + 1, tile_nn = tile + 2;
+  __syncthreads();
+  int4 d_cur = make_int4(-1, -1, 0, 0), d_nxt = make_int4(-1, -1, 0, 0);
+  if (tile < ntiles) d_cur = desc[(size_t)tile * 8 + wave];
+  if (tile_nxt < ntiles) d_nxt = desc[(size_t)tile_nxt * 8 + wave];
+  int rp = 0;
+  if (tile < ntiles) {
+    stage_idx(d_cur, 0);
+    asm volatile("s_waitcnt vmcnt(0)" ::: "memory");
+    if (tile_nxt < ntiles) stage_idx(d_nxt, 1);
+    if (d_cur.z > 0) issue_kstep(0, 0, min(4, d_cur.z), rp);
+  }
+
+  unsigned a_h0[NB], a_h1[NB];
+  const int a_lo = (lane & 8) ? -128 : 128;
+  {
+    const unsigned q = (unsigned)(lane & 15) >> 2, p = (unsigned)lane & 3u, g = (unsigned)j4;
+    const unsigned x0 = (q << 2) | ((2 * g) & 3u), x1 = (q << 2) | ((2 * g + 1) & 3u);
+    const unsigned b0 = ring_s + g * SLOT + q * RB + 8 * (p & 1), b1 = b0 + 4 * RB;
+#pragma unroll
+    for (int nb = 0; nb < NB; ++nb) {
+      const unsigned ch = 2 * nb + (p >> 1);
+      a_h0[nb] = b0 + 16 * (ch ^ x0);
+      a_h1[nb] = b1 + 16 * (ch ^ x1);
+    }
+  }
+
+  float pend_v[4] = {0.f, 0.f, 0.f, 0.f};
+  int pend_n[4] = {-1, -1, -1, -1};
+  auto flush_pending = [&]() {
+#pragma unroll
+    for (int r = 0; r < 4; ++r)
+      if (pend_n[r] >= 0) out[(size_t)pend_n[r] * COUT + ng * 16 + p16] = pend_v[r];
+  };
+  int par = 0;
+  for (; tile < ntiles; par ^= 1) {
+    const int4 d = d_cur;
+    int4 d_nn = make_int4(-1, -1, 0, 0);
+    const bool has_nxt = tile_nxt < ntiles, has_nn = tile_nn < ntiles;
+    if (has_nn) d_nn = desc[(size_t)tile_nn * 8 + wave];
+    int drawn = ntiles;
+    if (tid == 0 && has_nn) drawn = __hip_atomic_fetch_add(tile_ctr, 1, __ATOMIC_RELAXED, __HIP_MEMORY_SCOPE_AGENT);
+
+    asm volatile("s_waitcnt vmcnt(0)" ::: "memory");
+    const int nxt_live = has_nxt ? min(4, d_nxt.z) : 0;
+    bool first = true;
+#pragma unroll 1
+    for (int sel = 0; sel < 2; ++sel) {
+      const int n_it = sel ? d.w : d.z;
+      if (n_it == 0) continue;
+      const int qid = sel ? d.y : d.x, ql = sel ? 15 - wave : wave, jq = sel ? d.z : 0;
+      const float qx = q_xyz[3 * (size_t)qid], qy = q_xyz[3 * (size_t)qid + 1], qz = q_xyz[3 * (size_t)qid + 2];
+      const int nk = (n_it + 3) >> 2;
+      f32x4 acc[NB];
+#pragma unroll
+      for (int nb = 0; nb < NB; ++nb) acc[nb] = (f32x4){0.f, 0.f, 0.f, 0.f};
+      int cnt = 0;
+#pragma unroll 1
+      for (int t = 0; t < nk; ++t) {
+        if (!first) asm volatile("s_waitcnt vmcnt(0)" ::: "memory");
+        first = false;
+        kh8 xh[NB], xl[NB];
+#pragma unroll
+        for (int nb = 0; nb < NB; ++nb) {
+          xh[nb] = __builtin_shufflevector(tr_read_b64(a_h0[nb]), tr_read_b64(a_h1[nb]), 0, 1, 2, 3, 4, 5, 6, 7);
+          xl[nb] = __builtin_shufflevector(tr_read_b64(a_h0[nb] + a_lo), tr_read_b64(a_h1[nb] + a_lo), 0, 1, 2, 3, 4, 5, 6, 7);
+        }
+        asm volatile("s_waitcnt lgkmcnt(0)"
+                     : "+v"(xh[0]), "+v"(xh[1]), "+v"(xh[2]), "+v"(xh[3]), "+v"(xl[0]), "+v"(xl[1]), "+v"(xl[2]), "+v"(xl[3])
+                     :: "memory");
+        {
+          int npar = par, nj0 = jq + 4 * (t + 1), nlive = n_it - 4 * (t + 1);
+          if (nlive <= 0) {
+            if (sel == 0 && d.w > 0) { nj0 = d.z; nlive = d.w; }
+            else { npar = par ^ 1; nj0 = 0; nlive = nxt_live; }
+          }
+          if (nlive > 0) issue_kstep(npar, nj0, min(4, nlive), rp ^ 1);
+        }
+        const unsigned char* rbase = recb + (rp * 4 + j4) * 128;
+        typedef unsigned int u4_t __attribute__((ext_vector_type(4)));
+        u4_t ahu, alu;
+#pragma unroll
+        for (int j = 0; j < 4; ++j) {
+          float w[2];
+#pragma unroll
+          for (int h = 0; h < 2; ++h) {
+            const float4 rec = *reinterpret_cast<const float4*>(rbase + (2 * j + h) * 16);
+            const float dx = (rec.x - qx) - kx, dy = (rec.y - qy) - ky, dz = (rec.z - qz) - kz;
+            w[h] = fmaxf(0.f, 1.f - __builtin_amdgcn_sqrtf(dx * dx + dy * dy + dz * dz) * inv_extent);
+            cnt += __float_as_int(rec.w);
+          }
+          unsigned int hu, lu;
+          split_pk_s(w[0], w[1], sw, hu, lu);
+          ahu[j] = hu;
+          alu[j] = lu;
+          __builtin_amdgcn_sched_barrier(0);
+        }
+        const kh8 ah = __builtin_bit_cast(kh8, ahu), al = __builtin_bit_cast(kh8, alu);
+#pragma unroll
+        for (int nb = 0; nb < NB; ++nb) {
+          acc[nb] = __builtin_amdgcn_mfma_f32_16x16x32_f16(al, xh[nb], acc[nb], 0, 0, 0);
+          acc[nb] = __builtin_amdgcn_mfma_f32_16x16x32_f16(ah, xl[nb], acc[nb], 0, 0, 0);
+          acc[nb] = __builtin_amdgcn_mfma_f32_16x16x32_f16(ah, xh[nb], acc[nb], 0, 0, 0);
+        }
+        rp ^= 1;
+      }
+#pragma unroll
+      for (int nb = 0; nb < NB; ++nb) {
+#pragma unroll
+        for (int r = 0; r < 4; r += 2) {
+          unsigned int hu, lu;
+          split_pk_s(acc[nb][r], acc[nb][r + 1], sa2, hu, lu);
+          const int p = 4 * j4 + r;
+          const int o = ql * SH + p * CC + 16 * nb + p16;
+          unsigned short* ph = reinterpret_cast<unsigned short*>(wfh) + o;
+          unsigned short* pl = reinterpret_cast<unsigned short*>(wfl) + o;
+          ph[0] = (unsigned short)hu;
+          pl[0] = (unsigned short)lu;
+          if (p + 1 < kKP) {
+            ph[CC] = (unsigned short)(hu >> 16);
+            pl[CC] = (unsigned short)(lu >> 16);
+          }
+        }
+      }
+      int c = cnt;
+      c += __shfl_xor(c, 16, 64);
+      c += __shfl_xor(c, 32, 64);
+      if (lane == 0) {
+        lcnt[par * kRingTQ + ql] = c;
+        lqid[par * kRingTQ + ql] = qid;
+      }
+    }
+    if (first && nxt_live > 0) issue_kstep(par ^ 1, 0, nxt_live, rp);
+    if (lane == 0) {
+      if (d.x < 0) lqid[par * kRingTQ + wave] = -1;
+      if (d.y < 0) lqid[par * kRingTQ + 15 - wave] = -1;
+    }
+    if (sp == 0) flush_pending();
+    if (tid == 0) ltile[1 + par] = drawn;
+    if (has_nn) stage_idx(d_nn, par);
+    asm volatile("s_waitcnt lgkmcnt(0)" ::: "memory");
+    __builtin_amdgcn_s_barrier();
+
+    f32x4 acc2 = {0.f, 0.f, 0.f, 0.f};
+    {
+      const _Float16* ah_row = wfh + p16 * SH + 8 * j4;
+      const _Float16* al_row = wfl + p16 * SH + 8 * j4;
+#pragma unroll
+      for (int k = 0; k < KSW; ++k) {
+        const int ks = min(ks0 + k, KS - 1);
+        const kh8 ah = *reinterpret_cast<const kh8*>(ah_row + 32 * ks);
+        const kh8 al = *reinterpret_cast<const kh8*>(al_row + 32 * ks);
+        acc2 = __builtin_amdgcn_mfma_f32_16x16x32_f16(ah, bl[k], acc2, 0, 0, 0);
+        acc2 = __builtin_amdgcn_mfma_f32_16x16x32_f16(al, bh[k], acc2, 0, 0, 0);
+        acc2 = __builtin_amdgcn_mfma_f32_16x16x32_f16(ah, bh[k], acc2, 0, 0, 0);
+      }
+    }
+    if (sp > 0) {
+#pragma unroll
+      for (int r = 0; r < 4; ++r) red[((ng * (SPLIT - 1) + sp - 1) * 4 + r) * 64 + lane] = acc2[r];
+    }
+    asm volatile("s_waitcnt lgkmcnt(0)" ::: "memory");
+    __builtin_amdgcn_s_barrier();
+    if (sp == 0) {
+#pragma unroll
+      for (int s2 = 1; s2 < SPLIT; ++s2)
+#pragma unroll
+        for (int r = 0; r < 4; ++r) acc2[r] += red[((ng * (SPLIT - 1) + s2 - 1) * 4 + r) * 64 + lane];
+#pragma unroll
+      for (int r = 0; r < 4; ++r) {
+        const int ql = 4 * j4 + r;
+        pend_n[r] = lqid[par * kRingTQ + ql];
+        const float inv = unscale / (float)max(lcnt[par * kRingTQ + ql], 1);
+        pend_v[r] = acc2[r] * inv;
+      }
+    }
+    d_cur = d_nxt;
+    d_nxt = d_nn;
+    tile = tile_nxt;
+    tile_nxt = tile_nn;
+    tile_nn = __builtin_amdgcn_readfirstlane(ltile[1 + par]);
+  }
+  if (sp == 0) flush_pending();
+  asm volatile("s_waitcnt vmcnt(0)" ::: "memory");
+}
+
+template <int CC, int COUT>
+int launch_ringp(const float* q_xyz, int nq, int ns, const int* nbr, int nbr_stride, int kmax, const void* xp,
+                 const _Float16* Wh, const _Float16* Wl, const float* kpts, float inv_extent, const float4* sxf,
+                 const int4* desc, const int* pad_word, const float* x_parts, const float* w_parts, int n_xparts,
+                 int n_wparts, int x_exp, int* tile_ctr, float* out, hipStream_t stream) {
+  typedef RingPShape<CC, COUT> S;
+  const int idxw = kmax <= 64 ? 64 : 128;
+  const size_t lds = S::lds_bytes(idxw);
+  auto kern = k_kpconv_ringp<CC, COUT>;
+  ProfScope prof(stream, CC * 100000 + COUT, nq);
+  if (int rc = ensure_dyn_lds((const void*)kern, 160 * 1024)) return rc;
+  const int ntiles = cdiv(nq, kRingTQ);
+  const int n_cu = device_cu_count();
+  const int grid = ntiles < n_cu ? ntiles : n_cu;
+  hipLaunchKernelGGL(kern, dim3(grid), dim3(512), lds, stream, q_xyz, ns, nbr, nbr_stride, kmax,
+                     (const unsigned char*)xp, Wh, Wl, kpts, inv_extent, sxf, desc, ntiles, pad_word, idxw, x_parts,
+                     w_parts, n_xparts, n_wparts, x_exp, tile_ctr, out);
+  SPR_LAUNCH_CHECK();
+  return 0;
+}
+
+}
+
+void launch_rowflag_planes(const float* x, const float* s_xyz, int ns, int cin, unsigned char* flag, float4* sxf,
+                           int* tile_ctr, void* planes, const float* x_parts, int n_xparts, int x_exp,
+                           hipStream_t stream) {
   const int c4 = cin >> 2;
   const bool wide = (cin & 3) == 0 && c4 <= 64 && (c4 & (c4 - 1)) == 0;
   const long waves = wide ? cdiv(ns, (64 / c4) * 4) : (long)ns;
-  hipLaunchKernelGGL(k_rowflag, dim3(cdiv(waves * 64, 256)), dim3(256), 0, stream, x, s_xyz, ns, cin, flag, sxf, tile_ctr);
+  hipLaunchKernelGGL(k_rowflag, dim3(cdiv(waves * 64, 256)), dim3(256), 0, stream, x, s_xyz, ns, cin, flag, sxf, tile_ctr,
+                     wide ? (unsigned char*)planes : nullptr, x_parts, n_xparts, x_exp);
+}
+void launch_rowflag(const float* x, const float* s_xyz, int ns, int cin, unsigned char* flag, float4* sxf,
+                    int* tile_ctr, hipStream_t stream) {
+  launch_rowflag_planes(x, s_xyz, ns, cin, flag, sxf, tile_ctr, nullptr, nullptr, 0, 0, stream);
 }
 }
 
@@ -1101,6 +1491,11 @@
 static inline int w_chunk(int cin) { return cin % 64 == 0 ? 64 : 32; }
 static inline bool ring_shape(int cin, int cout) {
   return (cin == 32 || cin == 64) && cin * cout <= 4096 && cout % 32 == 0 && 8 % (cout / 16) == 0;
+}
+
+static inline bool plane_shape(int cin, int cout) { return cin == 64 && cout == 64; }
+static inline size_t plane_ws_bytes(int ns, int cin, int cout) {
+  return plane_shape(cin, cout) ? align_up((size_t)(ns > 0 ? ns : 1) * cin * 4, 256) : 0;
 }
 
 extern "C" size_t spr_kpconv_plan_bytes(int nq) { return plan_desc_bytes(nq) + 256; }
@@ -1139,7 +1534,7 @@
 extern "C" size_t spr_kpconv_workspace_bytes(int nq, int ns, int cin, int cout) {
   const size_t n = (size_t)(ns > 0 ? ns : 1);
   return align_up(n, 256) + align_up(16 * (n + 1), 256) + spr_kpconv_wplanes_bytes(cin, cout) +
-         2 * align_up(kAmaxParts * sizeof(float), 256) + spr_kpconv_plan_bytes(nq) + 256;
+         2 * align_up(kAmaxParts * sizeof(float), 256) + spr_kpconv_plan_bytes(nq) + 256 + plane_ws_bytes(ns, cin, cout);
 }
 
 extern "C" int spr_kpconv_fwd(const float* q_xyz, int nq, const float* s_xyz, int ns,
@@ -1163,13 +1558,14 @@
                           ws_bytes, stream_);
 }
 
-extern "C" int spr_kpconv_fwd_p(const float* q_xyz, int nq, const float* s_xyz, int ns,
-                                const int* nbr, int nbr_stride, int kmax, int rows_sorted,
-                                const float* x, int cin, const float* weights, int cout,
-                                const float* kernel_points, int n_kp, float kp_extent,
-                                float* out, int impl, const float* x_range, int x_range_n, const float* w_range,
-                                int w_range_n, const void* plan, const void* wplanes, void* ws, size_t ws_bytes,
-                                void* stream_) {
+static int kpconv_fwd_any(const float* q_xyz, int nq, const float* s_xyz, int ns,
+                          const int* nbr, int nbr_stride, int kmax, int rows_sorted,
+                          const float* x, const void* x_planes, const void* sxf_in, int x_exp, int cin,
+                          const float* weights, int cout,
+                          const float* kernel_points, int n_kp, float kp_extent,
+                          float* out, int impl, const float* x_range, int x_range_n, const float* w_range,
+                          int w_range_n, const void* plan, const void* wplanes, void* ws, size_t ws_bytes,
+                          void* stream_) {
   hipStream_t stream = (hipStream_t)stream_;
   SPR_REQUIRE((x_range == nullptr || x_range_n >= 1) && (w_range == nullptr || w_range_n >= 1),
               "kpconv: a range needs a count");
@@ -1186,6 +1582,11 @@
   float* w_parts = x_parts + align_up(kAmaxParts * sizeof(float), 256) / sizeof(float);
   void* ws_plan = (char*)w_parts + align_up(kAmaxParts * sizeof(float), 256);
   int* tile_ctr = (int*)((char*)ws_plan + spr_kpconv_plan_bytes(nq));
+  void* ws_planes = (char*)tile_ctr + 256;
+  const bool planes_in = x == nullptr;
+  SPR_REQUIRE(!planes_in || (x_planes != nullptr && sxf_in != nullptr && impl == 0 && n_kp == kKP && plane_shape(cin, cout) &&
+                             kmax <= 128),
+              "kpconv: the plane-row entry covers the 64 -> 64 ring shape (15 kernel points, kmax <= 128) only");
   SPR_REQUIRE(wplanes == nullptr || w_range != nullptr, "kpconv: prepared weight planes come with the range they were scaled by");
   if (wplanes != nullptr) {
     wh = (_Float16*)wplanes;
@@ -1202,26 +1603,39 @@
     return 0;
   }
 
-  launch_rowflag(x, s_xyz, ns, cin, flag, sxf, tile_ctr, stream);
-  SPR_LAUNCH_CHECK();
-
-  if ((impl == 0 || impl == 2) && n_kp == kKP && cin % 32 == 0 && cout % 32 == 0 && cout <= 256) {
-    const int ktot = n_kp * cin;
-    const float* xp = x_range != nullptr ? x_range : x_parts;
-    const float* wp = w_range != nullptr ? w_range : w_parts;
-    const int n_xp = x_range != nullptr ? x_range_n : kAmaxParts, n_wp = w_range != nullptr ? w_range_n : kAmaxParts;
-    if (x_range == nullptr && w_range == nullptr) {
+  const bool mfma_ok = (impl == 0 || impl == 2) && n_kp == kKP && cin % 32 == 0 && cout % 32 == 0 && cout <= 256;
+  const bool ring_ok = mfma_ok && impl == 0 && ring_shape(cin, cout) && kmax <= 128 && (size_t)ns * cin * 4 < (1ull << 32) &&
+                       (size_t)nq * nbr_stride * 4 < (1ull << 32);
+  const bool planes_ok = ring_ok && plane_shape(cin, cout);
+  SPR_REQUIRE(!planes_in || planes_ok, "kpconv: plane rows handed in for a launch the plane-row kernel does not cover");
+  const int ktot = n_kp * cin;
+  const float* xp = x_range != nullptr ? x_range : x_parts;
+  const float* wp = w_range != nullptr ? w_range : w_parts;
+  int n_xp = x_range != nullptr ? x_range_n : kAmaxParts;
+  const int n_wp = w_range != nullptr ? w_range_n : kAmaxParts;
+  if (planes_in) n_xp = 0;
+  if (mfma_ok) {
+    const bool need_x = x_range == nullptr && !planes_in;
+    if (need_x && w_range == nullptr) {
       if (int rc = launch_absmax2(x, ns, cin, cin, x_parts, weights, ktot, cout, cout, w_parts, stream)) return rc;
-    } else if (x_range == nullptr) {
+    } else if (need_x) {
       if (int rc = launch_absmax(x, ns, cin, cin, x_parts, stream)) return rc;
     } else if (w_range == nullptr) {
       if (int rc = launch_absmax(weights, ktot, cout, cout, w_parts, stream)) return rc;
     }
+  }
+  if (planes_in) {
+    sxf = (float4*)sxf_in;
+    if (hipMemsetAsync(tile_ctr, 0, sizeof(int), stream) != hipSuccess) return 1;
+  } else {
+    launch_rowflag_planes(x, s_xyz, ns, cin, flag, sxf, tile_ctr, planes_ok ? ws_planes : nullptr, xp, n_xp, 0, stream);
+    SPR_LAUNCH_CHECK();
+  }
+
+  if (mfma_ok) {
     if (wplanes == nullptr)
       hipLaunchKernelGGL(k_w_prep, dim3(cdiv((long)ktot * cout, 256)), dim3(256), 0, stream, weights, cin, cout,
                          w_chunk(cin), wp, n_wp, wh, wl);
-    const bool ring_ok = impl == 0 && ring_shape(cin, cout) && kmax <= 128 && (size_t)ns * cin * 4 < (1ull << 32) &&
-                         (size_t)nq * nbr_stride * 4 < (1ull << 32);
     if (ring_ok) {
       if (plan == nullptr) {
         if (int rc = spr_kpconv_plan(nbr, nq, ns, nbr_stride, kmax, rows_sorted, nullptr, ws_plan,
@@ -1233,7 +1647,10 @@
 #define SPR_RING_ARGS                                                                                       \
   q_xyz, nq, ns, nbr, nbr_stride, kmax, x, wh, wl, kernel_points, inv_extent, sxf, desc, pad_word, xp, wp, \
       n_xp, n_wp, tile_ctr, out, stream
-      if (cin == 64 && cout == 64) return launch_ring<64, 64, SPR_KP_NS64>(SPR_RING_ARGS);
+      if (planes_ok)
+        return launch_ringp<64, 64>(q_xyz, nq, ns, nbr, nbr_stride, kmax, planes_in ? x_planes : ws_planes, wh, wl,
+                                    kernel_points, inv_extent, sxf, desc, pad_word, xp, wp, n_xp, n_wp, x_exp, tile_ctr,
+                                    out, stream);
       if (cin == 64 && cout == 32) return launch_ring<64, 32, 4>(SPR_RING_ARGS);
       if (cin == 32 && cout == 32) return launch_ring<32, 32, 3>(SPR_RING_ARGS);
       if (cin == 32 && cout == 64) return launch_ring<32, 64, 8>(SPR_RING_ARGS);
@@ -1261,3 +1678,49 @@
   SPR_LAUNCH_CHECK();
   return 0;
 }
+
+extern "C" int spr_kpconv_fwd_p(const float* q_xyz, int nq, const float* s_xyz, int ns,
+                                const int* nbr, int nbr_stride, int kmax, int rows_sorted,
+                                const float* x, int cin, const float* weights, int cout,
+                                const float* kernel_points, int n_kp, float kp_extent,
+                                float* out, int impl, const float* x_range, int x_range_n, const float* w_range,
+                                int w_range_n, const void* plan, const void* wplanes, void* ws, size_t ws_bytes,
+                                void* stream_) {
+  SPR_REQUIRE(x != nullptr, "kpconv: x is required");
+  return kpconv_fwd_any(q_xyz, nq, s_xyz, ns, nbr, nbr_stride, kmax, rows_sorted, x, nullptr, nullptr, 0, cin, weights,
+                        cout, kernel_points, n_kp, kp_extent, out, impl, x_range, x_range_n, w_range, w_range_n, plan,
+                        wplanes, ws, ws_bytes, stream_);
+}
+
+extern "C" int spr_kpconv_plane_exp(float amax) { return pow2_exp_for(amax); }
+
+extern "C" int spr_kpconv_planes_supported(int cin, int cout) { return plane_shape(cin, cout) ? 1 : 0; }
+
+extern "C" size_t spr_kpconv_sxf_bytes(int ns) { return 16 * ((size_t)(ns > 0 ? ns : 1) + 1); }
+
+extern "C" int spr_kpconv_make_planes(const float* x, const float* s_xyz, int ns, int cin, int x_exp, void* planes,
+                                      void* sxf, unsigned char* flag, void* stream_) {
+  hipStream_t stream = (hipStream_t)stream_;
+  const int c4 = cin >> 2;
+  SPR_REQUIRE(ns > 0 && (cin & 3) == 0 && c4 >= 1 && c4 <= 64 && (c4 & (c4 - 1)) == 0,
+              "kpconv planes: cin must be 4 times a power of two, at most 256");
+  SPR_REQUIRE(x != nullptr && s_xyz != nullptr && planes != nullptr && sxf != nullptr && flag != nullptr,
+              "kpconv planes: null argument");
+  SPR_REQUIRE(x_exp >= -60 && x_exp <= 60, "kpconv planes: exponent out of range");
+  launch_rowflag_planes(x, s_xyz, ns, cin, flag, (float4*)sxf, nullptr, planes, nullptr, 0, x_exp, stream);
+  SPR_LAUNCH_CHECK();
+  return 0;
+}
+
+extern "C" int spr_kpconv_fwd_planes(const float* q_xyz, int nq, const float* s_xyz, int ns,
+                                     const int* nbr, int nbr_stride, int kmax, int rows_sorted,
+                                     const void* x_planes, int x_exp, const void* sxf, int cin,
+                                     const float* weights, int cout,
+                                     const float* kernel_points, int n_kp, float kp_extent,
+                                     float* out, const float* w_range, int w_range_n, const void* plan,
+                                     const void* wplanes, void* ws, size_t ws_bytes, void* stream_) {
+  SPR_REQUIRE(x_exp >= -60 && x_exp <= 60, "kpconv planes: exponent out of range");
+  return kpconv_fwd_any(q_xyz, nq, s_xyz, ns, nbr, nbr_stride, kmax, rows_sorted, nullptr, x_planes, sxf, x_exp, cin,
+                        weights, cout, kernel_points, n_kp, kp_extent, out, 0, nullptr, 0, w_range, w_range_n, plan,
+                        wplanes, ws, ws_bytes, stream_);
+}
diff --git a/superpoints_registration_amd/csrc/spr_common.h b/superpoints_registration_amd/csrc/spr_common.h
--- a/superpoints_registration_amd/csrc/spr_common.h
+++ b/superpoints_registration_amd/csrc/spr_common.h
@@ -135,6 +135,11 @@
       : "v"(hi_u), "v"(a), "v"(b), "v"(s));
 }
 
+__device__ __forceinline__ void plane_row_split4(const float4 v, float s, uint2& h, uint2& l) {
+  split_pk_s(v.x, v.y, s, h.x, l.x);
+  split_pk_s(v.z, v.w, s, h.y, l.y);
+}
+
 __device__ __forceinline__ void split_pk_s_hi(float a, float b, float s, unsigned int& hi_u) {
   asm("v_fma_mixlo_f16 %0, %1, %3, 0 op_sel_hi:[0,0,0]\n\t"
       "v_fma_mixhi_f16 %0, %2, %3, 0 op_sel_hi:[0,0,0]"
diff --git a/superpoints_registration_amd/ops.py b/superpoints_registration_amd/ops.py
--- a/superpoints_registration_amd/ops.py
+++ b/superpoints_registration_amd/ops.py
@@ -338,6 +338,46 @@
                                   _ptr(kernel_points), n_kp, float(kp_extent), _ptr(out), int(impl),
                                   _ptr(xr), int(xr_n), _ptr(wr), int(wr_n), _ptr(plan), _ptr(wplanes),
                                   _ptr(ws), ws.numel(), _stream(x)), "spr_kpconv_fwd_p")
+    return out
+
+
+def kpconv_make_planes(s_pts, x, bound: float):
+    s_pts = _dev(s_pts, "s_pts", torch.float32)
+    x = _dev(x, "x", torch.float32)
+    ns, cin = x.shape
+    L = _lib.lib()
+    x_exp = int(L.spr_kpconv_plane_exp(float(bound)))
+    planes = torch.empty((ns, 4 * cin), dtype=torch.uint8, device=x.device)
+    sxf = torch.empty((L.spr_kpconv_sxf_bytes(ns),), dtype=torch.uint8, device=x.device)
+    flag = torch.empty((ns,), dtype=torch.uint8, device=x.device)
+    _lib.check(L.spr_kpconv_make_planes(_ptr(x), _ptr(s_pts), ns, cin, x_exp, _ptr(planes), _ptr(sxf), _ptr(flag),
+                                        _stream(x)), "spr_kpconv_make_planes")
+    return planes, x_exp, sxf, flag
+
+
+def kpconv_planes(q_pts, s_pts, nbr, planes, x_exp: int, sxf, weights, kernel_points, kp_extent: float,
+                  rows_sorted: bool = False, order: Optional[torch.Tensor] = None) -> torch.Tensor:
+    q_pts = _dev(q_pts, "q_pts", torch.float32)
+    s_pts = _dev(s_pts, "s_pts", torch.float32)
+    weights = _dev(weights, "weights", torch.float32)
+    kernel_points = _dev(kernel_points, "kernel_points", torch.float32)
+    if nbr.dtype != torch.int32:
+        nbr = nbr.to(torch.int32)
+    nbr = nbr.contiguous()
+    nq, ns, kmax = q_pts.shape[0], s_pts.shape[0], nbr.shape[1]
+    n_kp, cin, cout = weights.shape
+    assert planes.shape == (ns, 4 * cin) and planes.dtype == torch.uint8
+    L = _lib.lib()
+    ws = _workspace(L.spr_kpconv_workspace_bytes(nq, ns, cin, cout), planes.device)
+    out = torch.empty((nq, cout), dtype=torch.float32, device=planes.device)
+    wr, wr_n = _static_range(weights)
+    plan = _kpconv_plan(nbr, nq, ns, kmax, kmax, bool(rows_sorted), order)
+    wplanes = _kpconv_wplanes(weights, wr, wr_n) if wr is not None else None
+    _lib.check(L.spr_kpconv_fwd_planes(_ptr(q_pts), nq, _ptr(s_pts), ns, _ptr(nbr), kmax, kmax, int(bool(rows_sorted)),
+                                       _ptr(planes), int(x_exp), _ptr(sxf), cin, _ptr(weights), cout,
+                                       _ptr(kernel_points), n_kp, float(kp_extent), _ptr(out), _ptr(wr), int(wr_n),
+                                       _ptr(plan), _ptr(wplanes), _ptr(ws), ws.numel(), _stream(planes)),
+               "spr_kpconv_fwd_planes")
     return out
 
 
```

Measured after the change: 1229 pairs/s (median of 2 runs). About the same (-0.6%).
